# blahgeek/OpenCV-octVR

Hardware: AMD Instinct MI355X
Metric: stitched megapixels/sec (6x4K->8K equirect) (higher is better)
Workload: dtype u8

## Files before the change

### include/octvr_hip.h

```cpp
#ifndef OCTVR_HIP_H
#define OCTVR_HIP_H

#include <stddef.h>
#include <stdint.h>

#ifdef __cplusplus
extern "C" {
#endif

#define OCTVR_HIP_ABI_VERSION 1

enum {
    OCTVR_OK = 0,
    OCTVR_E_INVALID = -1,
    OCTVR_E_PARSE = -2,
    OCTVR_E_HIP = -3,
    OCTVR_E_UNSUPPORTED = -4,
    OCTVR_E_IO = -5
};

typedef struct octvr_rig octvr_rig;
typedef struct octvr_mapper octvr_mapper;

typedef struct {
    int roi_x, roi_y, roi_w, roi_h;
    const float* map1;
    const float* map2;
    const uint8_t* mask;
    const uint8_t* seam_mask;
    const float* vignette;
    int vignette_w, vignette_h;
} octvr_input_view;

int octvr_abi_version(void);
const char* octvr_last_error(void);
int octvr_device_count(int* count);

int octvr_dev_malloc(int device, size_t bytes, void** ptr);
int octvr_dev_free(void* ptr);
int octvr_memcpy_h2d(void* dst_dev, const void* src_host, size_t bytes);
int octvr_memcpy_d2h(void* dst_host, const void* src_dev, size_t bytes);
int octvr_stream_sync(void* stream);

int octvr_rig_create_json(const char* json, int out_w, int out_h, int use_roi, int device, octvr_rig** rig);
#define OCTVR_JSON_EXACT 1
int octvr_rig_create(const char* out_type, const char* out_opts_json, int out_w, int out_h, int device, int flags,
                     octvr_rig** rig);
int octvr_rig_add_input(octvr_rig* rig, const char* type, const char* opts_json, int overlay, int use_roi, int flags);
int octvr_rig_load_dat(const char* path, octvr_rig** rig);
typedef size_t (*octvr_read_fn)(void* ctx, void* buf, size_t n);
typedef size_t (*octvr_write_fn)(void* ctx, const void* data, size_t n);
int octvr_rig_load_stream(octvr_read_fn read, void* ctx, octvr_rig** rig);
int octvr_rig_dump_stream(octvr_rig* rig, octvr_write_fn write, void* ctx);
int octvr_rig_dump_dat(octvr_rig* rig, const char* path);
int octvr_rig_create_masks(octvr_rig* rig, int device);
int octvr_rig_create_from_arrays(int out_w, int out_h, int n_inputs, const int* rois, const float* const* map1,
                                 const float* const* map2, const uint8_t* const* masks,
                                 const uint8_t* const* seam_masks_or_null, octvr_rig** rig);
int octvr_rig_set_vignette(octvr_rig* rig, int i, int overlay, const float* map, int w, int h);
int octvr_rig_add_overlay_arrays(octvr_rig* rig, const int* roi, const float* map1, const float* map2,
                                 const uint8_t* mask);
int octvr_rig_num_inputs(const octvr_rig* rig, int* n);
int octvr_rig_out_size(const octvr_rig* rig, int* w, int* h);
int octvr_rig_get_input(const octvr_rig* rig, int i, octvr_input_view* view);

int octvr_rig_num_overlays(const octvr_rig* rig, int* n);
int octvr_rig_get_overlay(const octvr_rig* rig, int i, octvr_input_view* view);
int octvr_rig_morph_controlpoints(octvr_rig* rig, const char* control_points_json, int* n_used);
int octvr_rig_get_triangles(const octvr_rig* rig, int i, float* src, float* dst, int cap, int* n);
void octvr_rig_destroy(octvr_rig* rig);
int octvr_rig_clone(const octvr_rig* rig, octvr_rig** out);

int octvr_mapper_create(const octvr_rig* rig, int device, int n_inputs, const int* in_w, const int* in_h, int blend,
                        int enable_gain, int scale_w, int scale_h, octvr_mapper** mapper);
#define OCTVR_REMAP_TEXTURE 1
int octvr_mapper_create_ex(const octvr_rig* rig, int device, int n_inputs, const int* in_w, const int* in_h, int blend,
                           int enable_gain, int scale_w, int scale_h, int flags, octvr_mapper** mapper);
int octvr_mapper_stitch_yuv420p(octvr_mapper* mapper, const uint8_t* const* in_dev, const size_t* in_pitch,
                                uint8_t* out_dev, size_t out_pitch, const double* gains, int n_gains, void* stream);
int octvr_mapper_stitch_batch(octvr_mapper* mapper, int n_frames, const uint8_t* const* in_dev, const size_t* in_pitch,
                              uint8_t* const* out_dev, size_t out_pitch, const double* gains, void* stream);
int octvr_mapper_stitch_preview(octvr_mapper* mapper, const uint8_t* const* in_dev, const size_t* in_pitch,
                                uint8_t* out_dev, size_t out_pitch, uint8_t* preview_dev, int preview_w, int preview_h,
                                size_t preview_pitch, const double* gains, int n_gains, void* stream);
int octvr_mapper_gains(octvr_mapper* mapper, double* gains, int n);
#define OCTVR_MAX_FRAMES_IN_FLIGHT 16
int octvr_mapper_set_frames_in_flight(octvr_mapper* mapper, int k);
enum { OCTVR_PIX_YUV420P = 0, OCTVR_PIX_NV12 = 1 };
int octvr_mapper_set_pixel_formats(octvr_mapper* mapper, int in_format, int out_format);
int octvr_mapper_pixel_formats(const octvr_mapper* mapper, int* in_format, int* out_format);
int octvr_mapper_traffic(const octvr_mapper* mapper, double* bytes_per_frame);
int octvr_mapper_traffic_parts(const octvr_mapper* mapper, double* lut_bytes, double* frame_bytes);
int octvr_mapper_set_timing(octvr_mapper* mapper, int enable);
int octvr_mapper_kernel_time(octvr_mapper* mapper, double* total_ms, int* launches);
int octvr_mapper_kernel_busy(octvr_mapper* mapper, double* span_ms, double* busy_ms, int* launches);
int octvr_mapper_kernel_intervals(octvr_mapper* mapper, double* start_ms, double* end_ms, int cap, int* n);
int octvr_interval_union(const double* start, const double* end, int n, double* span, double* busy);
int octvr_mapper_info(const octvr_mapper* mapper, char* buf, size_t len);
void octvr_mapper_destroy(octvr_mapper* mapper);

typedef struct octvr_async octvr_async;
int octvr_async_create(const octvr_rig* const* rigs, int n_rigs, int device, int n_inputs, const int* in_w,
                       const int* in_h, int out_w, int out_h, const int* blend_modes, const int* gain_modes,
                       const double* output_regions, octvr_async** async);
int octvr_async_create_ex(const octvr_rig* const* rigs, int n_rigs, int device, int n_inputs, const int* in_w,
                          const int* in_h, int out_w, int out_h, const int* blend_modes, const int* gain_modes,
                          const double* output_regions, int flags, octvr_async** async);
int octvr_async_create_preview(const octvr_rig* const* rigs, int n_rigs, int device, int n_inputs, const int* in_w,
                               const int* in_h, int out_w, int out_h, const int* blend_modes, const int* gain_modes,
                               const double* output_regions, int flags, int preview_w, int preview_h,
                               octvr_async** async);
typedef struct octvr_preview_header {
    int width, height;
    int step;
    double fps;
} octvr_preview_header;
int octvr_async_pop_preview(octvr_async* async, uint8_t* rgb, size_t pitch, octvr_preview_header* hdr);
typedef void (*octvr_preview_sink)(void* user, const uint8_t* rgb, size_t pitch, const octvr_preview_header* hdr);
int octvr_async_set_preview_sink(octvr_async* async, octvr_preview_sink sink, void* user);
int octvr_async_info(const octvr_async* async, char* buf, size_t len);
int octvr_async_set_pixel_formats(octvr_async* async, int in_format, int out_format);
int octvr_async_pixel_formats(const octvr_async* async, int* in_format, int* out_format);
int octvr_async_push(octvr_async* async, const uint8_t* const* in_planes, const size_t* in_pitches,
                     uint8_t* const* out_planes, const size_t* out_pitches);
int octvr_async_push_device(octvr_async* async, const uint8_t* const* in_dev, const size_t* in_pitch,
                            uint8_t* out_dev, size_t out_pitch, void* ready_event);
int octvr_async_pop(octvr_async* async);
int octvr_async_register_output(octvr_async* async, uint8_t* const* planes, const size_t* pitches);
int octvr_async_unregister_output(octvr_async* async, uint8_t* const* planes);
int octvr_async_pending(const octvr_async* async, int* n);
void octvr_async_destroy(octvr_async* async);

typedef struct octvr_fastmapper octvr_fastmapper;
int octvr_fastmapper_create(const octvr_rig* rig, int device, int n_inputs, const int* in_w, const int* in_h,
                            octvr_fastmapper** fastmapper);
int octvr_fastmapper_stitch_nv12(octvr_fastmapper* fastmapper, const uint8_t* const* in_dev, const size_t* in_pitch,
                                 uint8_t* out_dev, size_t out_pitch, void* stream);
int octvr_fastmapper_stitch_nv12_batch(octvr_fastmapper* fastmapper, int n_frames, const uint8_t* const* in_dev,
                                       const size_t* in_pitch, uint8_t* const* out_dev, size_t out_pitch, void* stream);
int octvr_fastmapper_traffic(const octvr_fastmapper* fastmapper, double* bytes);
int octvr_fastmapper_traffic_parts(const octvr_fastmapper* fastmapper, double* lut_bytes, double* frame_bytes);
void octvr_fastmapper_destroy(octvr_fastmapper* fastmapper);

int octvr_remap_u8(const uint8_t* src_dev, int sw, int sh, size_t spitch, int cn, const float* map1_dev,
                   const float* map2_dev, int mw, int mh, size_t mpitch_elems, float scale_x, float scale_y,
                   uint8_t* dst_dev, size_t dpitch, void* stream);

int octvr_fill_poly_u8(uint8_t* img, int w, int h, const int* pts, int npts, uint8_t color);
int octvr_png_decode_rgb(const uint8_t* png, size_t n, uint8_t* rgb, size_t rgb_cap, int* w, int* h);

int octvr_rig_lut_recomputed(const octvr_rig* rig, int i, uint64_t* n);
int octvr_debug_project_f64(const char* json, int out_w, int out_h, int input, int device, int where, double* x,
                            double* y, uint8_t* fragile);
int octvr_debug_fastmapper_audit(const octvr_rig* rig, int n_inputs, const int* in_w, const int* in_h, int force_wide,
                                 int pitch_pad, char* json, size_t len);
int octvr_debug_tiled_lut_info(const octvr_rig* rig, int n_inputs, const int* in_w, const int* in_h, int flags,
                               char* json, size_t len);
int octvr_debug_gain_plan(const octvr_rig* rig, int n_inputs, const int* in_w, const int* in_h, int flags,
                          uint32_t* samples, uint16_t* partners, size_t cap, size_t* count);
int octvr_debug_json_number(const char* json, int flags, double* value);
int octvr_debug_pack_runs(int n_inputs, const int* in_w, const int* in_h, const uint32_t* runs, int n_runs,
                          const uint8_t* const* planes, const size_t* pitches, int format, uint8_t* packed, size_t cap,
                          size_t* sizes, size_t* bytes);
int octvr_debug_worker_failure(int n_threads, int failing);
int octvr_selftest_sat_u8(const float* in_dev, uint8_t* out_dev, int n, int method, void* stream);

#ifdef __cplusplus
}
#endif
#endif
```

### opencv-octvr_amd/csrc/composite.hip

```cpp
#include <hip/hip_runtime.h>
#include <hip/hip_ext.h>

#include <algorithm>
#include <cfloat>
#include <cstddef>
#include <cstdint>
#include <cstring>

#include "device_common.hpp"
#include "kernels.hpp"

namespace octvr {

static_assert(sizeof(TileSlot) == 16, "TileSlot layout");

static_assert(offsetof(FrameBatch<1>, src) == 0 && offsetof(FrameBatch<4>, src) == 0, "FrameBatch layout");
__device__ __forceinline__ SourceFrame kernarg_frame(uint32_t idx) {
    const kSourceFrame* kf = (const kSourceFrame*)__builtin_amdgcn_kernarg_segment_ptr();
    SourceFrame s;
    s.yuv = kf[idx].yuv;
    s.w = kf[idx].w;
    s.h = kf[idx].h;
    s.pitch = kf[idx].pitch;
    s.vig = kf[idx].vig;
// ... 53 lines not shown
#pragma unroll
        for (int j = 1; j < kTileSlots; j++) q += (j < nslots && c >= (int)(slot_word(m, j, 3) & 0xFFFFu)) ? 1 : 0;
    }
    const uint32_t d0 = slot_word(m, q, 0), d1 = slot_word(m, q, 1);
    const uint32_t d2 = slot_word(m, q, 2), d3 = slot_word(m, q, 3);
    s.cam = s.live ? (d0 & 31u) : 0u;
    s.bw = d0 >> 16;
    s.bh = d1 & 0xFFFFu;
    s.lds = d1 >> 16;
    s.bx0 = d2 & 0xFFFFu;
    s.by0 = d2 >> 16;
    s.chunk0 = d3 & 0xFFFFu;
    s.f = kernarg_frame(m.fbase + s.cam);
    return s;
}

template <bool DWORD_STAGE, bool VIG, int IN = kInPlanar>
__device__ __forceinline__ void stage_load(const StageSlot& s, uint32_t stride, uint32_t g, StageGroup& sg,
                                           bool nv12 = false) {
    const bool ok = s.live && (g & kGroupValid) != 0u;
    const uint32_t row_k = ok ? (g & 255u) : 0u, col_k = ok ? (g >> 8) & 31u : 0u;
    const SourceFrame& f = s.f;
    const bool img = s.bx0 + col_k * 8u < (uint32_t)f.w && s.by0 + row_k < (uint32_t)f.h;
    const uint32_t row = img ? row_k : 0u, col = img ? col_k : 0u;
    const uint32_t p32 = (uint32_t)f.pitch;
    const gu8* base = (const gu8*)f.yuv;
    const gu8* Yb = base + (int64_t)s.by0 * f.pitch + s.bx0;
    const gu8* Ub = base + (int64_t)(f.h + (int)(s.by0 >> 1)) * f.pitch + (s.bx0 >> 1);
    const gu8* Vb = Ub + (f.w >> 1);
    const uint32_t oy = __umul24(row, p32) + col * 8u, oc = __umul24(row >> 1, p32) + col * 4u;
    if (IN == kInNv12 || (IN == kInRuntime && nv12)) {
        const gu8* Cp = base + (int64_t)(f.h + (int)(s.by0 >> 1)) * f.pitch + s.bx0 + (oc + col * 4u);
        if (DWORD_STAGE) {
            const uint64_t yy = *(const gu64*)(Yb + oy);
            const uint64_t cc = *(const gu64*)Cp;
            sg.y0 = (uint32_t)yy;
            sg.y1 = (uint32_t)(yy >> 32);
            sg.uq = (uint32_t)cc;
            sg.vq = (uint32_t)(cc >> 32);
        } else {
            const gu8* Yp = Yb + oy;
            sg.y0 = (uint32_t)Yp[0] | ((uint32_t)Yp[1] << 8) | ((uint32_t)Yp[2] << 16) | ((uint32_t)Yp[3] << 24);
            sg.y1 = (uint32_t)Yp[4] | ((uint32_t)Yp[5] << 8) | ((uint32_t)Yp[6] << 16) | ((uint32_t)Yp[7] << 24);
            sg.uq = (uint32_t)Cp[0] | ((uint32_t)Cp[1] << 8) | ((uint32_t)Cp[2] << 16) | ((uint32_t)Cp[3] << 24);
            sg.vq = (uint32_t)Cp[4] | ((uint32_t)Cp[5] << 8) | ((uint32_t)Cp[6] << 16) | ((uint32_t)Cp[7] << 24);
        }
    } else if (DWORD_STAGE) {
        const uint64_t yy = *(const gu64*)(Yb + oy);
        sg.y0 = (uint32_t)yy;
        sg.y1 = (uint32_t)(yy >> 32);
        sg.uq = *(const gu32*)(Ub + oc);
        sg.vq = *(const gu32*)(Vb + oc);
    } else {
        const gu8* Yp = Yb + oy;
        const gu8* Up = Ub + oc;
        const gu8* Vp = Vb + oc;
        sg.y0 = (uint32_t)Yp[0] | ((uint32_t)Yp[1] << 8) | ((uint32_t)Yp[2] << 16) | ((uint32_t)Yp[3] << 24);
        sg.y1 = (uint32_t)Yp[4] | ((uint32_t)Yp[5] << 8) | ((uint32_t)Yp[6] << 16) | ((uint32_t)Yp[7] << 24);
        sg.uq = (uint32_t)Up[0] | ((uint32_t)Up[1] << 8) | ((uint32_t)Up[2] << 16) | ((uint32_t)Up[3] << 24);
        sg.vq = (uint32_t)Vp[0] | ((uint32_t)Vp[1] << 8) | ((uint32_t)Vp[2] << 16) | ((uint32_t)Vp[3] << 24);
    }
    sg.flags = img ? 0u : kStageBlack;
    if (IN == kInRuntime && nv12) sg.flags |= kStageNv12;
    sg.dst = ok ? (int32_t)(s.lds + __umul24(row_k, stride) + col_k * 8u) : -1;
    if (VIG) {
        const float* gv = f.vig ? f.vig + (int64_t)(s.by0 + row) * f.w + s.bx0 + col * 8u
                                : reinterpret_cast<const float*>(f.yuv);
        sg.g0 = *reinterpret_cast<const float4*>(gv);
        sg.g1 = *reinterpret_cast<const float4*>(gv + 4);
        if (!f.vig) sg.flags |= kStageNoVig;
    }
}

__device__ __forceinline__ uint16_t group_issue(const __amdgpu_buffer_rsrc_t& gr, int t, int t_end, int lg) {
    const int tt = (t < t_end ? t : 0) >> lg;
    return __builtin_amdgcn_raw_buffer_load_b16(gr, (uint32_t)threadIdx.x * 2u,
                                                (uint32_t)uniform(tt) * (uint32_t)(kGroupFirst * 64 * 2), 0);
}

template <bool VIG, int IN = kInPlanar>
__device__ __forceinline__ void stage_store(const StageGroup& sg, uint32_t* s_rgb) {
    if (sg.dst < 0) return;
    const bool black = (sg.flags & kStageBlack) != 0;
    const uint32_t y0 = black ? 0u : sg.y0, y1 = black ? 0u : sg.y1;
    uint32_t uq = black ? 0u : sg.uq ^ 0x80808080u, vq = black ? 0u : sg.vq ^ 0x80808080u;
    auto ch = [](uint32_t w, int k) { return (float)(signed char)((w >> (8 * k)) & 255u); };
    uint4 a, b;
    if constexpr (IN == kInNv12) {
        yuv2_to_rgba_c(y0 & 255u, (y0 >> 8) & 255u, ch(uq, 0), ch(uq, 1), a.x, a.y);
        yuv2_to_rgba_c((y0 >> 16) & 255u, y0 >> 24, ch(uq, 2), ch(uq, 3), a.z, a.w);
        yuv2_to_rgba_c(y1 & 255u, (y1 >> 8) & 255u, ch(vq, 0), ch(vq, 1), b.x, b.y);
        yuv2_to_rgba_c((y1 >> 16) & 255u, y1 >> 24, ch(vq, 2), ch(vq, 3), b.z, b.w);
    } else {
        if (IN == kInRuntime && (sg.flags & kStageNv12)) {
            const uint32_t lo = uq, hi = vq;
            uq = __builtin_amdgcn_perm(hi, lo, 0x06040200u);
            vq = __builtin_amdgcn_perm(hi, lo, 0x07050301u);
        }
        yuv2_to_rgba_c(y0 & 255u, (y0 >> 8) & 255u, ch(uq, 0), ch(vq, 0), a.x, a.y);
        yuv2_to_rgba_c((y0 >> 16) & 255u, y0 >> 24, ch(uq, 1), ch(vq, 1), a.z, a.w);
        yuv2_to_rgba_c(y1 & 255u, (y1 >> 8) & 255u, ch(uq, 2), ch(vq, 2), b.x, b.y);
        yuv2_to_rgba_c((y1 >> 16) & 255u, y1 >> 24, ch(uq, 3), ch(vq, 3), b.z, b.w);
    }
    if (VIG && !(sg.flags & kStageNoVig)) {
        a.x = vig_mul(a.x, sg.g0.x);
        a.y = vig_mul(a.y, sg.g0.y);
        a.z = vig_mul(a.z, sg.g0.z);
        a.w = vig_mul(a.w, sg.g0.w);
        b.x = vig_mul(b.x, sg.g1.x);
        b.y = vig_mul(b.y, sg.g1.y);
        b.z = vig_mul(b.z, sg.g1.z);
        b.w = vig_mul(b.w, sg.g1.w);
    }
    *reinterpret_cast<uint4*>(s_rgb + sg.dst) = a;
    *reinterpret_cast<uint4*>(s_rgb + sg.dst + 4) = b;
}

constexpr int kStitchBlocksPerCU = 6;
constexpr int kStitchRegBlocks = kStitchBlocksPerCU + 1;
constexpr int kStitchSgprs = 96, kStitchVgprs = 72;
constexpr int kStitchTexRegBlocks = 5, kStitchTexVgprs = 96;

__device__ __forceinline__ uint4 meta_issue(const __amdgpu_buffer_rsrc_t& mr, int t, int t_end, int lg) {
    const int lane = threadIdx.x & 63;
    const int tt = (t < t_end ? t : 0) >> lg;
    typedef unsigned int u32x4 __attribute__((ext_vector_type(4)));
    uint4 v;
    if (lane < kMetaWords) {
        const u32x4 r = __builtin_amdgcn_raw_buffer_load_b128(mr, (uint32_t)lane * 16u,
                                                              (uint32_t)uniform(tt) * (uint32_t)(kMetaWords * 16), 0);
        v = uint4{r.x, r.y, r.z, r.w};
    }
    return v;
}

__device__ __forceinline__ TileMeta meta_read(const uint4& v, int t, int lg, int cam_lg) {
    TileMeta m;
    m.t = t;
    m.frame = (uint32_t)t & ((1u << lg) - 1u);
    m.fbase = m.frame << cam_lg;
    m.v = v;
    m.tile = (uint32_t)__builtin_amdgcn_readlane((int)v.x, 0);
    m.nslots = (uint32_t)__builtin_amdgcn_readlane((int)v.y, 0);
    m.stride = (uint32_t)__builtin_amdgcn_readlane((int)v.w, 0);
    m.map = (uint32_t)__builtin_amdgcn_readlane((int)v.z, 0);
    return m;
}

struct TileData {
    uint4 e4[kItemHalves];
    StageGroup sg;
};

template <bool DWORD_STAGE, bool VIG, bool E24, int IN = kInPlanar>
__device__ __forceinline__ void data_issue(const __amdgpu_buffer_rsrc_t& er, const TileMeta& m, int t_end, int lg,
                                           const StageSlot& sl, uint32_t g, TileData& d, bool nv12 = false) {
    const bool live = m.t < t_end;
    const int tid = threadIdx.x;
#pragma unroll
    for (int h = 0; h < kItemHalves; h++) {
        const uint32_t so =
            (uint32_t)uniform(((live ? m.t : 0) >> lg) * kItemHalves + h) * (uint32_t)(kTilePx * (E24 ? 3 : 4));
        if constexpr (E24) {
            typedef unsigned int u32x3e __attribute__((ext_vector_type(3)));
            const u32x3e v = __builtin_amdgcn_raw_buffer_load_b96(er, (uint32_t)tid * 12u, so, 0);
            d.e4[h] = uint4{v.x, v.y, v.z, 0u};
        } else {
            typedef unsigned int u32x4e __attribute__((ext_vector_type(4)));
            const u32x4e v = __builtin_amdgcn_raw_buffer_load_b128(er, (uint32_t)tid * 16u, so, 0);
            d.e4[h] = uint4{v.x, v.y, v.z, v.w};
        }
    }
    if (!sl.live) {
        d.sg.dst = -1;
        return;
    }
    stage_load<DWORD_STAGE, VIG, IN>(sl, m.stride & ((1u << kStrideBits) - 1u), g, d.sg, nv12);
}

template <int MODE>
__device__ __forceinline__ QuadOut finish_any(const float (&rgb)[4][3], const f32x2_t (&gain)[4]) {
    if constexpr (MODE == 0) {
        return finish_quad2f(rgb, gain);
    } else {
        uint32_t px[4];
#pragma unroll
        for (int p = 0; p < 4; p++) {
            uint32_t v = pack_u8(rgb[p][0] * gain[p].x, 0, 0u);
            v = pack_u8(rgb[p][1] * gain[p].x, 1, v);
            px[p] = pack_u8(rgb[p][2] * gain[p].x, 2, v);
        }
        return QuadOut{px[0], px[1], px[2], px[3]};
    }
}

struct RgbaSink {
    __amdgpu_buffer_rsrc_t rsrc;
    const MbCamLevel* cams;
};

__device__ __forceinline__ OutFrame make_result_frame(const RgbaOut& r) {
    OutFrame o;
    o.rsrc = __builtin_amdgcn_make_buffer_rsrc(r.res, 0, (int)r.res_bytes, 0x00020000);
    o.pitch = r.res_pitch;
    o.u_off = r.res_u_off;
    o.v_off = r.res_v_off;
    return o;
}

template <int OUT = kOutPlanar>
__device__ __forceinline__ void store_result(const OutFrame& o, bool rgba, const QuadOut& q, int x, int y, bool in) {
    if (rgba) {
        typedef unsigned int u32x2 __attribute__((ext_vector_type(2)));
        const uint32_t off = in ? (uint32_t)y * o.pitch + (uint32_t)x * 4u : kDropOffset;
        __builtin_amdgcn_raw_buffer_store_b64(u32x2{q.y01, q.y23}, o.rsrc, off, 0, 0);
        __builtin_amdgcn_raw_buffer_store_b64(u32x2{q.u, q.v}, o.rsrc, in ? off + o.pitch : kDropOffset, 0, 0);
        return;
    }
    const uint32_t px[4] = {q.y01, q.y23, q.u, q.v};
    store_quad<OUT>(o, quad_yuv(px), x, y, in);
}

__device__ __forceinline__ void store_rgba(const RgbaSink& o, const QuadOut& q, uint32_t cam, int x, int y, bool in) {
    typedef __attribute__((address_space(4))) const MbCamLevel kMbCamLevel;
    const kMbCamLevel* c = (const kMbCamLevel*)o.cams + uniform((int)cam);
    const int ox = c->ox, oy = c->oy, cw = c->w, chh = c->h;
    const uint32_t goff = c->g_off, gp = c->g_pitch;
    const int xl = x - ox, yl = y - oy;
    const bool ok = in && xl >= 0 && yl >= 0 && xl < cw && yl < chh;
    const uint32_t off = ok ? goff + (uint32_t)yl * gp + (uint32_t)xl * 4u : kDropOffset;
    typedef unsigned int u32x2 __attribute__((ext_vector_type(2)));
    const u32x2 r0 = {q.y01, q.y23}, r1 = {q.u, q.v};
    __builtin_amdgcn_raw_buffer_store_b64(r0, o.rsrc, off, 0, 0);
    __builtin_amdgcn_raw_buffer_store_b64(r1, o.rsrc, ok ? off + gp : kDropOffset, 0, 0);
}

template <int MODE, int OUT = kOutPlanar>
__device__ __forceinline__ void store_half(const OutFrame& of, const RgbaSink& ro, bool res_rgba, const QuadOut& q,
                                           uint32_t cam, uint32_t flags, int h, int x, int y, bool in) {
    if constexpr (MODE == 0) {
        store_quad<OUT>(of, q, x, y, in);
    } else {
        const int q4 = (int)((threadIdx.x & 63u) >> 4);
        if (flags & item_g0_bit(h, q4)) store_rgba(ro, q, cam, x, y, in);
        if (flags & item_result_bit(h, q4)) store_result<OUT>(of, res_rgba, q, x, y, in);
    }
}

struct alignas(16) StitchLds {
    uint32_t rgb[kTileLdsBytes / 4];
    uint32_t spare[kMaxCams];
    f32x2_t slot_gain[kTileSlots];
    uint32_t claim[2];
    uint32_t pad[2];
};
static_assert(sizeof(StitchLds) == 0x4000, "the weight table at LDS 0x4000 (wtab_read)");

__device__ __forceinline__ uint2 wtab_read(uint32_t e) {
    typedef __attribute__((address_space(3))) const uint64_t lds_u64;
    const uint64_t w = *(const lds_u64*)(uintptr_t)((e & 0x1FF8u) | 0x4000u);
    return uint2{(uint32_t)w, (uint32_t)(w >> 32)};
}

__device__ __forceinline__ uint32_t tap_off(uint32_t e) { return (e >> 13) & 0x3FFFu; }

constexpr int kPfPlanar = 0, kPfNv12 = 3, kPfRuntime = 4;
template <bool DWORD_STAGE, int MODE, bool VIG, bool TEX, int LG, bool E24, int PF = kPfPlanar>
__device__ __forceinline__ void stitch_tiled_body(const FrameBatch<1 << LG>& frames, TiledLut lut, int W, int H, int use_gain,
                                                  int64_t out_pitch, RgbaOut rgba, int pix = 0) {
    constexpr int IN = PF == kPfRuntime ? kInRuntime : PF == kPfNv12 ? kInNv12 : kInPlanar;
    constexpr int OUT = PF == kPfRuntime ? kOutRuntime : PF == kPfNv12 ? kOutNv12 : kOutPlanar;
    const bool in_nv12 = IN == kInRuntime ? (pix & kPixInNv12) != 0 : IN == kInNv12;
    const bool out_nv12 = OUT == kOutRuntime ? (pix & kPixOutNv12) != 0 : OUT == kOutNv12;
    __shared__ StitchLds L;
    extern __shared__ __attribute__((aligned(16))) uint2 s_wtab[];
    uint32_t* const s_rgb = L.rgb;
    float* const s_gain = reinterpret_cast<float*>(s_wtab + 1024);
    constexpr int lg = LG, cam_lg = LG <= 1 ? 5 : 4;
    static_assert(MODE == 0 || LG == 0, "frame batches: MODE 0 only");
    f32x2_t* const s_slot_gain = L.slot_gain;
    uint32_t* const s_claim = L.claim;
    constexpr int kItemH = kTileH * kItemHalves;

    const int groups = kStitchBands;
    const int g = blockIdx.x % groups;
    const int step = (gridDim.x - g + groups - 1) / groups;
    const int t_begin = lut.bands[g] << lg;
    const int t_end = lut.bands[g + 1] << lg;
    const __amdgpu_buffer_rsrc_t ersrc = __builtin_amdgcn_make_buffer_rsrc(
        const_cast<uint32_t*>(lut.entries), 0,
        (int)((uint32_t)max(lut.n_items, 1) * (uint32_t)(kItemHalves * kTilePx * (E24 ? 3 : 4))), 0x00020000);
    const __amdgpu_buffer_rsrc_t mrsrc = __builtin_amdgcn_make_buffer_rsrc(
        const_cast<TileHdr*>(lut.meta), 0, (int)((uint32_t)max(lut.n_items, 1) * (uint32_t)(kMetaWords * 16)), 0x00020000);
    const __amdgpu_buffer_rsrc_t grsrc = __builtin_amdgcn_make_buffer_rsrc(
        const_cast<uint16_t*>(lut.grp0), 0, (int)((uint32_t)max(lut.n_items, 1) * (uint32_t)(kGroupFirst * 64 * 2)), 0x00020000);
    const __amdgpu_buffer_rsrc_t g1rsrc =
        __builtin_amdgcn_make_buffer_rsrc(const_cast<uint16_t*>(lut.grp1), 0, (int)(lut.n_grp1 * 2u), 0x00020000);
    OutFrame of{};
    RgbaSink ro{};
    bool res_rgba = false;
    const int out_bytes = (int)((uint32_t)out_pitch * (uint32_t)(H + H / 2));
    if constexpr (MODE == 0) {
        of = make_out_frame(kernarg_out<1 << LG>(0), W, H, out_pitch, out_nv12);
    } else {
        ro = RgbaSink{__builtin_amdgcn_make_buffer_rsrc(rgba.base, 0, (int)rgba.bytes, 0x00020000), rgba.cams};
        of = make_result_frame(rgba);
        res_rgba = rgba.res_rgba != 0;
    }
    const int tid = threadIdx.x;
    const int qx = tid & 63, qy = tid >> 6;

    if (tid < (1 << (lg + cam_lg))) {
        const double* gf = kernarg_gains<1 << LG>((uint32_t)tid >> cam_lg);
        s_gain[tid] = use_gain ? (float)gf[tid & ((1 << cam_lg) - 1)] : 1.0f;
    }
    if (tid < kTileZeroDwords) s_rgb[tid] = 0u;
#pragma unroll
    for (int k = 0; k < 4; k++) s_wtab[tid + 256 * k] = bilerp_weights((uint32_t)(tid + 256 * k));
    const int t0 = t_begin + (int)(blockIdx.x / groups);
    const int dyn0 = t_begin + 3 * step;
    uint32_t* const q = lut.queue + g * kQueueStride;
    const int wave = uniform(tid >> 6);
    TileMeta cur = meta_read(meta_issue(mrsrc, t0, t_end, lg), t0, lg, cam_lg);
    const uint32_t g0 = group_issue(grsrc, t0, t_end, lg);
    __syncthreads();
    TileData d;
    data_issue<DWORD_STAGE, VIG, E24, IN>(ersrc, cur, t_end, lg, stage_slot<true>(cur, t_end, wave), g0, d, in_nv12);
    int t_mv = t0 + step < t_end ? t0 + step : t_end;
    int t_n2 = t_mv < t_end && t0 + 2 * step < t_end ? t0 + 2 * step : t_end;
    uint4 mv = meta_issue(mrsrc, t_mv, t_end, lg);
    uint16_t mg = group_issue(grsrc, t_mv, t_end, lg);
    uint32_t claim = 0u;
    bool claimed = false;
    bool first = true;
    asm volatile("" : "+v"(mv.x), "+v"(mv.y), "+v"(mv.z), "+v"(mv.w), "+v"(mg));
#pragma unroll
    for (int h = 0; h < kItemHalves; h++) {
        asm volatile("" : "+v"(d.e4[h].x), "+v"(d.e4[h].y), "+v"(d.e4[h].z));
        if constexpr (!E24) asm volatile("" : "+v"(d.e4[h].w));
    }
    asm volatile("" : "+v"(d.sg.y0), "+v"(d.sg.y1), "+v"(d.sg.uq), "+v"(d.sg.vq));

    QuadOut prev[kItemHalves];
#pragma unroll
    for (int h = 0; h < kItemHalves; h++) prev[h] = QuadOut{0u, 0u, 0u, 0u};
    int px = 0, py = 0;
    const uint32_t lane_y = (uint32_t)(2 * qy) * of.pitch + (uint32_t)(2 * qx),
                   lane_c = (uint32_t)qy * of.pitch + (uint32_t)(out_nv12 ? 2 * qx : qx);
    int pox = 0, poy = 0;
    bool pfull = false;
    uint32_t pcam = 0, pfl = 0;
    uint32_t pfr = 0;
    bool pin = false;
    uint32_t par = 0;
    while (cur.t < t_end) {
        const int x = (int)(cur.tile & 0xFFFFu) * kTileW + qx * 2, y = (int)(cur.tile >> 16) * kItemH + qy * 2;
        const uint32_t S = cur.stride & ((1u << kStrideBits) - 1u);
        uint4 e4[kItemHalves];
#pragma unroll
        for (int h = 0; h < kItemHalves; h++) e4[h] = d.e4[h];
        __syncthreads();
        if (tid < kTileZeroDwords) s_rgb[tid] = 0u;
        const TileMeta nxt = meta_read(mv, t_mv, lg, cam_lg);
        {
            const uint32_t cw = (uint32_t)__shfl((int)cur.v.x, 1 + (tid & 3), 64);
            const float gs = s_gain[cur.fbase + (cw & 31u)];
            const float gc = MODE == 0 ? __builtin_fminf(__builtin_fmaxf(gs, 0.f), FLT_MAX) : gs;
            if (tid < kTileSlots) s_slot_gain[tid] = f32x2_t{gc, gc};
        }
        if (claimed && tid == 0) s_claim[par] = claim;
        stage_store<VIG, IN>(d.sg, s_rgb);
        const uint32_t nch = (cur.nslots >> 8) & 0xFFu;
        if (nch > (uint32_t)kGroupFirst) {
            const uint32_t ovf = cur.stride >> kStrideBits;
            for (int c = kGroupFirst + wave; c < (int)nch; c += 4) {
                const uint32_t gk = __builtin_amdgcn_raw_buffer_load_b16(
                    g1rsrc, (uint32_t)(tid & 63) * 2u, (ovf + (uint32_t)(c - kGroupFirst)) * 128u, 0);
                StageGroup sg;
                stage_load<DWORD_STAGE, VIG, IN>(stage_slot(cur, t_end, c), S, gk, sg, in_nv12);
                stage_store<VIG, IN>(sg, s_rgb);
            }
        }
        __syncthreads();
        if (!first) {
            const uint32_t cv = min((uint32_t)uniform((int)s_claim[par]), 0x3FFFFFFFu);
            const int v = claimed ? dyn0 + (int)cv : t_end;
            t_n2 = v < t_end ? v : t_end;
        }
        first = false;
        if (MODE == 0 && lg) of.rsrc = __builtin_amdgcn_make_buffer_rsrc(kernarg_out<1 << LG>(pfr), 0, out_bytes, 0x00020000);
        if (MODE == 0 && pfull) {
#pragma unroll
            for (int h = 0; h < kItemHalves; h++) {
                const uint32_t sy = (uint32_t)uniform((poy + h * kTileH) * (int)of.pitch + pox);
                const uint32_t sc =
                    (uint32_t)uniform(((poy + h * kTileH) >> 1) * (int)of.pitch + (out_nv12 ? pox : pox >> 1));
                __builtin_amdgcn_raw_buffer_store_b16((uint16_t)prev[h].y01, of.rsrc, lane_y, sy, kOutPolicy);
                __builtin_amdgcn_raw_buffer_store_b16((uint16_t)prev[h].y23, of.rsrc, lane_y, sy + of.pitch, kOutPolicy);
                if (out_nv12) {
                    __builtin_amdgcn_raw_buffer_store_b16((uint16_t)(prev[h].u | prev[h].v << 8), of.rsrc, lane_c,
                                                          sc + of.u_off, kOutPolicy);
                } else {
                    __builtin_amdgcn_raw_buffer_store_b8((uint8_t)prev[h].u, of.rsrc, lane_c, sc + of.u_off, kOutPolicy);
                    __builtin_amdgcn_raw_buffer_store_b8((uint8_t)prev[h].v, of.rsrc, lane_c, sc + of.v_off, kOutPolicy);
                }
            }
        } else {
#pragma unroll
            for (int h = 0; h < kItemHalves; h++)
                store_half<MODE, OUT>(of, ro, res_rgba, prev[h], pcam, pfl, h, px, py + h * kTileH, pin && py + h * kTileH < H);
        }
        data_issue<DWORD_STAGE, VIG, E24, IN>(ersrc, nxt, t_end, lg, stage_slot<true>(nxt, t_end, wave), mg, d, in_nv12);
        mv = meta_issue(mrsrc, t_n2, t_end, lg);
        mg = group_issue(grsrc, t_n2, t_end, lg);
        t_mv = t_n2;
        claimed = t_n2 < t_end;
        if (claimed && tid == 0) {
            int zero = tid;
            asm volatile("" : "+v"(zero));
            claim = __hip_atomic_fetch_add(q + zero, 1u, __ATOMIC_RELAXED, __HIP_MEMORY_SCOPE_AGENT);
        }
#pragma unroll
        for (int h = 0; h < kItemHalves; h++) {
            const uint32_t ent[4] = {e4[h].x, E24 ? __builtin_amdgcn_alignbit(e4[h].y, e4[h].x, 24u) : e4[h].y,
                                     E24 ? __builtin_amdgcn_alignbit(e4[h].z, e4[h].y, 16u) : e4[h].z,
                                     E24 ? e4[h].z >> 8 : e4[h].w};
            float rgb[4][3];
            f32x2_t gain[4];
#pragma unroll
            for (int p = 0; p < 4; p++) {
                const uint32_t e = ent[p];
                const uint8_t* r0 = reinterpret_cast<const uint8_t*>(s_rgb) +
                                    (TEX ? (e >> 15) & 0x3FFCu : E24 ? (e >> 10) & 0x3FFCu : tap_off(e));
                const uint8_t* r1 = r0 + 4u * S;
                const uint32_t c00 = reinterpret_cast<const uint32_t*>(r0)[0];
                const uint32_t c01 = reinterpret_cast<const uint32_t*>(r0)[1];
                const uint32_t c10 = reinterpret_cast<const uint32_t*>(r1)[0];
                const uint32_t c11 = reinterpret_cast<const uint32_t*>(r1)[1];
                if constexpr (TEX) {
                    tex_bilerp_f(c00, c01, c10, c11, (e >> 1) & 255u, (e >> 9) & 255u, rgb[p]);
                    gain[p] = *reinterpret_cast<const f32x2_t*>(reinterpret_cast<const uint8_t*>(s_slot_gain) + ((e >> 30) << 3));
                } else {
                    bilerp_rgba_w(c00, c01, c10, c11, wtab_read(E24 ? e << 1 : e), rgb[p]);
                    const uint32_t go = E24 ? (e << 3) & 0x18u : e >> 27;
                    gain[p] = *reinterpret_cast<const f32x2_t*>(reinterpret_cast<const uint8_t*>(s_slot_gain) + go);
                }
                if (MODE == 1 && !E24 && (e & kEntryNoGain)) gain[p] = f32x2_t{1.0f, 1.0f};
            }
            prev[h] = finish_any<MODE>(rgb, gain);
        }
        px = x;
        py = y;
        pox = (int)(cur.tile & 0xFFFFu) * kTileW;
        poy = (int)(cur.tile >> 16) * kItemH;
        pfull = pox + kTileW <= W && poy + kItemH <= H;
        pcam = (cur.nslots >> 16) & 31u;
        pfr = cur.frame;
        pfl = MODE == 1 ? (cur.map >> 8) & 0xFFFFu : 0u;
        pin = x < W && y < H;
        par ^= 1u;
        cur = nxt;
    }
    if (tid == 0) {
        asm volatile("s_waitcnt vmcnt(0)" ::: "memory");
        (void)claim;
        if (__hip_atomic_fetch_add(lut.queue + kStitchBands * kQueueStride, 1u, __ATOMIC_RELAXED,
                                   __HIP_MEMORY_SCOPE_AGENT) == gridDim.x - 1) {
            for (int k = 0; k <= kStitchBands; k++)
                __hip_atomic_exchange(lut.queue + k * kQueueStride, 0u, __ATOMIC_RELAXED, __HIP_MEMORY_SCOPE_AGENT);
        }
    }
    if (MODE == 0 && lg) of.rsrc = __builtin_amdgcn_make_buffer_rsrc(kernarg_out<1 << LG>(pfr), 0, out_bytes, 0x00020000);
#pragma unroll
    for (int h = 0; h < kItemHalves; h++)
        store_half<MODE, OUT>(of, ro, res_rgba, prev[h], pcam, pfl, h, px, py + h * kTileH, pin && py + h * kTileH < H);
}

template <bool DWORD_STAGE, int MODE, bool VIG, int LG, bool E24, int PF = kPfPlanar>
__global__ void __launch_bounds__(256, kStitchRegBlocks) __attribute__((amdgpu_num_sgpr(kStitchSgprs)))
__attribute__((amdgpu_num_vgpr(kStitchVgprs))) stitch_tiled_kernel(FrameBatch<1 << LG> frames, TiledLut lut, int W, int H,
                                                                   int use_gain, int64_t out_pitch, RgbaOut rgba) {
    stitch_tiled_body<DWORD_STAGE, MODE, VIG, false, LG, E24, PF>(frames, lut, W, H, use_gain, out_pitch, rgba);
}
template <int MODE, bool TEX, int LG, bool E24>
__global__ void __launch_bounds__(256, kStitchTexRegBlocks) __attribute__((amdgpu_num_sgpr(kStitchSgprs)))
__attribute__((amdgpu_num_vgpr(kStitchTexVgprs))) stitch_tiled_pix_kernel(FrameBatch<1 << LG> frames, TiledLut lut, int W,
                                                                          int H, int use_gain, int64_t out_pitch,
                                                                          RgbaOut rgba, int pix) {
    stitch_tiled_body<false, MODE, true, TEX, LG, E24, kPfRuntime>(frames, lut, W, H, use_gain, out_pitch, rgba, pix);
}
template <bool DWORD_STAGE, int MODE, bool VIG, int LG>
__global__ void __launch_bounds__(256, kStitchTexRegBlocks) __attribute__((amdgpu_num_sgpr(kStitchSgprs)))
__attribute__((amdgpu_num_vgpr(kStitchTexVgprs))) stitch_tiled_tex_kernel(FrameBatch<1 << LG> frames, TiledLut lut, int W,
                                                                          int H, int use_gain, int64_t out_pitch,
                                                                          RgbaOut rgba) {
    stitch_tiled_body<DWORD_STAGE, MODE, VIG, true, LG, false>(frames, lut, W, H, use_gain, out_pitch, rgba);
}

template <int MODE>
__global__ void __launch_bounds__(256) stitch_wide_kernel(FrameSet frames, TiledLut lut, int W, int H,
                                                          const double* gains, int use_gain, uint8_t* out,
                                                          int64_t out_pitch, RgbaOut rgba, int pix) {
    __shared__ float s_gain[kMaxCams];
    const int tid = threadIdx.x;
    if (tid < kMaxCams) s_gain[tid] = use_gain ? (float)gains[tid] : 1.0f;
    __syncthreads();
    OutFrame of{};
    RgbaSink ro{};
    if constexpr (MODE == 0) {
        of = make_out_frame(out, W, H, out_pitch, (pix & kPixOutNv12) != 0);
    } else {
        ro = RgbaSink{__builtin_amdgcn_make_buffer_rsrc(rgba.base, 0, (int)rgba.bytes, 0x00020000), rgba.cams};
        of = make_result_frame(rgba);
    }
    const uint32_t tile = (uint32_t)uniform((int)lut.wide_tiles[blockIdx.x]);
    const int x = (int)(tile & 0xFFFFu) * kTileW + (tid & 63) * 2, y = (int)(tile >> 16) * kTileH + (tid >> 6) * 2;
    const uint4* wp = reinterpret_cast<const uint4*>(lut.wide + (int64_t)blockIdx.x * kTilePx) + tid * 2;
    const uint4 e0 = wp[0], e1 = wp[1];
    const uint32_t xy[4] = {e0.x, e0.z, e1.x, e1.z};
    const uint32_t cd[4] = {e0.y, e0.w, e1.y, e1.w};
    Taps tp[4];
#pragma unroll
    for (int p = 0; p < 4; p++) {
        if (pix & kPixInNv12)
            gather_taps<true>(frames, xy[p], cd[p], tp[p]);
        else
            gather_taps<false>(frames, xy[p], cd[p], tp[p]);
    }
    uint32_t rgb[4][3];
    f32x2_t gain[4];
#pragma unroll
    for (int p = 0; p < 4; p++) {
        if (cd[p] & kCodeTex)
            tex_bilerp(tp[p].c[0], tp[p].c[1], tp[p].c[2], tp[p].c[3], tp[p].fx, tp[p].fy, rgb[p]);
        else
            bilerp_rgba(tp[p].c[0], tp[p].c[1], tp[p].c[2], tp[p].c[3], tp[p].fx, tp[p].fy, rgb[p]);
        float gp = (MODE == 1 && (cd[p] & kCodeNoGain)) ? 1.0f : s_gain[(cd[p] >> 10) & 31u];
        gain[p] = f32x2_t{gp, gp};
    }
    const uint32_t camb = MODE == 1 ? (uint32_t)uniform((int)lut.wide_cams[blockIdx.x]) : 0u;
    float rgbf[4][3];
#pragma unroll
    for (int p = 0; p < 4; p++)
#pragma unroll
        for (int ch = 0; ch < 3; ch++) rgbf[p][ch] = (float)rgb[p][ch];
    const uint32_t fl = ((camb >> 8) & 15u) | ((camb >> 12) & 15u) << 8;
    store_half<MODE, kOutRuntime>(of, ro, rgba.res_rgba != 0, finish_any<MODE>(rgbf, gain), camb & 31u, fl, 0, x, y,
                                  x < W && y < H);
}

struct TiledLaunch {
    int blocks;
    const FrameSet* frames;
    const double* const* gains;
    uint8_t* const* out;
    const TiledLut& lut;
    int W, H, use_gain;
    int64_t out_pitch;
    const RgbaOut& rgba;
    hipStream_t s;
    hipEvent_t ev0, ev1;
    int pix;
    bool dw, vig;
    int lg;
};

template <bool DW, int MODE, bool V, bool TEX, int LG, bool E24, int PF>
constexpr auto tiled_kernel() {
    if constexpr (PF == kPfRuntime)
        return &stitch_tiled_pix_kernel<MODE, TEX, LG, E24>;
    else if constexpr (TEX)
        return &stitch_tiled_tex_kernel<DW, MODE, V, LG>;
    else
        return &stitch_tiled_kernel<DW, MODE, V, LG, E24, PF>;
}

static hipError_t stitch_lds_check(const void* kernel) {
    hipFuncAttributes a;
    const hipError_t e = hipFuncGetAttributes(&a, kernel);
    if (e != hipSuccess) return e;
    return a.sharedSizeBytes == sizeof(StitchLds) ? hipSuccess : hipErrorInvalidKernelFile;
}

constexpr uint32_t kStitchDynLds = kWtabBytes + 4u * 2u * kMaxCams;

template <int LG>
static void frame_batch(const FrameSet* frames, const double* const* gains, uint8_t* const* out,
                        FrameBatch<1 << LG>& fb) {
    constexpr int cam_lg = FrameBatch<1 << LG>::kCamLog2;
    memset(&fb, 0, sizeof fb);
    for (int f = 0; f < (1 << LG); f++) {
        for (int i = 0; i < (1 << cam_lg); i++) fb.src[(f << cam_lg) + i] = frames[f].f[i];
        fb.out[f] = out ? out[f] : nullptr;
        fb.gains[f] = gains[f];
    }
}

template <bool DW, int MODE, bool V, bool TEX, int LG, bool E24, int PF>
static hipError_t launch_tiled(const TiledLaunch& a) {
    static_assert(PF != kPfNv12 || !TEX, "compiled-in NV12: the default sampling's instances");
    constexpr auto kernel = tiled_kernel<DW, MODE, V, TEX, LG, E24, PF>();
    static const hipError_t lds_ok = stitch_lds_check(reinterpret_cast<const void*>(kernel));
    if (lds_ok != hipSuccess) return lds_ok;
    FrameBatch<1 << LG> fb;
    frame_batch<LG>(a.frames, a.gains, a.out, fb);
    const dim3 grid(a.blocks), block(256);
    if constexpr (PF == kPfRuntime) {
        if (a.ev0) (void)hipEventRecord(a.ev0, a.s);
        hipLaunchKernelGGL(kernel, grid, block, kStitchDynLds, a.s, fb, a.lut, a.W, a.H, a.use_gain, a.out_pitch, a.rgba,
                           a.pix);
        if (a.ev0) (void)hipEventRecord(a.ev1, a.s);
    } else if constexpr (TEX) {
        hipLaunchKernelGGL(kernel, grid, block, kStitchDynLds, a.s, fb, a.lut, a.W, a.H, a.use_gain, a.out_pitch, a.rgba);
        if (a.ev0) (void)hipEventRecord(a.ev1, a.s);
    } else if (a.ev0) {
        hipExtLaunchKernelGGL(kernel, grid, block, kStitchDynLds, a.s, a.ev0, a.ev1, 0, fb, a.lut, a.W, a.H, a.use_gain,
                              a.out_pitch, a.rgba);
    } else {
        hipLaunchKernelGGL(kernel, grid, block, kStitchDynLds, a.s, fb, a.lut, a.W, a.H, a.use_gain, a.out_pitch, a.rgba);
    }
    return hipGetLastError();
}

template <bool DW, int MODE, bool V, bool TEX, bool E24, int PF = kPfPlanar>
static hipError_t launch_tiled_lg(const TiledLaunch& a) {
    if constexpr (MODE == 0) {
        if (a.lg == 1) return launch_tiled<DW, MODE, V, TEX, 1, E24, PF>(a);
        if (a.lg == 2) return launch_tiled<DW, MODE, V, TEX, 2, E24, PF>(a);
    }
    if (a.lg != 0) return hipErrorInvalidValue;
    return launch_tiled<DW, MODE, V, TEX, 0, E24, PF>(a);
}

template <int MODE, bool TEX, bool E24>
static hipError_t launch_tiled_vd(const TiledLaunch& a) {
    if (a.pix) {
        if constexpr (MODE == 0 && !TEX) {
            if (a.pix == (kPixInNv12 | kPixOutNv12) && a.dw && !a.vig)
                return launch_tiled_lg<true, MODE, false, TEX, E24, kPfNv12>(a);
        }
        return launch_tiled_lg<false, MODE, true, TEX, E24, kPfRuntime>(a);
    }
    if (a.dw && !a.vig) return launch_tiled_lg<true, MODE, false, TEX, E24>(a);
    if (a.dw) return launch_tiled_lg<true, MODE, true, TEX, E24>(a);
    if (!a.vig) return launch_tiled_lg<false, MODE, false, TEX, E24>(a);
    return launch_tiled_lg<false, MODE, true, TEX, E24>(a);
}

template <int MODE, bool TEX>
static hipError_t launch_tiled_for(const TiledLaunch& a) {
    if constexpr (!TEX) {
        if (a.lut.e24) return launch_tiled_vd<MODE, TEX, true>(a);
    } else {
        if (a.lut.e24) return hipErrorInvalidValue;
    }
    return launch_tiled_vd<MODE, TEX, false>(a);
}

template <int MODE>
static hipError_t launch_composite(const FrameSet* frames, int nf, const TiledLut& lut, int W, int H,
                                   const double* const* gains, int use_gain, uint8_t* const* out, int64_t out_pitch,
                                   const RgbaOut& rgba, hipStream_t s, hipEvent_t ev0 = nullptr,
                                   hipEvent_t ev1 = nullptr, int pix = 0) {
    if (pix & ~(kPixInNv12 | kPixOutNv12)) return hipErrorInvalidValue;
    if (lut.n_items > 0 && lut.qpl != kItemHalves) return hipErrorInvalidValue;
    const int lg = nf == 1 ? 0 : nf == 2 ? 1 : nf == 4 ? 2 : -1;
    if (lg < 0 || (MODE == 1 && nf != 1)) return hipErrorInvalidValue;
    const int cam_lg = nf <= 2 ? 5 : 4;
    for (int f = 0; f < nf; f++)
        for (int i = 1 << cam_lg; i < kMaxCams; i++)
            if (frames[f].f[i].yuv) return hipErrorInvalidValue;
    const bool ext_ev = ev0 && lut.n_items > 0 && lut.n_wide == 0;
    if (ev0 && !ext_ev) {
        const hipError_t e = hipEventRecord(ev0, s);
        if (e != hipSuccess) return e;
    }
    if (lut.n_items > 0) {
        const int units = lut.n_items * nf;
        int blocks = std::min(units, 256 * kStitchBlocksPerCU);
        if (units < 3 * 256 * kStitchBlocksPerCU) blocks = (units + 2) / 3;
        blocks = std::max(8, (blocks + 7) / 8 * 8);
        bool dw = true, vig = false;
        for (int f = 0; f < nf; f++)
            for (int i = 0; i < kMaxCams; i++) {
                const SourceFrame& sf = frames[f].f[i];
                if (!sf.yuv) continue;
                if ((reinterpret_cast<uintptr_t>(sf.yuv) & 7u) || (sf.pitch & 7) || (sf.w & 7)) dw = false;
                vig |= sf.vig != nullptr;
            }
        const TiledLaunch a{blocks, frames, gains, out, lut, W, H, use_gain, out_pitch, rgba, s,
                            ext_ev ? ev0 : nullptr, ext_ev ? ev1 : nullptr, pix, dw, vig, lg};
        const hipError_t e = lut.tex ? launch_tiled_for<MODE, true>(a) : launch_tiled_for<MODE, false>(a);
        if (e != hipSuccess) return e;
    }
    if (lut.n_wide > 0)
        for (int f = 0; f < nf; f++)
            hipLaunchKernelGGL(stitch_wide_kernel<MODE>, dim3(lut.n_wide), dim3(256), 0, s, frames[f], lut, W, H,
                               gains[f], use_gain, out ? out[f] : nullptr, out_pitch, rgba, pix);
    if (ev0 && !ext_ev) {
        const hipError_t e = hipEventRecord(ev1, s);
        if (e != hipSuccess) return e;
    }
    return hipGetLastError();
}

int composite_qpl() { return kItemHalves; }

hipError_t launch_stitch_batch(const FrameSet* frames, int nf, const TiledLut& lut, int W, int H,
                               const double* const* gains, int use_gain, uint8_t* const* out, int64_t out_pitch,
                               hipStream_t s, hipEvent_t ev0, hipEvent_t ev1, int pix) {
    if (nf < 1 || nf > kMaxBatch) return hipErrorInvalidValue;
    return launch_composite<0>(frames, nf, lut, W, H, gains, use_gain, out, out_pitch, RgbaOut{}, s, ev0, ev1, pix);
}

hipError_t launch_stitch(const FrameSet& frames, const TiledLut& lut, int W, int H, const double* gains,
                         int use_gain, uint8_t* out, int64_t out_pitch, hipStream_t s, hipEvent_t ev0, hipEvent_t ev1,
                         int pix) {
    return launch_composite<0>(&frames, 1, lut, W, H, &gains, use_gain, &out, out_pitch, RgbaOut{}, s, ev0, ev1, pix);
}

hipError_t launch_mb_remap(const FrameSet& frames, const TiledLut& lut, const double* gains, int use_gain,
                           const RgbaOut& out, hipStream_t s, int pix) {
    const int p = (pix & kPixInNv12) | ((out.res && !out.res_rgba && out.res_v_off == 0u) ? kPixOutNv12 : 0);
    return launch_composite<1>(&frames, 1, lut, 1 << 16, 1 << 16, &gains, use_gain, nullptr, 0, out, s, nullptr, nullptr, p);
}

__global__ void __launch_bounds__(256) resize_rgba_yuv420_kernel(const uint8_t* __restrict__ rgba, int sw, int sh,
                                                                 int64_t spitch, float fx, float fy, uint8_t* out,
                                                                 int dw, int dh, int64_t out_pitch, int out_nv12) {
    const OutFrame of = make_out_frame(out, dw, dh, out_pitch, out_nv12 != 0);
    const int qw = dw >> 1, qh = dh >> 1;
    const int64_t total = (int64_t)qw * qh;
    for (int64_t q = (int64_t)blockIdx.x * blockDim.x + threadIdx.x; q < total; q += (int64_t)gridDim.x * blockDim.x) {
        const int qy = (int)(q / qw), qx = (int)(q - (int64_t)qy * qw);
        uint32_t rgb[4][3];
#pragma unroll
        for (int p = 0; p < 4; p++) {
            const int x = 2 * qx + (p & 1), y = 2 * qy + (p >> 1);
            const float src_x = (float)x * fx, src_y = (float)y * fy;
            const int x1 = (int)floorf(src_x), y1 = (int)floorf(src_y);
            const int x2 = x1 + 1, y2 = y1 + 1;
            const int x2r = min(x2, sw - 1), y2r = min(y2, sh - 1);
            const uint32_t* r1 = reinterpret_cast<const uint32_t*>(rgba + (int64_t)y1 * spitch);
            const uint32_t* r2 = reinterpret_cast<const uint32_t*>(rgba + (int64_t)y2r * spitch);
            const uint32_t c00 = r1[x1], c01 = r1[x2r], c10 = r2[x1], c11 = r2[x2r];
            const float w00 = ((float)x2 - src_x) * ((float)y2 - src_y);
            const float w01 = (src_x - (float)x1) * ((float)y2 - src_y);
            const float w10 = ((float)x2 - src_x) * (src_y - (float)y1);
            const float w11 = (src_x - (float)x1) * (src_y - (float)y1);
#pragma unroll
            for (int ch = 0; ch < 3; ch++) {
                const uint32_t sh8 = 8u * ch;
                float o = 0.f;
                o = __builtin_fmaf((float)((c00 >> sh8) & 255u), w00, o);
                o = __builtin_fmaf((float)((c01 >> sh8) & 255u), w01, o);
                o = __builtin_fmaf((float)((c10 >> sh8) & 255u), w10, o);
                o = __builtin_fmaf((float)((c11 >> sh8) & 255u), w11, o);
                rgb[p][ch] = (uint32_t)sat_u8_rne(o);
            }
        }
        store_quad<kOutRuntime>(of, finish_quad_u8(rgb), 2 * qx, 2 * qy, true);
    }
}

hipError_t launch_resize_rgba_yuv420(const uint8_t* rgba, int sw, int sh, int64_t spitch, uint8_t* out, int dw, int dh,
                                     int64_t out_pitch, hipStream_t s, int out_nv12) {
    if (dw <= 0 || dh <= 0 || (dw & 1) || (dh & 1)) return hipErrorInvalidValue;
    const float fx = (float)(1.0 / ((double)dw / sw)), fy = (float)(1.0 / ((double)dh / sh));
    const int64_t total = (int64_t)(dw / 2) * (dh / 2);
    const int blocks = (int)std::min<int64_t>((total + 255) / 256, 256 * 16);
    hipLaunchKernelGGL(resize_rgba_yuv420_kernel, dim3(blocks), dim3(256), 0, s, rgba, sw, sh, spitch, fx, fy, out, dw,
                       dh, out_pitch, out_nv12);
    return hipGetLastError();
}

}
```

### opencv-octvr_amd/csrc/debug_abi.cpp

```cpp
#include <hip/hip_runtime.h>

#include <algorithm>
#include <cstdio>
#include <cstring>
#include <string>
#include <vector>

#include "abi_guard.hpp"
#include "async_host.hpp"
#include "camera_math.hpp"
#include "json_lite.hpp"
#include "mapper.hpp"

using namespace octvr;

extern "C" {

int octvr_debug_pack_runs(int n_inputs, const int* in_w, const int* in_h, const uint32_t* runs, int n_runs,
                          const uint8_t* const* planes, const size_t* pitches, int format, uint8_t* packed, size_t cap,
                          size_t* sizes, size_t* bytes) {
    return guarded([&] {
        REQUIRE(in_w && in_h && runs && planes && pitches && packed && bytes, "NULL argument");
        REQUIRE(n_inputs > 0 && n_inputs <= kMaxCams && n_runs >= 0, "bad counts");
        REQUIRE(format == OCTVR_PIX_YUV420P || format == OCTVR_PIX_NV12,
// ... 11 lines not shown
        size_t off = 0;
        for (int k = 0; k < n_runs; k++) {
            const uint32_t cam = runs[4 * k], rp = runs[4 * k + 1], g0 = runs[4 * k + 2], ng = runs[4 * k + 3];
            REQUIRE(cam < (uint32_t)n_inputs, "run: no such camera");
            const int w = in_w[cam], h = in_h[cam];
            REQUIRE(rp < (uint32_t)h / 2 && ng > 0 && g0 < (uint32_t)(w + 7) / 8 && ng <= (uint32_t)(w + 7) / 8 - g0,
                    "run outside its frame");
            const size_t n = 3 * (size_t)run_luma_bytes(w, (int)g0, (int)ng);
            REQUIRE(off + n <= cap, "buffer too small");
            const size_t got = pack_run(packed + off, w, (int)rp, (int)g0, (int)ng, planes + 3 * cam, pitches + 3 * cam, nv12);
            REQUIRE(got == n, "pack_run size");
            if (sizes) sizes[k] = got;
            off += got;
        }
        *bytes = off;
    });
}

int octvr_debug_gain_plan(const octvr_rig* rig, int n_inputs, const int* in_w, const int* in_h, int flags,
                          uint32_t* samples, uint16_t* partners, size_t cap, size_t* count) {
    return guarded([&] {
        REQUIRE(rig && in_w && in_h && count, "bad arguments");
        REQUIRE((flags & ~OCTVR_REMAP_TEXTURE) == 0, "unknown mapper flags");
        const int n = (int)rig->inputs.size();
        REQUIRE(n_inputs == n && n > 0 && n <= kGainMaxCams, "in_sizes must cover the inputs");
        const GainPlan g = plan_gain(*rig, n, std::vector<int>(in_w, in_w + n), std::vector<int>(in_h, in_h + n),
                                     (flags & OCTVR_REMAP_TEXTURE) ? 1 : 0);
        *count = g.samples.size();
        if (!samples || !partners) return;
        REQUIRE(cap >= g.samples.size(), "buffer too small");
        for (size_t k = 0; k < g.samples.size(); k++) {
            samples[2 * k] = g.samples[k].xy;
            samples[2 * k + 1] = g.samples[k].code;
            partners[k] = g.partners[k];
        }
    });
}

int octvr_debug_tiled_lut_info(const octvr_rig* rig, int n_inputs, const int* in_w, const int* in_h, int flags,
                               char* json, size_t len) {
    return guarded([&] {
        REQUIRE(rig && in_w && in_h && json && len > 0, "bad arguments");
        REQUIRE((flags & ~OCTVR_REMAP_TEXTURE) == 0, "unknown mapper flags");
        const bool tex = (flags & OCTVR_REMAP_TEXTURE) != 0;
        const int n = (int)rig->inputs.size();
        REQUIRE(n_inputs == n && n > 0 && n <= kMaxCams, "in_sizes must cover the inputs");
        const int W = rig->out_w, H = rig->out_h;
        std::vector<CompositeEntry> lut((size_t)W * H, CompositeEntry{0u, 0u});
        parallel_for((size_t)H, [&](size_t y) {
            for (int i = 0; i < n; i++) {
                const RigInput& in = rig->inputs[i];
                const int ry = (int)y - in.roi[1];
                if (ry < 0 || ry >= in.roi[3]) continue;
                for (int rx = 0; rx < in.roi[2]; rx++) {
                    const size_t k = (size_t)ry * in.roi[2] + rx;
                    if (!in.mask[k]) continue;
                    lut[y * W + (size_t)(rx + in.roi[0])] =
                        tex ? make_entry_tex(in.map1[k], in.map2[k], (float)in_w[i], (float)in_h[i], i)
                            : make_entry(in.map1[k], in.map2[k], (float)in_w[i], (float)in_h[i], i);
                }
            }
        });
        const TiledLutBuild b = build_frame_tiles(lut, W, H, std::vector<int>(in_w, in_w + n), std::vector<int>(in_h, in_h + n));
        const int qpl = b.qpl;
        double box_px = 0;
        for (int t = 0; t < b.n_items; t++)
            for (int j = 0; j < (int)(b.hdr[t].nslots & 0xFFu); j++)
                box_px += (double)b.slots[(size_t)t * kTileSlots + j].bw * b.slots[(size_t)t * kTileSlots + j].bh;
        double tap_cyc = 0, tap_extra = 0, wt_cyc = 0, wt_extra = 0, st_cyc = 0, st_extra = 0;
        {
            const int item_px = kTilePx * qpl;
            auto group_cost = [](const uint32_t* a, int n, int lanes, int banks, double& cyc, double& extra) {
                uint32_t seen[64][16];
                int cnt[64] = {};
                int mx = 0;
                for (int l = 0; l < lanes; l++)
                    for (int i = 0; i < n; i++) {
                        const uint32_t d = a[l * n + i], bk = d % (uint32_t)banks;
                        bool dup = false;
                        for (int k = 0; k < cnt[bk]; k++) dup |= seen[bk][k] == d;
                        if (!dup && cnt[bk] < 16) seen[bk][cnt[bk]++] = d;
                        mx = std::max(mx, cnt[bk]);
                    }
                cyc += std::max(mx, 1);
                extra += std::max(mx, 1) - 1;
            };
            uint32_t a[64 * 4];
            for (int t = 0; t < b.n_items; t++) {
                const TileHdr& hd = b.hdr[t];
                const uint32_t S = hd.stride & ((1u << kStrideBits) - 1u);
                const uint32_t* E = b.entries.data() + (size_t)t * item_px;
                for (int h = 0; h < qpl; h++)
                    for (int w = 0; w < 4; w++)
                        for (int p = 0; p < 4; p++) {
                            for (int half = 0; half < 2; half++) {
                                const uint32_t* e = E + (size_t)h * kTilePx + (size_t)(w * 64 + half * 32) * 4 + p;
                                for (int r = 0; r < 2; r++)
                                    for (int c = 0; c < 2; c++) {
                                        for (int l = 0; l < 32; l++)
                                            a[l] = (b.tex ? (e[l * 4] >> 17) & 0xFFFu : ((e[l * 4] >> 13) & 0x3FFFu) / 4u) + r * S + c;
                                        group_cost(a, 1, 32, 32, tap_cyc, tap_extra);
                                    }
                                if (b.tex) continue;
                                for (int l = 0; l < 32; l++) {
                                    const uint32_t d = (0x4000u | (e[l * 4] & 0x1FF8u)) / 4u;
                                    a[2 * l] = d;
                                    a[2 * l + 1] = d + 1;
                                }
                                group_cost(a, 2, 32, 64, wt_cyc, wt_extra);
                            }
                        }
                const int ns = (int)(hd.nslots & 0xFFu), nch = (int)((hd.nslots >> 8) & 0xFFu);
                const TileSlot* ts = b.slots.data() + (size_t)t * kTileSlots;
                for (int c = 0; c < nch; c++) {
                    int j = 0;
                    for (int k = 1; k < ns; k++)
                        if (c >= (int)ts[k].chunk0) j = k;
                    const uint16_t* G = c < kGroupFirst ? b.grp0.data() + ((size_t)t * kGroupFirst + c) * 64
                                                        : b.grp1.data() + ((size_t)(hd.stride >> kStrideBits) + c - kGroupFirst) * 64;
                    for (int sgi = 0; sgi < 2; sgi++)
                        for (int grp = 0; grp < 8; grp++) {
                            int n = 0;
                            for (int l = grp * 8; l < grp * 8 + 8; l++) {
                                if (!(G[l] & kGroupValid)) continue;
                                const uint32_t d = ts[j].lds + (G[l] & 255u) * S + ((G[l] >> 8) & 31u) * 8u + 4u * sgi;
                                for (int i = 0; i < 4; i++) a[n * 4 + i] = d + i;
                                n++;
                            }
                            if (n) group_cost(a, 4, n, 32, st_cyc, st_extra);
                        }
                }
            }
        }
        SourceFootprint fp;
        fp.init(std::vector<int>(in_w, in_w + n), std::vector<int>(in_h, in_h + n));
        footprint_add_tiles(fp, b);
        const double foot = fp.bytes();
        double frame_bytes = 0;
        for (int i = 0; i < n; i++) frame_bytes += 1.5 * in_w[i] * in_h[i];
        char tmp[1024];
        snprintf(tmp, sizeof tmp,
                 "{\"tex\": %d, \"footprint_bytes\": %.0f, \"frame_bytes\": %.0f, \"lds_model\": {\"tap_cycles\": %.0f, \"tap_extra\": %.0f, \"wtab_cycles\": %.0f, "
                 "\"wtab_extra\": %.0f, \"stage_cycles\": %.0f, \"stage_extra\": %.0f}, "
                 "\"items\": %d, \"wide_tiles\": %d, \"staged_px\": %.0f, \"box_px\": %.0f, \"staged_bytes\": %.0f, "
                 "\"source_bytes\": %.0f, \"grp1_entries\": %zu, ",
                 b.tex, foot, frame_bytes, tap_cyc, tap_extra, wt_cyc, wt_extra, st_cyc, st_extra, b.n_items, b.n_wide, b.staged_bytes / 2.0, box_px, b.staged_bytes, b.source_bytes,
                 b.grp1.size());
        std::string js = std::string(tmp) + b.stats + "}";
        REQUIRE(js.size() < len, "buffer too small");
        memcpy(json, js.c_str(), js.size() + 1);
    });
}

int octvr_debug_json_number(const char* json, int flags, double* value) {
    return guarded([&] {
        REQUIRE(json && value, "NULL argument");
        const JsonValue v = json_parse(json, (flags & OCTVR_JSON_EXACT) != 0);
        const JsonValue& n = v.kind == JsonValue::Array ? v[0] : v;
        *value = n.as_double();
    });
}

int octvr_debug_worker_failure(int n_threads, int failing) {
    return guarded([&] {
        REQUIRE(n_threads > 0 && n_threads <= 64, "bad arguments");
        run_threads((size_t)n_threads, [&](size_t t) {
            REQUIRE((int)t != failing, "worker " + std::to_string(t) + " failed (test hook)");
        });
    });
}

int octvr_rig_lut_recomputed(const octvr_rig* rig, int i, uint64_t* n) {
    return guarded([&] {
        REQUIRE(rig && n && i >= 0 && i < (int)rig->inputs.size(), "bad arguments");
        *n = rig->inputs[i].n_fragile;
    });
}

int octvr_debug_project_f64(const char* json, int out_w, int out_h, int input, int device, int where, double* x,
                            double* y, uint8_t* fragile) {
    return guarded([&] {
        REQUIRE(json && x && y && out_w > 0 && out_h > 0 && (where == 0 || where == 1), "bad arguments");
        JsonValue doc = json_parse(json);
        const CameraParams out_cam = camera_from_json(doc["output"]);
        const JsonValue& ins = doc["inputs"];
        REQUIRE(input >= 0 && input < (int)ins.size(), "bad input index");
        const JsonValue& cam = ins[(size_t)input];
        CameraParams c = camera_from_json(cam);
        std::vector<uint8_t> excl, incl;
        if (cam.has("options")) build_camera_masks(cam["options"], excl, incl);
        if (!excl.empty() || !incl.empty()) {
            c.sel = 0;
            c.width = cam["options"]["width"].as_int();
            c.height = cam["options"]["height"].as_int();
        }
        const size_t total = (size_t)out_w * out_h;
        if (where == 1) {
            c.excl = excl.empty() ? nullptr : excl.data();
            c.incl = nullptr;
            parallel_for((size_t)out_h, [&](size_t h) {
                for (int w = 0; w < out_w; w++)
                    project_output_to_input(out_cam, c, (double)w / out_w, (double)h / out_h, &x[h * out_w + w],
                                            &y[h * out_w + w]);
            });
            return;
        }
        REQUIRE(fragile, "fragile is NULL");
        DeviceGuard dg(device);
        DevBuf<uint8_t> excl_d;
        if (!excl.empty()) {
            excl_d.upload(excl.data(), excl.size());
            c.excl = excl_d.p;
        }
        c.incl = nullptr;
        const CameraParams both[2] = {out_cam, c};
        DevBuf<CameraParams> cams;
        cams.upload(both, 2);
        DevBuf<double> xd, yd;
        DevBuf<uint8_t> fd;
        xd.alloc(total);
        yd.alloc(total);
        fd.alloc(total);
        HIP_CHECK(launch_project_f64(cams.p, out_w, out_h, xd.p, yd.p, fd.p, nullptr));
        HIP_CHECK(hipDeviceSynchronize());
        HIP_CHECK(hipMemcpy(x, xd.p, total * sizeof(double), hipMemcpyDeviceToHost));
        HIP_CHECK(hipMemcpy(y, yd.p, total * sizeof(double), hipMemcpyDeviceToHost));
        HIP_CHECK(hipMemcpy(fragile, fd.p, total, hipMemcpyDeviceToHost));
    });
}

int octvr_selftest_sat_u8(const float* in, uint8_t* out, int n, int method, void* stream) {
    return guarded([&] {
        REQUIRE(in && out && n >= 0 && (method == 0 || method == 1), "bad arguments");
        HIP_CHECK(launch_selftest_sat(in, out, n, method, (hipStream_t)stream));
    });
}

}
```

### opencv-octvr_amd/csrc/host_common.hpp

```cpp
#pragma once

#include <hip/hip_runtime.h>

#include <algorithm>
#include <cstdint>
#include <exception>
#include <functional>
#include <iosfwd>
#include <memory>
#include <mutex>
#include <stdexcept>
#include <string>
#include <thread>
#include <vector>

#include "kernels.hpp"
#include "octvr_hip.h"

namespace octvr {

struct OctvrError : std::runtime_error {
    int code;
    OctvrError(int c, const std::string& m) : std::runtime_error(m), code(c) {}
};

#define HIP_CHECK(expr)                                                                                \
    do {                                                                                               \
        hipError_t e_ = (expr);                                                                        \
        if (e_ != hipSuccess)                                                                          \
            throw ::octvr::OctvrError(OCTVR_E_HIP, std::string(#expr) + ": " + hipGetErrorString(e_)); \
    } while (0)

#define REQUIRE(cond, msg)                                                  \
    do {                                                                    \
        if (!(cond)) throw ::octvr::OctvrError(OCTVR_E_INVALID, (msg));     \
    } while (0)

template <class F>
void run_threads(size_t T, F f) {
    std::exception_ptr first;
    std::mutex mu;
    std::vector<std::thread> th;
    th.reserve(T);
    for (size_t t = 0; t < T; t++)
        th.emplace_back([&, t] {
            try {
                f(t);
            } catch (...) {
                std::lock_guard<std::mutex> g(mu);
                if (!first) first = std::current_exception();
            }
        });
    for (auto& x : th) x.join();
    if (first) std::rethrow_exception(first);
}

template <class F>
void parallel_for(size_t n, F f) {
    const size_t T = std::max<size_t>(1, std::min<size_t>({16, (size_t)std::thread::hardware_concurrency(), n}));
    if (T <= 1) {
        for (size_t k = 0; k < n; k++) f(k);
        return;
    }
    run_threads(T, [&](size_t t) {
        for (size_t k = n * t / T; k < n * (t + 1) / T; k++) f(k);
    });
}

struct DeviceGuard {
    int prev = -1;
    explicit DeviceGuard(int dev) {
        HIP_CHECK(hipGetDevice(&prev));
        if (dev != prev) HIP_CHECK(hipSetDevice(dev));
    }
    ~DeviceGuard() {
        if (prev >= 0) (void)hipSetDevice(prev);
    }
};

template <class T>
struct DevBuf {
    T* p = nullptr;
    size_t n = 0;
    DevBuf() = default;
    DevBuf(const DevBuf&) = delete;
    DevBuf& operator=(const DevBuf&) = delete;
    DevBuf(DevBuf&& o) noexcept : p(o.p), n(o.n) { o.p = nullptr; o.n = 0; }
    ~DevBuf() { reset(); }
    void alloc(size_t count) {
        reset();
        if (count == 0) return;
        HIP_CHECK(hipMalloc(reinterpret_cast<void**>(&p), count * sizeof(T)));
        n = count;
    }
    void upload(const T* h, size_t count) {
        alloc(count);
        if (count) HIP_CHECK(hipMemcpy(p, h, count * sizeof(T), hipMemcpyHostToDevice));
    }
    void reset() {
        if (p) (void)hipFree(p);
        p = nullptr;
        n = 0;
    }
};

}

struct RigInput {
    int roi[4] = {0, 0, 0, 0};
    int in_w = 0, in_h = 0;
    std::vector<float> map1, map2;
    std::vector<uint8_t> mask;
    std::vector<float> vignette;
    int vig_w = 0, vig_h = 0;
    std::vector<float> src_tris, dst_tris;
    size_t n_fragile = 0;
};

struct octvr_rig {
    int out_w = 0, out_h = 0;
    int device = 0;
    std::vector<RigInput> inputs;
    std::vector<RigInput> overlays;
    std::vector<std::vector<uint8_t>> seam_masks;
    bool has_cameras = false;
    bool out_cam_masks = false;
    octvr::CameraParams out_cam{};
    std::vector<octvr::CameraParams> cams;
    octvr::DevBuf<uint8_t> visible;
};

namespace octvr {
void rig_create_masks(octvr_rig& rig);
struct JsonValue;
int rig_morph_controlpoints(octvr_rig& rig, const JsonValue& control_points);
void chamfer_l2_3x3(const uint8_t* src, int w, int h, float* dist);

CameraParams camera_from_json(const JsonValue& cam);
void build_camera_masks(const JsonValue& options, std::vector<uint8_t>& excl, std::vector<uint8_t>& incl);
std::unique_ptr<octvr_rig> rig_new(const JsonValue& out_cam, int out_w, int out_h, int device);
void rig_add(octvr_rig& rig, const JsonValue& cam, bool overlay, bool use_roi);
JsonValue camera_json(const char* type, const char* opts_json, int flags);

void dat_write(octvr_rig& rig, std::ostream& os);
void dat_write(octvr_rig& rig, octvr_write_fn write, void* ctx);
std::unique_ptr<octvr_rig> dat_read(std::istream& is);
std::unique_ptr<octvr_rig> dat_read(octvr_read_fn read, void* ctx);

SourceFrame checked_source_frame(const uint8_t* ptr, size_t pitch, int w, int h, const float* vig);

struct TileJob {
    int tx, ty;
    int cam;
    uint32_t flags = kItemAllG0;
};
using EntryFn = std::function<CompositeEntry(int job, int x, int y)>;
struct TiledLutBuild {
    std::vector<TileHdr> hdr;
    std::vector<TileSlot> slots;
    std::vector<uint32_t> entries;
    std::vector<CompositeEntry> wide;
    std::vector<uint32_t> wide_tiles;
    std::vector<uint16_t> wide_cams;
    std::vector<uint16_t> item_flags;
    std::vector<uint16_t> grp0, grp1;
    std::vector<int32_t> bands;
    int n_items = 0, n_wide = 0;
    int qpl = 1;
    int tex = 0;
    double staged_bytes = 0;
    double source_bytes = 0;
    std::string stats;
};
TiledLutBuild build_tiled_lut(const std::vector<TileJob>& jobs, const EntryFn& entry, const std::vector<int>& in_w,
                              const std::vector<int>& in_h, int qpl = 1);
struct TiledLutDev {
    DevBuf<TileHdr> meta;
    DevBuf<uint32_t> entries;
    DevBuf<CompositeEntry> wide;
    DevBuf<uint32_t> wide_tiles;
    DevBuf<uint16_t> wide_cams;
    DevBuf<int32_t> bands;
    DevBuf<uint32_t> queue;
    DevBuf<uint16_t> grp0, grp1;
    double staged_bytes = 0;
    double source_bytes = 0;
    double g0_bytes = 0;
    double result_bytes = 0;
    std::string stats;
    TiledLut view{};
    void upload(const TiledLutBuild& b, bool e24 = false);
};

struct SourceFootprint {
    std::vector<int> w, h;
    std::vector<std::vector<uint64_t>> bits;
    void init(const std::vector<int>& in_w, const std::vector<int>& in_h);
    int groups(int i) const { return (w[i] + 7) / 8; }
    int words(int i) const { return (groups(i) + 63) / 64; }
    int row_pairs(int i) const { return (h[i] + 1) / 2; }
    bool test(int cam, int r, int g) const { return (bits[cam][(size_t)r * words(cam) + g / 64] >> (g % 64)) & 1u; }
    void mark(int cam, int y, int g) { bits[cam][(size_t)(y >> 1) * words(cam) + g / 64] |= 1ull << (g % 64); }
    void mark_taps(const CompositeEntry& e);
    void merge(const SourceFootprint& o);
    double bytes() const;
};
void footprint_add_tiles(SourceFootprint& f, const TiledLutBuild& b);

struct OverlayListDev {
    DevBuf<uint32_t> groups;
    DevBuf<CompositeEntry> entries;
    size_t covered = 0;
    double source_bytes = 0;
    OverlayList view{};
};

class MultiBand;
struct MultiBandDeleter {
    void operator()(MultiBand* p) const;
};
MultiBand* multiband_create(const octvr_rig& rig, int device, int bands, const std::vector<int>& in_w,
                            const std::vector<int>& in_h, int feather_border = 0, SourceFootprint* foot = nullptr,
                            int tex = 0);
void multiband_run(MultiBand& mb, int slot, const FrameSet& frames, const double* gains_dev, int use_gain, uint8_t* out,
                   int64_t out_pitch, hipStream_t s, uint8_t* rgba = nullptr, int64_t rgba_pitch = 0, int pix = 0);
void multiband_set_slots(MultiBand& mb, int k);
double multiband_traffic(const MultiBand& mb);
std::string multiband_info(const MultiBand& mb);
}
```

### opencv-octvr_amd/csrc/kernels.hpp

```cpp
#pragma once

#include <hip/hip_runtime.h>
#include <cstdint>

#include "camera_math.hpp"

namespace octvr {

constexpr int kMaxCams = 32;

struct CompositeEntry {
    uint32_t xy;
    uint32_t code;
};

__host__ __device__ inline int quantize_coord(float m, float scale) {
    float X = m * scale;
    float f = X * 32.0f;
    if (!(f >= -2147483648.f && f < 2147483648.f)) return INT32_MIN;
    return (int)rintf(f);
}

__host__ __device__ inline CompositeEntry make_entry(float m1, float m2, float w, float h, int cam) {
    int ix = quantize_coord(m1, w), iy = quantize_coord(m2, h);
// ... 28 lines not shown
    c.ix1 = (unsigned)(sx + 1) < (unsigned)w;
    c.iy0 = (unsigned)sy < (unsigned)h;
    c.iy1 = (unsigned)(sy + 1) < (unsigned)h;
    c.x0 = min(max(sx, 0), w - 1);
    c.x1 = min(max(sx + 1, 0), w - 1);
    c.y0 = min(max(sy, 0), h - 1);
    c.y1 = min(max(sy + 1, 0), h - 1);
    return c;
}

constexpr int kTileW = 128, kTileH = 8, kTilePx = kTileW * kTileH;
constexpr int kTileSlots = 4;
constexpr int kItemHalves = 2;
constexpr int kTileLdsBytes = 16 * 1024 - 176;
static_assert(kTileLdsBytes <= (1 << 14), "the tiled entry's LDS byte offset field");
constexpr uint32_t kWtabBytes = 1024u * 8u;
constexpr int kTileZeroDwords = 4;
constexpr int kStageAlignDwords = 4;
constexpr uint32_t kStridePadMax = 28;

struct TileSlot {
    uint16_t cam;
    uint16_t bw, bh;
    uint16_t lds;
    uint16_t bx0, by0;
    uint16_t chunk0;
    uint16_t pad1;
};

struct TileHdr {
    uint32_t tile;
    uint32_t nslots;
    uint32_t stage_groups;
    uint32_t stride;
};
constexpr int kStrideBits = 9;
static_assert(256 + kStridePadMax < (1u << kStrideBits), "a padded stride fits its field");
constexpr int kGroupFirst = 4;
constexpr uint32_t kGroupValid = 0x8000u;

constexpr int kPixInNv12 = 1, kPixOutNv12 = 2;

struct SourceFrame {
    const uint8_t* yuv;
    int32_t w, h;
    int64_t pitch;
    const float* vig;
};

struct FrameSet {
    SourceFrame f[kMaxCams];
};

constexpr int kMaxBatch = 4;
template <int NF>
struct FrameBatch {
    static constexpr int kCamLog2 = NF <= 2 ? 5 : 4;
    SourceFrame src[NF << kCamLog2];
    uint8_t* out[NF];
    const double* gains[NF];
};


struct FastMapperPlane {
    bool compact;
    const uint2* ent;
    const uint32_t* off;
    const uint8_t* wgt;
    const uint2* hdr;
    const uint2* runs;
    uint32_t nblk;
};

struct CamTemplate {
    const float* map1;
    const float* map2;
    const uint8_t* mask;
    int32_t roi_x, roi_y, roi_w, roi_h;
    int32_t in_w, in_h;
};

constexpr int kGainMaxCams = 16;
constexpr int kGainPer = 3;
constexpr int kGainWaveRun = 64 * kGainPer;
constexpr int kGainChunk = 4 * kGainWaveRun;
constexpr int kGainTotalStride = 32;

hipError_t launch_lut_build(const CameraParams* cams_dev, int W, int H, float* map1, float* map2, uint8_t* mask,
                            int32_t* bbox, uint8_t* visible, uint32_t* fragile, uint32_t cap, hipStream_t s);

hipError_t launch_project_f64(const CameraParams* cams_dev, int W, int H, double* x, double* y, uint8_t* fragile,
                              hipStream_t s);

hipError_t launch_composite_lut(const CamTemplate* cams_dev, int n, int W, int H, CompositeEntry* lut,
                                hipStream_t s, int tex = 0);

hipError_t launch_gain_feed(const FrameSet& frames, const CompositeEntry* samples, const uint16_t* partners, int tex,
                            int n_chunks, const int32_t* N, int n,
                            unsigned long long* totals, uint32_t* tickets, double* gains, hipStream_t s,
                            bool lean = false,
                            int pix = 0);

template <int NF>
struct FastBatch {
    SourceFrame src[NF << (NF <= 2 ? 5 : 4)];
    uint8_t* out[NF];
};

template <int NF>
struct FeedBatch {
    SourceFrame src[NF * kGainMaxCams];
    unsigned long long* totals[NF];
    uint32_t* tickets[NF];
    double* gains[NF];
};
hipError_t launch_gain_feed_batch(const FrameSet* frames, int nf, const CompositeEntry* samples, const uint16_t* partners,
                                  int tex, int n_chunks, const int32_t* N, int n, unsigned long long* const* totals,
                                  uint32_t* const* tickets, double* const* gains, hipStream_t s, bool lean, int pix = 0);

hipError_t launch_set_gains(const double* host_gains, int n, double* gains_dev, hipStream_t s);

struct FootRun {
    uint32_t cam;
    uint32_t g0, ng;
    uint32_t off;
};
struct FootFrames {
    uint8_t* f[kMaxCams];
    int w[kMaxCams], h[kMaxCams];
};
hipError_t launch_unpack_runs(const uint8_t* packed, const FootRun* runs, int n_runs, const FootFrames& frames,
                              hipStream_t s);
hipError_t launch_unpack_runs_layout(const uint8_t* packed, const FootRun* runs, int n_runs, const FootFrames& frames,
                                     int nv12, hipStream_t s);
struct MergeTable;
hipError_t launch_merge_regions(uint8_t* out, const MergeTable& t, hipStream_t s);

struct TiledLut {
    const TileHdr* meta;
    const uint32_t* entries;
    int n_items;
    const uint32_t* wide_tiles;
    const CompositeEntry* wide;
    int n_wide;
    const uint16_t* wide_cams;
    const int32_t* bands;
    uint32_t* queue;
    int qpl;
    const uint16_t* grp0;
    const uint16_t* grp1;
    uint32_t n_grp1;
    int tex;
    int e24;
};
constexpr int kMetaWords = 1 + kTileSlots;
constexpr int kQueueStride = 32;
constexpr int kStitchBands = 8;
constexpr uint32_t kEntryNoGain = 1u;
constexpr int kEntrySlotShift = 30;
constexpr uint32_t kCodeNoGain = 1u << 16;

__host__ __device__ constexpr uint32_t tiled_entry(uint32_t off, uint32_t fxy, uint32_t slot, bool nogain) {
    return (nogain ? kEntryNoGain : 0u) | (fxy & 1023u) << 3 | off << 13 | slot << kEntrySlotShift;
}

__host__ __device__ constexpr uint32_t tiled_entry24(uint32_t e) {
    return (e >> 30) | ((e >> 3) & 1023u) << 2 | ((e >> 15) & 4095u) << 12;
}

__host__ __device__ constexpr uint32_t tiled_entry_tex(uint32_t off, uint32_t ab, uint32_t slot, bool nogain) {
    return (nogain ? kEntryNoGain : 0u) | (ab & 0xFFFFu) << 1 | (off >> 2) << 17 | slot << kEntrySlotShift;
}

int composite_qpl();

hipError_t launch_stitch(const FrameSet& frames_dev, const TiledLut& lut, int W, int H,
                         const double* gains, int use_gain, uint8_t* out, int64_t out_pitch, hipStream_t s,
                         hipEvent_t ev0 = nullptr, hipEvent_t ev1 = nullptr, int pix = 0);
hipError_t launch_stitch_batch(const FrameSet* frames, int nf, const TiledLut& lut, int W, int H,
                               const double* const* gains, int use_gain, uint8_t* const* out, int64_t out_pitch,
                               hipStream_t s, hipEvent_t ev0 = nullptr, hipEvent_t ev1 = nullptr, int pix = 0);

constexpr int kMbMaxBands = 10;
constexpr int kUpPatchRows = 8, kUpPatchCols = 72;
struct alignas(16) UpQuad {
    uint16_t idx[3];
    uint16_t pad0;
    uint8_t w0[3], w1[3];
    uint8_t pad1[2];
};
static_assert(sizeof(UpQuad) == 16, "UpQuad layout");

__host__ __device__ inline int up_clamp(int u, int n_src) {
    u = u < 0 ? -u : u;
    return u < n_src - 1 ? u : n_src - 1;
}
struct UpArith {
    int idx[3];
    int w0[3], w1[3];
};
__host__ __device__ inline UpArith up_arith(int g, int off, int n_local, int n_src, bool rows) {
    UpArith e;
    const int o0 = g - off;
    const int h = o0 >> 1;
    const bool odd = (o0 & 1) != 0;
    const int m8 = o0 & 7;
    const bool v0 = o0 >= 0 && o0 < n_local, v1 = o0 + 1 >= 0 && o0 + 1 < n_local;
    int u0, u2;
    if (!odd) {
        u0 = h - 1;
        u2 = h + 1 + ((rows && m8 == 6) ? 1 : 0);
        e.w0[0] = 1, e.w0[1] = 6, e.w0[2] = 1;
        e.w1[0] = 0, e.w1[1] = 4, e.w1[2] = 4;
    } else {
        u0 = h;
        u2 = h + 2 + ((rows && m8 == 5) ? 1 : 0);
        const bool q7 = rows && m8 == 7;
        e.w0[0] = 4, e.w0[1] = q7 ? 0 : 4, e.w0[2] = q7 ? 4 : 0;
        e.w1[0] = 1, e.w1[1] = 6, e.w1[2] = 1;
    }
    e.idx[0] = up_clamp(u0, n_src);
    e.idx[1] = up_clamp(u0 + 1, n_src);
    e.idx[2] = up_clamp(u2, n_src);
#pragma unroll
    for (int j = 0; j < 3; j++) {
        e.w0[j] = v0 ? e.w0[j] : 0;
        e.w1[j] = v1 ? e.w1[j] : 0;
    }
    return e;
}

struct MbCamLevel {
    uint32_t g_off;
    uint32_t g_pitch;
    int32_t ox, oy, w, h;
    const void* weight;
    const UpQuad* up_rows;
    const UpQuad* up_cols;
    const int32_t* up_r0;
    const int32_t* up_c0;
};

struct RgbaOut {
    uint8_t* base;
    uint32_t bytes;
    const MbCamLevel* cams;
    uint8_t* res;
    uint32_t res_bytes;
    uint32_t res_pitch, res_u_off, res_v_off;
    int res_rgba;
};
constexpr int kSubW = 32, kSubs = kTileW / kSubW;
__host__ __device__ constexpr uint32_t item_result_bit(int h, int q) { return 1u << (4 * h + q); }
__host__ __device__ constexpr uint32_t item_g0_bit(int h, int q) { return 1u << (8 + 4 * h + q); }
constexpr uint32_t kItemAllG0 = 0xFF00u;

hipError_t launch_mb_remap(const FrameSet& frames, const TiledLut& lut, const double* gains, int use_gain,
                           const RgbaOut& out, hipStream_t s, int pix = 0);
hipError_t launch_mb_down(const uint2* items, int n_items, const MbCamLevel* cams_l, const MbCamLevel* cams_prev,
                          const uint8_t* g_prev, uint8_t* g_l, hipStream_t s);
struct MbBlendArgs {
    int level, bands, n_cams;
    int w_u8;
    int feather;
    float out_scale;
    int W, H;
    int tiles_x;
    const uint32_t* tile_cams;
    const uint8_t* owned;
    const uint2* work;
    int n_work;
    const MbCamLevel* cams;
    const MbCamLevel* cams_next;
    const uint8_t* g;
    const uint8_t* g_next;
    const int16_t* r_next;
    int W_next, H_next;
    const UpQuad* rup_rows;
    const UpQuad* rup_cols;
    const int32_t* rup_r0;
    const int32_t* rup_c0;
    int16_t* r_out;
    uint8_t* out;
    int64_t out_pitch;
    int out_nv12;
    int out_w, out_h;
    int ax, ay, crop_w, crop_h;
    uint8_t* rgba;
    int64_t rgba_pitch;
};
hipError_t launch_mb_blend(const MbBlendArgs& a, hipStream_t s);
hipError_t launch_pyr_down_f32(const float* src, int sw, int sh, float* dst, int dw, int dh, hipStream_t s);
hipError_t launch_block_activity(const void* weight, int is_u8, int w, int h, int ox, int oy, int bx_n, uint8_t* blocks,
                                 hipStream_t s);

hipError_t launch_remap_u8(const uint8_t* src, int sw, int sh, int64_t spitch, int cn, const float* map1,
                           const float* map2, int mw, int mh, int64_t mpitch, float scale_x, float scale_y,
                           uint8_t* dst, int64_t dpitch, hipStream_t s);

hipError_t launch_morph_warp(const float* map1, const float* map2, const uint8_t* mask, int w, int h,
                             const int16_t* owner, const double* M, float* out1, float* out2, uint8_t* out_mask,
                             hipStream_t s);

struct ResizeTables {
    const int32_t* xofs;
    const int16_t* ax;
    const int32_t* rows;
    const int16_t* by;
    int32_t xmax;
    int32_t area2;
};
hipError_t launch_resize_u8(const uint8_t* src, int sw, int sh, int64_t spitch, uint8_t* dst, int dw, int dh,
                            int64_t dpitch, const ResizeTables& t, hipStream_t s);

hipError_t launch_resize_rgba_yuv420(const uint8_t* rgba, int sw, int sh, int64_t spitch, uint8_t* out, int dw, int dh,
                                     int64_t out_pitch, hipStream_t s, int out_nv12 = 0);

hipError_t launch_resize_rgba_rgb(const uint8_t* rgba, int sw, int sh, int64_t spitch, uint8_t* out, int dw, int dh,
                                  int64_t out_pitch, hipStream_t s);

// ... 15 lines not shown
```

### opencv-octvr_amd/csrc/mapper.cpp

```cpp
#include "mapper.hpp"
#include "overlay_list.hpp"

#include <hip/hip_runtime.h>

#include <cmath>
#include <cstring>
#include <memory>
#include <vector>

namespace octvr {

namespace {

void ensure_result(octvr_mapper& m) {
    if (m.result.p) return;
    REQUIRE((uint64_t)m.W * m.H * 4 < 0x7FFFFF80ull, "stitch frame larger than 2 GiB as RGBA");
    DeviceGuard dg(m.device);
    m.result.alloc((size_t)m.W * m.H * 4);
    HIP_CHECK(hipMemset(m.result.p, 0, m.result.n));
    MbCamLevel v{};
    v.g_off = 0;
    v.g_pitch = (uint32_t)m.W * 4;
    v.w = m.W;
    v.h = m.H;
// ... 174 lines not shown
    const bool timed = e0 != nullptr;
    const bool overlays = m->ov.view.n_groups > 0;
    if (timed && (m->scaled || m->mb || preview)) HIP_CHECK(hipEventRecord(e0, s));
    if (m->scaled || preview || overlays) {
        if (m->mb)
            multiband_run(*m->mb, 0, fs, sl.gains, m->use_gain, nullptr, 0, s, m->result.p, (int64_t)m->W * 4, m->pix);
        else
            HIP_CHECK(launch_mb_remap(fs, m->tiles.view, sl.gains, m->use_gain,
                                      RgbaOut{m->result.p, (uint32_t)m->result.n, m->result_view.p}, s, m->pix));
        if (overlays) HIP_CHECK(launch_overlay_apply(fs, m->ov.view, m->result.p, (int64_t)m->W * 4, s, m->pix));
        HIP_CHECK(launch_resize_rgba_yuv420(m->result.p, m->W, m->H, (int64_t)m->W * 4, out_dev, m->SW, m->SH,
                                            (int64_t)out_pitch, s, (m->pix & kPixOutNv12) != 0));
        if (preview)
            HIP_CHECK(launch_resize_rgba_rgb(m->result.p, m->W, m->H, (int64_t)m->W * 4, preview->dev, preview->w,
                                             preview->h, (int64_t)preview->pitch, s));
    } else if (m->mb) {
        multiband_run(*m->mb, m->cur_slot, fs, sl.gains, m->use_gain, out_dev, (int64_t)out_pitch, s, nullptr, 0, m->pix);
    } else {
        TiledLut view = m->tiles.view;
        view.queue = sl.queue;
        HIP_CHECK(launch_stitch(fs, view, m->W, m->H, sl.gains, m->use_gain, out_dev, (int64_t)out_pitch, s, e0, e1,
                                m->pix));
    }
    if (timed && (m->scaled || m->mb || preview)) HIP_CHECK(hipEventRecord(e1, s));
    ev.keep();
    finish_slot(sl, s);
}

void mapper_stitch_batch(octvr_mapper* m, int nb, const uint8_t* const* in_dev, const size_t* in_pitch,
                         uint8_t* const* out_dev, size_t out_pitch, const double* gains, hipStream_t s) {
    REQUIRE(m && in_dev && in_pitch && out_dev, "NULL argument");
    REQUIRE(nb == 1 || nb == 2 || nb == 4, "a batch holds 1, 2 or 4 frames");
    for (int f = 0; f < nb; f++) REQUIRE(out_dev[f], "NULL output");
    if (nb == 1 || m->scaled || m->mb) {
        for (int f = 0; f < nb; f++)
            mapper_stitch(m, in_dev + (size_t)f * m->nc, in_pitch + (size_t)f * m->nc, out_dev[f], out_pitch,
                          gains ? gains + (size_t)f * m->n : nullptr, gains ? m->n : 0, nullptr, s);
        return;
    }
    REQUIRE((int)m->slots.size() >= nb, "a batch of n frames needs n frames in flight (octvr_mapper_set_frames_in_flight)");
    REQUIRE(nb <= 2 || m->nc <= 16, "a batch of 4 frames holds 16 cameras per frame (inputs and overlays)");
    check_out_pitch(m, out_pitch);
    DeviceGuard dg(m->device);
    FrameSet fs[kMaxBatch];
    for (int f = 0; f < nb; f++) fs[f] = frame_set(m, in_dev + (size_t)f * m->nc, in_pitch + (size_t)f * m->nc);
    const double* g[kMaxBatch];
    octvr_mapper::FrameSlot* sl[kMaxBatch];
    const bool feed = m->use_gain && !gains && m->n_chunks > 0;
    unsigned long long* tot[kMaxBatch];
    uint32_t* tick[kMaxBatch];
    double* gd[kMaxBatch];
    for (int f = 0; f < nb; f++) {
        sl[f] = &take_slot(m, s);
        if (!feed) stitch_gains(m, *sl[f], fs[f], gains ? gains + (size_t)f * m->n : nullptr, nullptr, s);
        g[f] = sl[f]->gains;
        tot[f] = sl[f]->totals;
        tick[f] = sl[f]->tickets;
        gd[f] = sl[f]->gains;
    }
    if (feed)
        HIP_CHECK(launch_gain_feed_batch(fs, nb, m->samples.p, m->partners.p, m->tex, m->n_chunks, m->N.p, m->n, tot, tick,
                                         gd, s, true, m->pix));
    TimedPair ev(m);
    TiledLut view = m->tiles.view;
    view.queue = sl[0]->queue;
    HIP_CHECK(launch_stitch_batch(fs, nb, view, m->W, m->H, g, m->use_gain, out_dev, (int64_t)out_pitch, s, ev.e0, ev.e1,
                                  m->pix));
    ev.keep();
    for (int f = 0; f < nb; f++) finish_slot(*sl[f], s);
}

int mapper_num_inputs(const octvr_mapper* m) { return m->n; }
bool mapper_has_gain(const octvr_mapper* m) { return m->use_gain != 0; }
const double* mapper_gains_dev(const octvr_mapper* m) { return m->slots[m->cur_slot].gains; }
const SourceFootprint& mapper_footprint(const octvr_mapper* m) { return m->foot; }
void mapper_out_size(const octvr_mapper* m, int* w, int* h) {
    *w = m->SW;
    *h = m->SH;
}

SourceFrame checked_source_frame(const uint8_t* ptr, size_t pitch, int w, int h, const float* vig) {
    REQUIRE(ptr && pitch >= (size_t)w, "bad input frame");
    REQUIRE(pitch < ((size_t)1 << 24), "input pitch must be below 16 MiB");
    REQUIRE((uint64_t)pitch * (uint64_t)(h + h / 2) < 0x7FFFFFFFull, "input frame larger than 2 GiB");
    REQUIRE((uint64_t)pitch * (uint64_t)(h + h / 2) >= 8, "input frame below 8 bytes");
    return SourceFrame{ptr, w, h, (int64_t)pitch, vig};
}

TiledLutBuild build_frame_tiles(const std::vector<CompositeEntry>& lut, int W, int H, const std::vector<int>& in_w,
                                const std::vector<int>& in_h, int* n_jobs) {
    const int qpl = composite_qpl();
    const int tx_n = (W + kTileW - 1) / kTileW, ty_n = (H + kTileH * qpl - 1) / (kTileH * qpl);
    std::vector<TileJob> jobs;
    jobs.reserve((size_t)tx_n * ty_n);
    for (int ty = 0; ty < ty_n; ty++)
        for (int tx = 0; tx < tx_n; tx++) jobs.push_back(TileJob{tx, ty, 0});
    if (n_jobs) *n_jobs = tx_n * ty_n;
    return build_tiled_lut(jobs, [&](int, int x, int y) {
        return (x < W && y < H) ? lut[(size_t)y * W + x] : CompositeEntry{0u, 0u};
    }, in_w, in_h, qpl);
}

std::unique_ptr<octvr_mapper> mapper_create(const octvr_rig* rig, int device, int n_inputs, const int* in_w,
                                            const int* in_h, int blend, int enable_gain, int scale_w, int scale_h,
                                            int flags) {
    REQUIRE(rig && in_w && in_h, "NULL argument");
    REQUIRE((flags & ~OCTVR_REMAP_TEXTURE) == 0, "unknown mapper flags");
    const int n_in = (int)rig->inputs.size(), n_ov = (int)rig->overlays.size();
    REQUIRE(n_in + n_ov <= kMaxCams, "too many inputs and overlays");
    REQUIRE(n_inputs == n_in + n_ov, n_ov ? "in_sizes must cover every input and every overlay (N + K)"
                                          : "in_sizes must cover every input");
    REQUIRE(scale_w >= 0 && scale_h >= 0 && (scale_w == 0) == (scale_h == 0), "bad scaled output size");
    REQUIRE(rig->out_w % 2 == 0 && rig->out_h % 2 == 0, "YUV420 output needs even width/height");
    auto m = std::make_unique<octvr_mapper>();
    m->device = device;
    m->tex = (flags & OCTVR_REMAP_TEXTURE) ? 1 : 0;
    m->n = n_in;
    m->nc = n_in + n_ov;
    m->W = rig->out_w;
    m->H = rig->out_h;
    m->SW = scale_w ? scale_w : m->W;
    m->SH = scale_h ? scale_h : m->H;
    REQUIRE(m->SW % 2 == 0 && m->SH % 2 == 0, "YUV420 output needs even width/height");
    m->scaled = m->SW != m->W || m->SH != m->H;
    REQUIRE(!m->scaled || (uint64_t)m->W * m->H * 4 < 0x7FFFFF80ull, "stitch frame larger than 2 GiB as RGBA");
    m->in_w.assign(in_w, in_w + n_inputs);
    m->in_h.assign(in_h, in_h + n_inputs);
    for (int i = 0; i < m->nc; i++)
        REQUIRE(m->in_w[i] > 0 && m->in_h[i] > 0 && m->in_w[i] % 2 == 0 && m->in_h[i] % 2 == 0 &&
                    m->in_w[i] <= 65535 && m->in_h[i] <= 65535,
                "input and overlay sizes must be even and < 65536");
    m->use_gain = (enable_gain && m->n > 1) ? 1 : 0;
    m->blend = m->n > 1 ? blend : 0;
    REQUIRE(!m->use_gain || m->n <= 16, "gain estimation supports at most 16 inputs");
    DeviceGuard dg(device);
    auto camera = [&](int i) -> const RigInput& { return i < n_in ? rig->inputs[i] : rig->overlays[i - n_in]; };
    m->vig.resize(m->nc);
    for (int i = 0; i < m->nc; i++) {
        const RigInput& in = camera(i);
        if (in.vignette.empty()) continue;
        const std::vector<float> v = resize_linear_f32(in.vignette.data(), in.vig_w, in.vig_h, m->in_w[i], m->in_h[i]);
        m->vig[i].upload(v.data(), v.size());
    }
    m->foot.init(m->in_w, m->in_h);
    if (m->blend > 0) {
        const int bands = (int)(std::ceil(std::log((double)m->blend) / std::log(2.)) - 1.);
        m->mb.reset(multiband_create(*rig, device, bands, m->in_w, m->in_h, 0, &m->foot, m->tex));
    } else if (m->blend < 0) {
        m->mb.reset(multiband_create(*rig, device, 0, m->in_w, m->in_h, -m->blend, &m->foot, m->tex));
    } else {
        const std::vector<CompositeEntry> lut8 = winner_lut(*m, camera, 0, m->nc);
        const TiledLutBuild tb = build_frame_tiles(lut8, m->W, m->H, m->in_w, m->in_h, &m->n_tiles);
        footprint_add_tiles(m->foot, tb);
        m->tiles.upload(tb);
    }
    if (m->mb && n_ov) setup_overlays(*m, camera);
    if (m->scaled || m->ov.view.n_groups) ensure_result(*m);
    m->last_gains.assign(m->n, 1.0);
    if (m->use_gain) setup_gain(*m, *rig);
    m->slots.push_back(make_slot(*m));
    HIP_CHECK(hipDeviceSynchronize());
    return m;
}

void mapper_sync(octvr_mapper& m) {
    for (auto& sl : m.slots)
        if (sl.done) HIP_CHECK(hipEventSynchronize(sl.done));
}

void mapper_set_frames_in_flight(octvr_mapper* m, int k) {
    REQUIRE(m && k >= 1 && k <= OCTVR_MAX_FRAMES_IN_FLIGHT, "frames in flight must be 1..OCTVR_MAX_FRAMES_IN_FLIGHT");
    if (k > 1 && m->scaled)
        throw OctvrError(OCTVR_E_UNSUPPORTED, "frames in flight > 1 need the output at template size (no scaled output)");
    if (k > 1 && m->ov.view.n_groups)
        throw OctvrError(OCTVR_E_UNSUPPORTED, "frames in flight > 1 with overlays need blend 0 (no multi-band or feather)");
    DeviceGuard dg(m->device);
    mapper_sync(*m);
    if (m->cur_slot != 0) {
        HIP_CHECK(hipMemcpy(m->slots[0].gains, m->slots[m->cur_slot].gains, sizeof(double) * m->n,
                            hipMemcpyDeviceToDevice));
        m->cur_slot = 0;
    }
    for (size_t i = 1; i < m->slots.size(); i++)
        if (m->slots[i].done) (void)hipEventDestroy(m->slots[i].done);
    m->slots.resize(1);
    m->slot_bufs.resize(1);
    for (int i = 1; i < k; i++) m->slots.push_back(make_slot(*m));
    if (m->mb) multiband_set_slots(*m->mb, k);
    HIP_CHECK(hipDeviceSynchronize());
}

void mapper_set_timing(octvr_mapper* m, int enable) {
    REQUIRE(m && enable >= 0, "bad arguments");
    m->timing = enable;
    m->timed_calls = 0;
    if (enable) {
        DeviceGuard dg(m->device);
        constexpr size_t kEventReserve = 1024;
        while (m->free_events.size() + m->events.size() < kEventReserve) {
            hipEvent_t e0 = nullptr, e1 = nullptr;
            HIP_CHECK(hipEventCreate(&e0));
            const hipError_t e = hipEventCreate(&e1);
            if (e != hipSuccess) (void)hipEventDestroy(e0);
            HIP_CHECK(e);
            m->free_events.emplace_back(e0, e1);
        }
    }
}

int mapper_drain_timing(octvr_mapper* m, const std::function<void(double, double)>& f) {
    DeviceGuard dg(m->device);
    for (auto& e : m->events) {
        HIP_CHECK(hipEventSynchronize(e.second));
        float start = 0, len = 0;
        HIP_CHECK(hipEventElapsedTime(&start, m->events[0].first, e.first));
        HIP_CHECK(hipEventElapsedTime(&len, e.first, e.second));
        f((double)start, (double)start + (double)len);
    }
    const int launches = (int)m->events.size();
    m->free_events.insert(m->free_events.end(), m->events.begin(), m->events.end());
    m->events.clear();
    return launches;
}

double tiled_lut_bytes(const TiledLut& t) {
    return (t.e24 ? 3.0 : 4.0) * t.n_items * kTilePx * t.qpl + 8.0 * t.n_wide * kTilePx +
           (double)t.n_items * (sizeof(TileHdr) + kTileSlots * sizeof(TileSlot)) + 4.0 * t.n_wide;
}

double mapper_traffic(const octvr_mapper* m) {
    if (m->mb && m->ov.view.n_groups)
        return multiband_traffic(*m->mb) + 4.0 * m->W * m->H + 1.5 * m->SW * m->SH +
               (double)m->ov.view.n_groups * (4.0 + 8.0 * kOvGroupPx) + m->ov.source_bytes + 4.0 * (double)m->ov.covered;
    if (m->mb) return multiband_traffic(*m->mb);
    return tiled_lut_bytes(m->tiles.view) + 1.5 * m->W * m->H + m->tiles.source_bytes;
}

}
```

### opencv-octvr_amd/csrc/mapper.hpp

```cpp
#pragma once

#include <memory>
#include <utility>
#include <vector>

#include "host_common.hpp"

struct octvr_mapper {
    template <class T>
    using DevBuf = octvr::DevBuf<T>;
    int device = 0;
    int n = 0;
    int nc = 0;
    int W = 0, H = 0;
    int use_gain = 0;
    std::vector<int> in_w, in_h;
    octvr::TiledLutDev tiles;
    int n_tiles = 0;
    std::unique_ptr<octvr::MultiBand, octvr::MultiBandDeleter> mb;
    int blend = 0;
    DevBuf<octvr::CompositeEntry> samples;
    DevBuf<uint16_t> partners;
    DevBuf<int32_t> N;
    int n_chunks = 0, n_samples = 0;
    size_t n_entries = 0;
    std::vector<double> last_gains;
    std::vector<DevBuf<float>> vig;
    octvr::SourceFootprint foot;
    int tex = 0;
    int SW = 0, SH = 0;
    bool scaled = false;
    DevBuf<uint8_t> result;
    DevBuf<octvr::MbCamLevel> result_view;
    octvr::OverlayListDev ov;
    struct FrameSlot {
        double* gains = nullptr;
        unsigned long long* totals = nullptr;
        uint32_t* tickets = nullptr;
        uint32_t* queue = nullptr;
        hipEvent_t done = nullptr;
    };
    struct SlotBufs {
        DevBuf<double> gains;
        DevBuf<unsigned long long> totals;
        DevBuf<uint32_t> tickets, queue;
    };
    std::vector<FrameSlot> slots;
    std::vector<std::unique_ptr<SlotBufs>> slot_bufs;
    int cur_slot = 0;
    int timing = 0;
    uint64_t timed_calls = 0;
    int pix = 0;
    std::vector<std::pair<hipEvent_t, hipEvent_t>> events, free_events;
    ~octvr_mapper() {
        for (auto& sl : slots)
            if (sl.done) (void)hipEventDestroy(sl.done);
        for (auto* v : {&events, &free_events})
            for (auto& e : *v) {
                (void)hipEventDestroy(e.first);
                (void)hipEventDestroy(e.second);
            }
    }
};

namespace octvr {

std::unique_ptr<octvr_mapper> mapper_create(const octvr_rig* rig, int device, int n_inputs, const int* in_w,
                                            const int* in_h, int blend, int enable_gain, int scale_w, int scale_h,
                                            int flags);
struct PreviewOut {
    uint8_t* dev;
    int w, h;
    size_t pitch;
};
void mapper_stitch(octvr_mapper* m, const uint8_t* const* in_dev, const size_t* in_pitch, uint8_t* out_dev,
                   size_t out_pitch, const double* gains, int n_gains, const double* gains_dev, hipStream_t s,
                   const PreviewOut* preview = nullptr);
void mapper_stitch_batch(octvr_mapper* m, int nb, const uint8_t* const* in_dev, const size_t* in_pitch,
                         uint8_t* const* out_dev, size_t out_pitch, const double* gains, hipStream_t s);
void mapper_sync(octvr_mapper& m);
void mapper_set_frames_in_flight(octvr_mapper* m, int k);
void mapper_set_timing(octvr_mapper* m, int enable);
int mapper_drain_timing(octvr_mapper* m, const std::function<void(double start_ms, double end_ms)>& f);
double mapper_traffic(const octvr_mapper* m);
double tiled_lut_bytes(const TiledLut& t);
TiledLutBuild build_frame_tiles(const std::vector<CompositeEntry>& lut, int W, int H, const std::vector<int>& in_w,
                                const std::vector<int>& in_h, int* n_jobs = nullptr);
int mapper_num_inputs(const octvr_mapper* m);
bool mapper_has_gain(const octvr_mapper* m);
const double* mapper_gains_dev(const octvr_mapper* m);
void mapper_out_size(const octvr_mapper* m, int* w, int* h);
const SourceFootprint& mapper_footprint(const octvr_mapper* m);

struct GainPlan {
    std::vector<CompositeEntry> samples;
    std::vector<uint16_t> partners;
    std::vector<int32_t> N;
    int n_chunks = 0;
    size_t pairs_px = 0;
};
GainPlan plan_gain(const octvr_rig& rig, int n, const std::vector<int>& in_w, const std::vector<int>& in_h, int tex);
void setup_gain(octvr_mapper& m, const octvr_rig& rig);
std::vector<float> resize_linear_f32(const float* src, int sw, int sh, int dw, int dh);

}
```

### opencv-octvr_amd/csrc/octvr_hip.cpp

```cpp
#include "octvr_hip.h"

#include <hip/hip_runtime.h>

#include <algorithm>
#include <cstdio>
#include <cstring>
#include <fstream>
#include <memory>
#include <string>
#include <vector>

#include "abi_guard.hpp"
#include "json_lite.hpp"
#include "mapper.hpp"
#include "masks.hpp"

using namespace octvr;

extern "C" {

int octvr_abi_version(void) { return OCTVR_HIP_ABI_VERSION; }

const char* octvr_last_error(void) { return last_error().c_str(); }

// ... 222 lines not shown
int octvr_rig_get_overlay(const octvr_rig* rig, int i, octvr_input_view* v) {
    return guarded([&] {
        REQUIRE(rig && v && i >= 0 && i < (int)rig->overlays.size(), "bad overlay index");
        const RigInput& in = rig->overlays[i];
        v->roi_x = in.roi[0];
        v->roi_y = in.roi[1];
        v->roi_w = in.roi[2];
        v->roi_h = in.roi[3];
        v->map1 = in.map1.data();
        v->map2 = in.map2.data();
        v->mask = in.mask.data();
        v->seam_mask = nullptr;
        v->vignette = in.vignette.empty() ? nullptr : in.vignette.data();
        v->vignette_w = in.vig_w;
        v->vignette_h = in.vig_h;
    });
}

int octvr_rig_morph_controlpoints(octvr_rig* rig, const char* control_points_json, int* n_used) {
    return guarded([&] {
        REQUIRE(rig && control_points_json, "NULL argument");
        if (rig->has_cameras && rig->out_cam_masks)
            throw OctvrError(OCTVR_E_UNSUPPORTED, "morph_controlpoints with output-camera masks is not implemented");
        const JsonValue cps = json_parse(control_points_json);
        const int k = rig_morph_controlpoints(*rig, cps);
        if (n_used) *n_used = k;
    });
}

int octvr_rig_get_triangles(const octvr_rig* rig, int i, float* src, float* dst, int cap, int* n) {
    return guarded([&] {
        REQUIRE(rig && n && i >= 0 && i < (int)rig->inputs.size(), "bad input index");
        const RigInput& in = rig->inputs[i];
        const int nt = (int)in.src_tris.size() / 6;
        *n = nt;
        if (src && dst) {
            REQUIRE(cap >= nt, "triangle buffer too small");
            std::copy(in.src_tris.begin(), in.src_tris.end(), src);
            std::copy(in.dst_tris.begin(), in.dst_tris.end(), dst);
        }
    });
}

void octvr_rig_destroy(octvr_rig* rig) { delete rig; }

int octvr_rig_clone(const octvr_rig* src, octvr_rig** out) {
    return guarded([&] {
        REQUIRE(src && out, "NULL argument");
        auto r = std::make_unique<octvr_rig>();
        r->out_w = src->out_w;
        r->out_h = src->out_h;
        r->device = src->device;
        r->inputs = src->inputs;
        r->overlays = src->overlays;
        r->seam_masks = src->seam_masks;
        r->has_cameras = src->has_cameras;
        r->out_cam_masks = src->out_cam_masks;
        r->out_cam = src->out_cam;
        r->cams = src->cams;
        if (src->visible.p) {
            DeviceGuard dg(src->device);
            r->visible.alloc(src->visible.n);
            HIP_CHECK(hipMemcpy(r->visible.p, src->visible.p, src->visible.n, hipMemcpyDeviceToDevice));
        }
        *out = r.release();
    });
}

int octvr_mapper_create(const octvr_rig* rig, int device, int n_inputs, const int* in_w, const int* in_h, int blend,
                        int enable_gain, int scale_w, int scale_h, octvr_mapper** out) {
    return octvr_mapper_create_ex(rig, device, n_inputs, in_w, in_h, blend, enable_gain, scale_w, scale_h, 0, out);
}

int octvr_mapper_create_ex(const octvr_rig* rig, int device, int n_inputs, const int* in_w, const int* in_h, int blend,
                           int enable_gain, int scale_w, int scale_h, int flags, octvr_mapper** out) {
    return guarded([&] {
        REQUIRE(out, "NULL argument");
        *out = mapper_create(rig, device, n_inputs, in_w, in_h, blend, enable_gain, scale_w, scale_h, flags).release();
    });
}

int octvr_mapper_stitch_yuv420p(octvr_mapper* m, const uint8_t* const* in_dev, const size_t* in_pitch,
                                uint8_t* out_dev, size_t out_pitch, const double* gains, int n_gains, void* stream) {
    return guarded([&] {
        mapper_stitch(m, in_dev, in_pitch, out_dev, out_pitch, gains, n_gains, nullptr, (hipStream_t)stream);
    });
}

int octvr_mapper_stitch_batch(octvr_mapper* m, int n_frames, const uint8_t* const* in_dev, const size_t* in_pitch,
                              uint8_t* const* out_dev, size_t out_pitch, const double* gains, void* stream) {
    return guarded([&] {
        mapper_stitch_batch(m, n_frames, in_dev, in_pitch, out_dev, out_pitch, gains, (hipStream_t)stream);
    });
}

int octvr_mapper_stitch_preview(octvr_mapper* m, const uint8_t* const* in_dev, const size_t* in_pitch,
                                uint8_t* out_dev, size_t out_pitch, uint8_t* preview_dev, int preview_w, int preview_h,
                                size_t preview_pitch, const double* gains, int n_gains, void* stream) {
    return guarded([&] {
        const PreviewOut pv{preview_dev, preview_w, preview_h, preview_pitch};
        mapper_stitch(m, in_dev, in_pitch, out_dev, out_pitch, gains, n_gains, nullptr, (hipStream_t)stream,
                      preview_dev ? &pv : nullptr);
    });
}

int octvr_mapper_gains(octvr_mapper* m, double* g, int n) {
    return guarded([&] {
        REQUIRE(m && g && n >= m->n, "bad arguments");
        DeviceGuard dg(m->device);
        if (!m->use_gain) {
            for (int i = 0; i < n; i++) g[i] = 1.0;
            return;
        }
        const octvr_mapper::FrameSlot& sl = m->slots[m->cur_slot];
        if (sl.done) HIP_CHECK(hipEventSynchronize(sl.done));
        HIP_CHECK(hipMemcpy(g, sl.gains, m->n * sizeof(double), hipMemcpyDeviceToHost));
    });
}

int octvr_mapper_set_frames_in_flight(octvr_mapper* m, int k) {
    return guarded([&] { mapper_set_frames_in_flight(m, k); });
}

int octvr_mapper_set_pixel_formats(octvr_mapper* m, int in_format, int out_format) {
    return guarded([&] {
        REQUIRE(m, "NULL argument");
        REQUIRE((in_format == OCTVR_PIX_YUV420P || in_format == OCTVR_PIX_NV12) &&
                    (out_format == OCTVR_PIX_YUV420P || out_format == OCTVR_PIX_NV12),
                "pixel format must be OCTVR_PIX_YUV420P or OCTVR_PIX_NV12");
        DeviceGuard dg(m->device);
        mapper_sync(*m);
        m->pix = (in_format == OCTVR_PIX_NV12 ? kPixInNv12 : 0) | (out_format == OCTVR_PIX_NV12 ? kPixOutNv12 : 0);
    });
}

int octvr_mapper_pixel_formats(const octvr_mapper* m, int* in_format, int* out_format) {
    return guarded([&] {
        REQUIRE(m && in_format && out_format, "NULL argument");
        *in_format = (m->pix & kPixInNv12) ? OCTVR_PIX_NV12 : OCTVR_PIX_YUV420P;
        *out_format = (m->pix & kPixOutNv12) ? OCTVR_PIX_NV12 : OCTVR_PIX_YUV420P;
    });
}

int octvr_mapper_traffic(const octvr_mapper* m, double* bytes) {
    return guarded([&] {
        REQUIRE(m && bytes, "NULL argument");
        *bytes = mapper_traffic(m);
    });
}

int octvr_mapper_traffic_parts(const octvr_mapper* m, double* lut_bytes, double* frame_bytes) {
    return guarded([&] {
        REQUIRE(m && lut_bytes && frame_bytes, "NULL argument");
        *lut_bytes = m->mb ? 0.0 : tiled_lut_bytes(m->tiles.view);
        *frame_bytes = mapper_traffic(m) - *lut_bytes;
    });
}

int octvr_mapper_set_timing(octvr_mapper* m, int enable) {
    return guarded([&] { mapper_set_timing(m, enable); });
}

int octvr_interval_union(const double* start, const double* end, int n, double* span, double* busy) {
    return guarded([&] {
        REQUIRE(n >= 0 && span && busy && (n == 0 || (start && end)), "bad arguments");
        std::vector<std::pair<double, double>> iv;
        double sp = 0;
        for (int k = 0; k < n; k++) {
            REQUIRE(end[k] >= start[k], "interval ends before it starts");
            iv.emplace_back(start[k], end[k]);
            sp += end[k] - start[k];
        }
        std::sort(iv.begin(), iv.end());
        double bz = 0;
        bool open = false;
        double ra = 0, rb = 0;
        for (const auto& x : iv) {
            if (open && x.first <= rb) {
                rb = std::max(rb, x.second);
            } else {
                if (open) bz += rb - ra;
                ra = x.first;
                rb = x.second;
                open = true;
            }
        }
        if (open) bz += rb - ra;
        *span = sp;
        *busy = bz;
    });
}

int octvr_mapper_kernel_time(octvr_mapper* m, double* total_ms, int* launches) {
    return guarded([&] {
        REQUIRE(m && total_ms && launches, "NULL argument");
        double t = 0;
        *launches = mapper_drain_timing(m, [&](double a, double b) { t += b - a; });
        *total_ms = t;
    });
}

int octvr_mapper_kernel_busy(octvr_mapper* m, double* span_ms, double* busy_ms, int* launches) {
    return guarded([&] {
        REQUIRE(m && span_ms && busy_ms && launches, "NULL argument");
        std::vector<double> st, en;
        *launches = mapper_drain_timing(m, [&](double a, double b) {
            st.push_back(a);
            en.push_back(b);
        });
        if (octvr_interval_union(st.data(), en.data(), (int)st.size(), span_ms, busy_ms) != OCTVR_OK)
            throw OctvrError(OCTVR_E_HIP, "kernel_busy: inconsistent event timestamps");
    });
}

int octvr_mapper_kernel_intervals(octvr_mapper* m, double* start_ms, double* end_ms, int cap, int* n) {
    return guarded([&] {
        REQUIRE(m && n && cap >= 0 && (cap == 0 || (start_ms && end_ms)), "bad arguments");
        int k = 0;
        *n = mapper_drain_timing(m, [&](double a, double b) {
            if (k < cap) {
                start_ms[k] = a;
                end_ms[k] = b;
            }
            k++;
        });
    });
}

int octvr_mapper_info(const octvr_mapper* m, char* buf, size_t len) {
    return guarded([&] {
        REQUIRE(m && buf && len > 0, "bad arguments");
        char tmp[768];
        snprintf(tmp, sizeof tmp,
                 "{\"inputs\": %d, \"out\": [%d, %d], \"blend\": %d, \"tiles\": %d, \"wide_tiles\": %d, "
                 "\"staged_bytes\": %.0f, \"source_bytes\": %.0f, \"gain\": %d, \"gain_samples\": %d, \"gain_pairs_px\": %zu, "
                 "\"gain_chunks\": %d, \"scaled_out\": [%d, %d], \"footprint_bytes\": %.0f, \"overlays\": %d, "
                 "\"overlay_groups\": %d, \"overlay_px\": %zu",
                 m->n, m->W, m->H, m->blend, m->n_tiles, m->tiles.view.n_wide,
                 m->mb ? 0.0 : m->tiles.staged_bytes, m->mb ? 0.0 : m->tiles.source_bytes, m->use_gain, m->n_samples, m->n_entries, m->n_chunks, m->SW, m->SH,
                 m->foot.bytes(), m->nc - m->n, m->ov.view.n_groups, m->ov.covered);
        std::string js = tmp;
        if (m->mb) js += ", " + multiband_info(*m->mb);
        else if (!m->tiles.stats.empty()) js += ", " + m->tiles.stats;
        js += "}";
        REQUIRE(js.size() < len, "buffer too small");
        memcpy(buf, js.c_str(), js.size() + 1);
    });
}

void octvr_mapper_destroy(octvr_mapper* m) {
    if (!m) return;
    int prev = -1;
    if (hipGetDevice(&prev) == hipSuccess && prev != m->device) (void)hipSetDevice(m->device);
    delete m;
    if (prev >= 0) (void)hipSetDevice(prev);
}

int octvr_remap_u8(const uint8_t* src, int sw, int sh, size_t spitch, int cn, const float* map1, const float* map2,
                   int mw, int mh, size_t mpitch, float scale_x, float scale_y, uint8_t* dst, size_t dpitch,
                   void* stream) {
    return guarded([&] {
        REQUIRE(src && map1 && map2 && dst && sw > 0 && sh > 0 && mw >= 0 && mh >= 0, "bad arguments");
        REQUIRE(cn == 1 || cn == 3 || cn == 4, "cn must be 1, 3 or 4");
        if (mw == 0 || mh == 0) return;
        HIP_CHECK(launch_remap_u8(src, sw, sh, (int64_t)spitch, cn, map1, map2, mw, mh, (int64_t)mpitch, scale_x,
                                  scale_y, dst, (int64_t)dpitch, (hipStream_t)stream));
    });
}


}
```

### opencv-octvr_amd/csrc/tiling.cpp

```cpp
#include <algorithm>
#include <atomic>
#include <cstring>
#include <cstdlib>
#include <thread>
#include <vector>

#include "host_common.hpp"
#include "kernels.hpp"

namespace octvr {

TiledLutBuild build_tiled_lut(const std::vector<TileJob>& jobs, const EntryFn& entry, const std::vector<int>& in_w,
                              const std::vector<int>& in_h, int qpl) {
    const int n_jobs = (int)jobs.size();
    const int item_px = kTilePx * qpl;
    TiledLutBuild b;
    b.qpl = qpl;
    b.hdr.resize(n_jobs);
    b.slots.resize((size_t)n_jobs * kTileSlots);
    b.entries.assign((size_t)n_jobs * item_px, 0u);
    std::vector<uint8_t> is_wide(n_jobs, 0);
    std::vector<std::vector<CompositeEntry>> wide_raw(n_jobs);
    std::vector<std::vector<uint16_t>> grp_job(n_jobs);
    const int T = std::max(1u, std::min(16u, std::thread::hardware_concurrency()));
    std::atomic<int> any_tex{0};
    auto work = [&](int tid) {
        struct Px {
            int slot, x0, y0, fxy, mask, nogain;
        };
        std::vector<Px> px(item_px);
        std::vector<CompositeEntry> raw(item_px);
        for (int t = tid; t < n_jobs; t += T) {
            const TileJob& J = jobs[t];
            int cams[8], ns = 0;
            int minx[8], maxx[8], miny[8], maxy[8];
            bool wide = false, item_tex = false;
            for (int k = 0; k < item_px; k++) {
                const int h = k / kTilePx, q = (k % kTilePx) >> 2, p = k & 3;
                const int x = J.tx * kTileW + (q & 63) * 2 + (p & 1);
                const int y = J.ty * kTileH * qpl + h * kTileH + (q >> 6) * 2 + (p >> 1);
                const CompositeEntry e = entry(t, x, y);
                raw[k] = e;
                px[k].mask = 0;
                if (!(e.code & 0x8000u)) continue;
                const int cam = (int)((e.code >> 10) & 31u);
                const int sx = (int)(int16_t)(e.xy & 0xFFFFu), sy = (int)(int16_t)(e.xy >> 16);
                const int iw = in_w[cam], ih = in_h[cam];
                int mask, fxy;
                if (e.code & kCodeTex) {
                    if (sx < 0 || sy < 0 || sx + 1 >= iw || sy + 1 >= ih) {
                        wide = true;
                        continue;
                    }
                    mask = 15;
                    fxy = (int)((e.code & 255u) | ((e.code >> 17) & 255u) << 8);
                    item_tex = true;
                } else {
                    const TapCell tc = tap_cell(e.xy, iw, ih);
                    mask = ((tc.ix0 && tc.iy0) ? 1 : 0) | ((tc.ix1 && tc.iy0) ? 2 : 0) | ((tc.ix0 && tc.iy1) ? 4 : 0) |
                           ((tc.ix1 && tc.iy1) ? 8 : 0);
                    if (!mask) continue;
                    if (sx < 0 || sy < 0) {
                        wide = true;
                        continue;
                    }
                    fxy = (int)(e.code & 1023u);
                }
                const int x0 = sx, y0 = sy, x1 = x0 + 1, y1 = y0 + 1;
                int sl = -1;
                for (int j = 0; j < ns; j++)
                    if (cams[j] == cam) sl = j;
                if (sl < 0) {
                    if (ns == 8) {
                        wide = true;
                        continue;
                    }
                    sl = ns++;
                    cams[sl] = cam;
                    minx[sl] = miny[sl] = INT32_MAX;
                    maxx[sl] = maxy[sl] = -1;
                }
                minx[sl] = std::min(minx[sl], x0);
                maxx[sl] = std::max(maxx[sl], x1);
                miny[sl] = std::min(miny[sl], y0);
                maxy[sl] = std::max(maxy[sl], y1);
                px[k] = Px{sl, x0, y0, fxy, mask, (e.code & kCodeNoGain) ? 1 : 0};
            }
            if (ns > kTileSlots) wide = true;
            TileSlot ts[kTileSlots] = {};
            int bws[kTileSlots] = {}, bhs[kTileSlots] = {};
            uint32_t stride = 0;
            for (int j = 0; j < ns && !wide; j++) {
                if (in_w[cams[j]] % 8) {
                    wide = true;
                    break;
                }
                const int bx0 = minx[j] & ~7, by0 = miny[j] & ~1;
                const int bx1 = (maxx[j] + 1 + 7) & ~7, by1 = (maxy[j] + 1 + 1) & ~1;
                bws[j] = bx1 - bx0;
                bhs[j] = by1 - by0;
                if (bws[j] > 256 || bhs[j] > 256) {
                    wide = true;
                    break;
                }
                ts[j].cam = (uint16_t)cams[j];
                ts[j].bw = (uint16_t)bws[j];
                ts[j].bh = (uint16_t)bhs[j];
                ts[j].bx0 = (uint16_t)bx0;
                ts[j].by0 = (uint16_t)by0;
                stride = std::max<uint32_t>(stride, (uint32_t)bws[j]);
            }
            std::vector<uint16_t>& G = grp_job[t];
            G.clear();
            uint32_t chunks = 0, groups = 0;
            if (!wide) {
                std::vector<int> g_lo[kTileSlots], g_hi[kTileSlots];
                for (int j = 0; j < ns; j++) {
                    g_lo[j].assign(bhs[j], INT32_MAX);
                    g_hi[j].assign(bhs[j], -1);
                }
                for (int k = 0; k < item_px; k++) {
                    if (!px[k].mask) continue;
                    const int j = px[k].slot;
                    const int r = px[k].y0 - ts[j].by0, ga = (px[k].x0 - ts[j].bx0) >> 3, gb = (px[k].x0 + 1 - ts[j].bx0) >> 3;
                    for (int rr = r; rr <= r + 1; rr++) {
                        g_lo[j][rr] = std::min(g_lo[j][rr], ga);
                        g_hi[j][rr] = std::max(g_hi[j][rr], gb);
                    }
                }
                for (int j = 0; j < ns; j++) {
                    ts[j].chunk0 = (uint16_t)chunks;
                    uint32_t n = 0;
                    for (int r = 0; r < bhs[j]; r++)
                        for (int g = g_lo[j][r]; g <= g_hi[j][r]; g++, n++)
                            G.push_back((uint16_t)(kGroupValid | (uint32_t)g << 8 | (uint32_t)r));
                    const uint32_t c = (n + 63) / 64;
                    G.resize((size_t)(chunks + c) * 64, 0);
                    chunks += c;
                    groups += n;
                }
                std::vector<uint32_t> staged[kTileSlots];
                for (int j = 0; j < ns; j++) staged[j].assign(bhs[j], 0u);
                for (int j = 0; j < ns; j++) {
                    const uint32_t c_end = j + 1 < ns ? ts[j + 1].chunk0 : chunks;
                    for (uint32_t c = ts[j].chunk0; c < c_end; c++)
                        for (int i = 0; i < 64; i++) {
                            const uint16_t g = G[(size_t)c * 64 + i];
                            if (g & kGroupValid) staged[j][g & 255] |= 1u << ((g >> 8) & 31);
                        }
                }
                for (int k = 0; k < item_px; k++) {
                    if (!px[k].mask) continue;
                    const int j = px[k].slot, r = px[k].y0 - ts[j].by0;
                    const int ga = (px[k].x0 - ts[j].bx0) >> 3, gb = (px[k].x0 + 1 - ts[j].bx0) >> 3;
                    const uint32_t need = (1u << ga) | (1u << gb);
                    REQUIRE((staged[j][r] & need) == need && (staged[j][r + 1] & need) == need,
                            "tiled LUT: a tap outside the staged groups (internal error)");
                }
            }
            if (!wide && ns > 0) {
                uint32_t bh_sum = 0;
                for (int j = 0; j < ns; j++) bh_sum += (uint32_t)bhs[j];
                uint32_t lo[kTileSlots];
// ... 39 lines not shown
                    const uint64_t c = cycles(S);
                    if (c < best_cyc) {
                        best_cyc = c;
                        best = S;
                    }
                }
                stride = best;
            }
            uint32_t lds = kTileZeroDwords;
            for (int j = 0; j < ns && !wide; j++) {
                ts[j].lds = (uint16_t)std::min<uint32_t>(lds, 65535u);
                lds += stride * (uint32_t)bhs[j];
            }
            for (int j = ns; j < kTileSlots; j++) ts[j].chunk0 = (uint16_t)std::min<uint32_t>(chunks, 255u);
            if (chunks > 255) wide = true;
            if (lds * 4 > (uint32_t)kTileLdsBytes) wide = true;
            if (wide) {
                is_wide[t] = 1;
                wide_raw[t] = raw;
                G.clear();
                continue;
            }
            if (item_tex) any_tex = 1;
            b.hdr[t] = TileHdr{(uint32_t)J.tx | ((uint32_t)J.ty << 16),
                               (uint32_t)ns | (chunks << 8) | ((uint32_t)J.cam << 16),
                               2 * groups, stride};
            for (int j = 0; j < kTileSlots; j++) b.slots[(size_t)t * kTileSlots + j] = ts[j];
            uint32_t* out = b.entries.data() + (size_t)t * item_px;
            for (int k = 0; k < item_px; k++) {
                if (!px[k].mask) continue;
                const TileSlot& sl = ts[px[k].slot];
                const uint32_t off = sl.lds + (uint32_t)(px[k].y0 - sl.by0) * stride + (uint32_t)(px[k].x0 - sl.bx0);
                out[k] = item_tex ? tiled_entry_tex(off * 4u, (uint32_t)px[k].fxy, (uint32_t)px[k].slot, px[k].nogain != 0)
                                  : tiled_entry(off * 4u, (uint32_t)px[k].fxy, (uint32_t)px[k].slot, px[k].nogain != 0);
            }
        }
    };
    run_threads((size_t)T, [&](size_t i) { work((int)i); });
    b.tex = any_tex.load();
    int n_items = 0;
    for (int t = 0; t < n_jobs; t++) {
        if (is_wide[t]) {
            const TileJob& J = jobs[t];
            for (int h = 0; h < qpl; h++) {
                b.wide_tiles.push_back((uint32_t)J.tx | ((uint32_t)(J.ty * qpl + h) << 16));
                const uint32_t rq = (J.flags >> (4 * h)) & 15u, gq = (J.flags >> (8 + 4 * h)) & 15u;
                b.wide_cams.push_back((uint16_t)(J.cam | rq << 8 | gq << 12));
                b.wide.insert(b.wide.end(), wide_raw[t].begin() + (size_t)h * kTilePx,
                              wide_raw[t].begin() + (size_t)(h + 1) * kTilePx);
            }
            continue;
        }
        if (n_items != t) {
            b.hdr[n_items] = b.hdr[t];
            std::copy(b.slots.begin() + (size_t)t * kTileSlots, b.slots.begin() + (size_t)(t + 1) * kTileSlots,
                      b.slots.begin() + (size_t)n_items * kTileSlots);
            std::copy(b.entries.begin() + (size_t)t * item_px, b.entries.begin() + (size_t)(t + 1) * item_px,
                      b.entries.begin() + (size_t)n_items * item_px);
        }
        b.staged_bytes += 8.0 * b.hdr[n_items].stage_groups;
        b.item_flags.push_back((uint16_t)jobs[t].flags);
        {
            const std::vector<uint16_t>& G = grp_job[t];
            b.grp0.resize((size_t)(n_items + 1) * kGroupFirst * 64, 0);
            const size_t first = std::min<size_t>(G.size(), (size_t)kGroupFirst * 64);
            std::copy(G.begin(), G.begin() + first, b.grp0.begin() + (size_t)n_items * kGroupFirst * 64);
            const size_t ovf_chunk = b.grp1.size() / 64;
            REQUIRE(ovf_chunk < (1u << 23), "tiled LUT: staging group overflow table too large");
            b.hdr[n_items].stride |= (uint32_t)ovf_chunk << kStrideBits;
            b.grp1.insert(b.grp1.end(), G.begin() + first, G.end());
            std::vector<uint16_t>().swap(grp_job[t]);
        }
        n_items++;
    }
    b.n_items = n_items;
    b.n_wide = (int)b.wide_tiles.size();
    {
        const int nc = (int)in_w.size();
        std::vector<std::vector<uint8_t>> lum(nc), chr(nc);
        std::vector<int> cw(nc);
        for (int c = 0; c < nc; c++) {
            cw[c] = (in_w[c] + 7) / 8;
            lum[c].assign((size_t)cw[c] * in_h[c], 0);
            chr[c].assign((size_t)cw[c] * ((in_h[c] + 1) / 2), 0);
        }
        auto mark = [&](int c, int x, int y) {
            if (c < 0 || c >= nc || x < 0 || y < 0 || x >= in_w[c] || y >= in_h[c]) return;
            lum[c][(size_t)y * cw[c] + x / 8] = 1;
            chr[c][(size_t)(y / 2) * cw[c] + x / 8] = 1;
        };
        for (int t = 0; t < n_items; t++) {
            const int ns = (int)(b.hdr[t].nslots & 0xFFu), nch = (int)((b.hdr[t].nslots >> 8) & 0xFFu);
            for (int c = 0; c < nch; c++) {
                int j = 0;
                while (j + 1 < ns && c >= (int)b.slots[(size_t)t * kTileSlots + j + 1].chunk0) j++;
                const TileSlot& sl = b.slots[(size_t)t * kTileSlots + j];
                const uint16_t* g = c < kGroupFirst ? b.grp0.data() + ((size_t)t * kGroupFirst + c) * 64
                                                     : b.grp1.data() + ((size_t)(b.hdr[t].stride >> kStrideBits) + c - kGroupFirst) * 64;
                for (int i = 0; i < 64; i++)
                    if (g[i] & kGroupValid) mark(sl.cam, sl.bx0 + 8 * ((g[i] >> 8) & 31), sl.by0 + (g[i] & 255));
            }
        }
        for (const CompositeEntry& e : b.wide) {
            if (!(e.code & 0x8000u)) continue;
            const int c = (int)((e.code >> 10) & 31u);
            const int sx = (int)(int16_t)(e.xy & 0xFFFFu), sy = (int)(int16_t)(e.xy >> 16);
            for (int k = 0; k < 4; k++) mark(c, sx + (k & 1), sy + (k >> 1));
        }
        double groups = 0, pairs = 0;
        for (int c = 0; c < nc; c++) {
            for (uint8_t x : lum[c]) groups += x;
            for (uint8_t x : chr[c]) pairs += x;
        }
        b.source_bytes = groups * 8 + pairs * 8;
    }
    {
        std::vector<double> cum(n_items + 1, 0.0);
        for (int t = 0; t < n_items; t++) cum[t + 1] = cum[t] + 1.0;
        b.bands.assign(kStitchBands + 1, n_items);
        b.bands[0] = 0;
        int t = 0;
        for (int g = 1; g < kStitchBands; g++) {
            const double goal = cum[n_items] * g / kStitchBands;
            while (t < n_items && cum[t] < goal) t++;
            b.bands[g] = std::max(t, b.bands[g - 1]);
        }
    }
    {
        const int edges[] = {0, 1, 2, 3, 4, 6, 8, 12, 16, 32, 256};
        const int n_bins = (int)(sizeof(edges) / sizeof(edges[0])) - 1;
        std::vector<long> hist(n_bins, 0), lds_hist(7, 0);
        std::vector<long> band_chunks(kStitchBands, 0);
        for (int t = 0; t < n_items; t++) {
            const int ch = (int)((b.hdr[t].nslots >> 8) & 0xFFu);
            int k = 0;
            while (k + 1 < n_bins && ch >= edges[k + 1]) k++;
            hist[k]++;
            uint32_t lds = kTileZeroDwords;
            for (int j = 0; j < (int)(b.hdr[t].nslots & 0xFFu); j++)
                lds += (b.hdr[t].stride & ((1u << kStrideBits) - 1)) * b.slots[(size_t)t * kTileSlots + j].bh;
            const uint32_t kb = lds * 4u / 1024u;
            lds_hist[kb < 1 ? 0 : kb < 2 ? 1 : kb < 4 ? 2 : kb < 8 ? 3 : kb < 16 ? 4 : kb < 24 ? 5 : 6]++;
            for (int g = 0; g < kStitchBands; g++)
                if (t >= b.bands[g] && t < b.bands[g + 1]) band_chunks[g] += ch;
        }
        std::string s = "\"items_by_chunks\": {";
        for (int k = 0; k < n_bins; k++)
            s += (k ? ", \"" : "\"") + std::to_string(edges[k]) + "\": " + std::to_string(hist[k]);
        s += "}, \"items_by_lds_kib\": [";
        for (int k = 0; k < 7; k++) s += (k ? ", " : "") + std::to_string(lds_hist[k]);
        s += "], \"band_chunks\": [";
        for (int g = 0; g < kStitchBands; g++) s += (g ? ", " : "") + std::to_string(band_chunks[g]);
        s += "]";
        b.stats = s;
    }
    b.hdr.resize(std::max(n_items, 1));
    b.grp0.resize((size_t)std::max(n_items, 1) * kGroupFirst * 64, 0);
    if (b.grp1.empty()) b.grp1.assign(64, 0);
    b.slots.resize((size_t)std::max(n_items, 1) * kTileSlots);
    b.entries.resize((size_t)std::max(n_items, 1) * item_px);
    if (b.wide.empty()) {
        b.wide.push_back(CompositeEntry{0, 0});
        b.wide_tiles.push_back(0u);
        b.wide_cams.push_back(0);
    }
    return b;
}

void TiledLutDev::upload(const TiledLutBuild& b, bool want_e24) {
    static_assert(sizeof(TileHdr) == 16 && sizeof(TileSlot) == 16, "16-byte metadata words");
    std::vector<TileHdr> m(b.hdr.size() * kMetaWords);
    for (size_t t = 0; t < b.hdr.size(); t++) {
        m[t * kMetaWords] = b.hdr[t];
        uint32_t map = 0;
        const int ns = (int)(b.hdr[t].nslots & 0xFFu);
        for (int c = 0; c < 4; c++) {
            int q = 0;
            for (int j = 1; j < kTileSlots; j++) q += (j < ns && c >= (int)b.slots[t * kTileSlots + j].chunk0) ? 1 : 0;
            map |= (uint32_t)q << (2 * c);
        }
        if (t < b.item_flags.size()) map |= (uint32_t)b.item_flags[t] << 8;
        m[t * kMetaWords].stage_groups = map;
        std::memcpy(&m[t * kMetaWords + 1], &b.slots[t * kTileSlots], kTileSlots * sizeof(TileSlot));
    }
    meta.upload(m.data(), m.size());
    REQUIRE(b.grp0.size() * 2 < (size_t)1 << 31 && b.grp1.size() * 2 < (size_t)1 << 31, "staging group tables exceed 2 GiB");
    grp0.upload(b.grp0.data(), b.grp0.size());
    grp1.upload(b.grp1.data(), b.grp1.size());
    REQUIRE(b.entries.size() * sizeof(uint32_t) < (size_t)1 << 32, "tiled LUT entries exceed 4 GiB");
    bool e24 = want_e24 && !b.tex && std::getenv("OCTVR_ENTRY32") == nullptr;
    for (size_t k = 0; e24 && k < b.entries.size(); k++) e24 = (b.entries[k] & kEntryNoGain) == 0u;
    if (e24) {
        REQUIRE(b.entries.size() % 4 == 0, "tiled entries: whole quads");
        std::vector<uint32_t> p(b.entries.size() / 4 * 3);
        for (size_t q = 0; q < b.entries.size() / 4; q++) {
            const uint32_t c0 = tiled_entry24(b.entries[4 * q]), c1 = tiled_entry24(b.entries[4 * q + 1]);
            const uint32_t c2 = tiled_entry24(b.entries[4 * q + 2]), c3 = tiled_entry24(b.entries[4 * q + 3]);
            p[3 * q] = c0 | c1 << 24;
            p[3 * q + 1] = c1 >> 8 | c2 << 16;
            p[3 * q + 2] = c2 >> 16 | c3 << 8;
        }
        entries.upload(p.data(), p.size());
    } else {
        entries.upload(b.entries.data(), b.entries.size());
    }
    wide.upload(b.wide.data(), b.wide.size());
    wide_tiles.upload(b.wide_tiles.data(), b.wide_tiles.size());
    wide_cams.upload(b.wide_cams.data(), b.wide_cams.size());
    bands.upload(b.bands.data(), b.bands.size());
    queue.alloc((size_t)(kStitchBands + 1) * kQueueStride);
    HIP_CHECK(hipMemset(queue.p, 0, queue.n * sizeof(uint32_t)));
    staged_bytes = b.staged_bytes;
    source_bytes = b.source_bytes;
    result_bytes = 0;
    g0_bytes = 0;
    constexpr double kSubPx = (double)kSubW * kTileH;
    for (size_t t = 0; t < b.item_flags.size(); t++) {
        const uint32_t f = b.item_flags[t];
        g0_bytes += 4.0 * kSubPx * __builtin_popcount(f & 0xFF00u);
        result_bytes += kSubPx * __builtin_popcount(f & 0xFFu);
    }
    if (!b.item_flags.empty())
        for (uint16_t c : b.wide_cams) {
            g0_bytes += 4.0 * kSubPx * __builtin_popcount((uint32_t)c >> 12);
            result_bytes += kSubPx * __builtin_popcount(((uint32_t)c >> 8) & 15u);
        }
    if (b.item_flags.empty()) g0_bytes = 4.0 * kTilePx * ((double)b.n_items * b.qpl + b.n_wide);
    stats = b.stats;
    view = TiledLut{meta.p, entries.p, b.n_items, wide_tiles.p, wide.p, b.n_wide, wide_cams.p, bands.p, queue.p,
                    b.qpl, grp0.p, grp1.p, (uint32_t)b.grp1.size(), b.tex, e24 ? 1 : 0};
}

void SourceFootprint::init(const std::vector<int>& in_w, const std::vector<int>& in_h) {
    w = in_w;
    h = in_h;
    bits.assign(w.size(), {});
    for (size_t i = 0; i < w.size(); i++) bits[i].assign((size_t)row_pairs((int)i) * words((int)i), 0ull);
}

void SourceFootprint::mark_taps(const CompositeEntry& e) {
    if (!(e.code & 0x8000u)) return;
    const int cam = (int)((e.code >> 10) & 31u);
    if (cam >= (int)w.size()) return;
    const TapCell c = tap_cell(e.xy, w[cam], h[cam]);
    const bool all = (e.code & kCodeTex) != 0;
    if (all || (c.iy0 && c.ix0)) mark(cam, c.y0, c.x0 >> 3);
    if (all || (c.iy0 && c.ix1)) mark(cam, c.y0, c.x1 >> 3);
    if (all || (c.iy1 && c.ix0)) mark(cam, c.y1, c.x0 >> 3);
    if (all || (c.iy1 && c.ix1)) mark(cam, c.y1, c.x1 >> 3);
}

void SourceFootprint::merge(const SourceFootprint& o) {
    REQUIRE(o.w == w && o.h == h, "footprints of different input sizes");
    for (size_t i = 0; i < bits.size(); i++)
        for (size_t k = 0; k < bits[i].size(); k++) bits[i][k] |= o.bits[i][k];
}

double SourceFootprint::bytes() const {
    double n = 0;
    for (int i = 0; i < (int)w.size(); i++)
        for (int r = 0; r < row_pairs(i); r++)
            for (int g = 0; g < groups(i); g++) {
                if (!test(i, r, g)) continue;
                const int yb = std::min(8, w[i] - 8 * g), cb = std::max(0, std::min(4, w[i] / 2 - 4 * g));
                n += yb * (2 * r + 1 < h[i] ? 2 : 1) + 2 * cb;
            }
    return n;
}

void footprint_add_tiles(SourceFootprint& f, const TiledLutBuild& b) {
    for (int t = 0; t < b.n_items; t++) {
        const TileHdr& hd = b.hdr[t];
        const int ns = (int)(hd.nslots & 0xFFu), nch = (int)((hd.nslots >> 8) & 0xFFu);
        const TileSlot* ts = b.slots.data() + (size_t)t * kTileSlots;
        for (int c = 0; c < nch; c++) {
            int j = 0;
            for (int k = 1; k < ns; k++)
                if (c >= (int)ts[k].chunk0) j = k;
            const uint16_t* G = c < kGroupFirst ? b.grp0.data() + ((size_t)t * kGroupFirst + c) * 64
                                                : b.grp1.data() + ((size_t)(hd.stride >> kStrideBits) + c - kGroupFirst) * 64;
            const int cam = ts[j].cam;
            for (int l = 0; l < 64; l++) {
                if (!(G[l] & kGroupValid)) continue;
                const int y = ts[j].by0 + (G[l] & 255), x = ts[j].bx0 + ((G[l] >> 8) & 31) * 8;
                if (y < f.h[cam] && x < f.w[cam]) f.mark(cam, y, x >> 3);
            }
        }
    }
    for (const CompositeEntry& e : b.wide) f.mark_taps(e);
}

}
```

### opencv-octvr_amd/octvr_amd/__init__.py

```python
import ctypes as C
import json as _json
import os

import numpy as np
import torch

_HERE = os.path.dirname(os.path.abspath(__file__))
LIB_PATH = os.environ.get("OCTVR_HIP_LIB") or os.path.join(os.path.dirname(_HERE), "lib", "liboctvr_hip.so")

if not os.path.exists(LIB_PATH):
    raise ImportError(
        "liboctvr_hip.so not found at %s — build it with `make -C opencv-octvr_amd` or "
        "`python -c 'import __graft_entry__ as g; g.build()'`" % LIB_PATH)

_lib = C.CDLL(LIB_PATH)


E_INVALID, E_PARSE, E_HIP, E_UNSUPPORTED, E_IO = -1, -2, -3, -4, -5


class OctvrError(RuntimeError):
    def __init__(self, code, msg):
        super().__init__("octvr error %d: %s" % (code, msg))
        self.code = code


class InputView(C.Structure):
    _fields_ = [("roi_x", C.c_int), ("roi_y", C.c_int), ("roi_w", C.c_int), ("roi_h", C.c_int),
                ("map1", C.c_void_p), ("map2", C.c_void_p), ("mask", C.c_void_p), ("seam_mask", C.c_void_p),
                ("vignette", C.c_void_p), ("vignette_w", C.c_int), ("vignette_h", C.c_int)]


def _check(rc):
    if rc != 0:
        raise OctvrError(rc, _lib.octvr_last_error().decode())


_lib.octvr_last_error.restype = C.c_char_p
_VP = C.c_void_p
_lib.octvr_rig_create_json.argtypes = [C.c_char_p, C.c_int, C.c_int, C.c_int, C.c_int, C.POINTER(_VP)]
_lib.octvr_rig_load_dat.argtypes = [C.c_char_p, C.POINTER(_VP)]
_lib.octvr_rig_dump_dat.argtypes = [_VP, C.c_char_p]
_lib.octvr_rig_create_masks.argtypes = [_VP, C.c_int]
_lib.octvr_rig_create_from_arrays.argtypes = [C.c_int, C.c_int, C.c_int, C.POINTER(C.c_int), C.POINTER(_VP),
                                              C.POINTER(_VP), C.POINTER(_VP), C.POINTER(_VP), C.POINTER(_VP)]
_lib.octvr_rig_num_inputs.argtypes = [_VP, C.POINTER(C.c_int)]
_lib.octvr_rig_out_size.argtypes = [_VP, C.POINTER(C.c_int), C.POINTER(C.c_int)]
_lib.octvr_rig_get_input.argtypes = [_VP, C.c_int, C.POINTER(InputView)]
_lib.octvr_rig_num_overlays.argtypes = [_VP, C.POINTER(C.c_int)]
_lib.octvr_rig_get_overlay.argtypes = [_VP, C.c_int, C.POINTER(InputView)]
_lib.octvr_rig_morph_controlpoints.argtypes = [_VP, C.c_char_p, C.POINTER(C.c_int)]
_lib.octvr_rig_get_triangles.argtypes = [_VP, C.c_int, _VP, _VP, C.c_int, C.POINTER(C.c_int)]
_lib.octvr_rig_destroy.argtypes = [_VP]
_lib.octvr_rig_destroy.restype = None
_lib.octvr_mapper_create.argtypes = [_VP, C.c_int, C.c_int, C.POINTER(C.c_int), C.POINTER(C.c_int), C.c_int, C.c_int,
                                     C.c_int, C.c_int, C.POINTER(_VP)]
if hasattr(_lib, "octvr_mapper_create_ex"):
    _lib.octvr_mapper_create_ex.argtypes = [_VP, C.c_int, C.c_int, C.POINTER(C.c_int), C.POINTER(C.c_int), C.c_int,
                                            C.c_int, C.c_int, C.c_int, C.c_int, C.POINTER(_VP)]
REMAP_TEXTURE = 1
_lib.octvr_mapper_stitch_batch.argtypes = [_VP, C.c_int, C.POINTER(_VP), C.POINTER(C.c_size_t), C.POINTER(_VP),
                                           C.c_size_t, _VP, _VP]
_lib.octvr_mapper_stitch_yuv420p.argtypes = [_VP, C.POINTER(_VP), C.POINTER(C.c_size_t), _VP, C.c_size_t,
                                             C.POINTER(C.c_double), C.c_int, _VP]
_lib.octvr_mapper_stitch_preview.argtypes = [_VP, C.POINTER(_VP), C.POINTER(C.c_size_t), _VP, C.c_size_t, _VP, C.c_int,
                                             C.c_int, C.c_size_t, C.POINTER(C.c_double), C.c_int, _VP]
_lib.octvr_mapper_gains.argtypes = [_VP, C.POINTER(C.c_double), C.c_int]
_lib.octvr_mapper_set_frames_in_flight.argtypes = [_VP, C.c_int]
if hasattr(_lib, "octvr_mapper_set_pixel_formats"):
    _lib.octvr_mapper_set_pixel_formats.argtypes = [_VP, C.c_int, C.c_int]
    _lib.octvr_mapper_pixel_formats.argtypes = [_VP, C.POINTER(C.c_int), C.POINTER(C.c_int)]
_lib.octvr_mapper_traffic.argtypes = [_VP, C.POINTER(C.c_double)]
_lib.octvr_mapper_set_timing.argtypes = [_VP, C.c_int]
_lib.octvr_mapper_kernel_time.argtypes = [_VP, C.POINTER(C.c_double), C.POINTER(C.c_int)]
_lib.octvr_mapper_kernel_busy.argtypes = [_VP, C.POINTER(C.c_double), C.POINTER(C.c_double), C.POINTER(C.c_int)]
_lib.octvr_mapper_kernel_intervals.argtypes = [_VP, C.POINTER(C.c_double), C.POINTER(C.c_double), C.c_int,
                                               C.POINTER(C.c_int)]
_lib.octvr_rig_lut_recomputed.argtypes = [_VP, C.c_int, C.POINTER(C.c_uint64)]
_lib.octvr_debug_project_f64.argtypes = [C.c_char_p, C.c_int, C.c_int, C.c_int, C.c_int, C.c_int, _VP, _VP, _VP]
_lib.octvr_interval_union.argtypes = [_VP, _VP, C.c_int, C.POINTER(C.c_double), C.POINTER(C.c_double)]
_lib.octvr_fastmapper_traffic.argtypes = [_VP, C.POINTER(C.c_double)]
_lib.octvr_mapper_info.argtypes = [_VP, C.c_char_p, C.c_size_t]
_lib.octvr_mapper_destroy.argtypes = [_VP]
_lib.octvr_mapper_destroy.restype = None
_lib.octvr_async_create.argtypes = [C.POINTER(_VP), C.c_int, C.c_int, C.c_int, C.POINTER(C.c_int), C.POINTER(C.c_int),
                                    C.c_int, C.c_int, C.POINTER(C.c_int), C.POINTER(C.c_int), C.POINTER(C.c_double),
                                    C.POINTER(_VP)]
if hasattr(_lib, "octvr_async_create_ex"):
    _lib.octvr_async_create_ex.argtypes = [C.POINTER(_VP), C.c_int, C.c_int, C.c_int, C.POINTER(C.c_int),
                                           C.POINTER(C.c_int), C.c_int, C.c_int, C.POINTER(C.c_int), C.POINTER(C.c_int),
                                           C.POINTER(C.c_double), C.c_int, C.POINTER(_VP)]
_lib.octvr_async_create_preview.argtypes = [C.POINTER(_VP), C.c_int, C.c_int, C.c_int, C.POINTER(C.c_int),
                                            C.POINTER(C.c_int), C.c_int, C.c_int, C.POINTER(C.c_int),
                                            C.POINTER(C.c_int), C.POINTER(C.c_double), C.c_int, C.c_int, C.c_int,
                                            C.POINTER(_VP)]


class PreviewDataHeader(C.Structure):
    _fields_ = [("width", C.c_int), ("height", C.c_int), ("step", C.c_int), ("fps", C.c_double)]


PREVIEW_SINK = C.CFUNCTYPE(None, C.c_void_p, C.POINTER(C.c_uint8), C.c_size_t, C.POINTER(PreviewDataHeader))
_lib.octvr_async_pop_preview.argtypes = [_VP, _VP, C.c_size_t, C.POINTER(PreviewDataHeader)]
_lib.octvr_async_set_preview_sink.argtypes = [_VP, PREVIEW_SINK, _VP]
_lib.octvr_async_info.argtypes = [_VP, C.c_char_p, C.c_size_t]
_lib.octvr_async_register_output.argtypes = [_VP, C.POINTER(_VP), C.POINTER(C.c_size_t)]
_lib.octvr_async_unregister_output.argtypes = [_VP, C.POINTER(_VP)]
_lib.octvr_async_push.argtypes = [_VP, C.POINTER(_VP), C.POINTER(C.c_size_t), C.POINTER(_VP), C.POINTER(C.c_size_t)]
if hasattr(_lib, "octvr_async_push_device"):
    _lib.octvr_async_push_device.argtypes = [_VP, C.POINTER(_VP), C.POINTER(C.c_size_t), _VP, C.c_size_t, _VP]
_lib.octvr_async_pop.argtypes = [_VP]
_lib.octvr_async_pending.argtypes = [_VP, C.POINTER(C.c_int)]
if hasattr(_lib, "octvr_async_set_pixel_formats"):
    _lib.octvr_async_set_pixel_formats.argtypes = [_VP, C.c_int, C.c_int]
    _lib.octvr_async_pixel_formats.argtypes = [_VP, C.POINTER(C.c_int), C.POINTER(C.c_int)]
_lib.octvr_async_destroy.argtypes = [_VP]
_lib.octvr_async_destroy.restype = None
_lib.octvr_fill_poly_u8.argtypes = [_VP, C.c_int, C.c_int, C.POINTER(C.c_int), C.c_int, C.c_uint8]
_lib.octvr_png_decode_rgb.argtypes = [C.c_char_p, C.c_size_t, _VP, C.c_size_t, C.POINTER(C.c_int), C.POINTER(C.c_int)]
_lib.octvr_fastmapper_create.argtypes = [_VP, C.c_int, C.c_int, C.POINTER(C.c_int), C.POINTER(C.c_int), C.POINTER(_VP)]
_lib.octvr_fastmapper_stitch_nv12.argtypes = [_VP, C.POINTER(_VP), C.POINTER(C.c_size_t), _VP, C.c_size_t, _VP]
_lib.octvr_fastmapper_stitch_nv12_batch.argtypes = [_VP, C.c_int, C.POINTER(_VP), C.POINTER(C.c_size_t),
                                                    C.POINTER(_VP), C.c_size_t, _VP]
_lib.octvr_fastmapper_traffic_parts.argtypes = [_VP, C.POINTER(C.c_double), C.POINTER(C.c_double)]
_lib.octvr_mapper_traffic_parts.argtypes = [_VP, C.POINTER(C.c_double), C.POINTER(C.c_double)]
_lib.octvr_fastmapper_destroy.argtypes = [_VP]
_lib.octvr_fastmapper_destroy.restype = None
if hasattr(_lib, "octvr_debug_json_number"):
    _lib.octvr_debug_json_number.argtypes = [C.c_char_p, C.c_int, C.POINTER(C.c_double)]
if hasattr(_lib, "octvr_debug_tiled_lut_info"):
    _lib.octvr_debug_tiled_lut_info.argtypes = [_VP, C.c_int, C.POINTER(C.c_int), C.POINTER(C.c_int), C.c_int,
                                                C.c_char_p, C.c_size_t]
if hasattr(_lib, "octvr_debug_fastmapper_audit"):
    _lib.octvr_debug_fastmapper_audit.argtypes = [_VP, C.c_int, C.POINTER(C.c_int), C.POINTER(C.c_int), C.c_int,
                                                  C.c_int, C.c_char_p, C.c_size_t]
if hasattr(_lib, "octvr_debug_gain_plan"):
    _lib.octvr_debug_gain_plan.argtypes = [_VP, C.c_int, C.POINTER(C.c_int), C.POINTER(C.c_int), C.c_int, _VP, _VP,
                                           C.c_size_t, C.POINTER(C.c_size_t)]
if hasattr(_lib, "octvr_debug_pack_runs"):
    _lib.octvr_debug_pack_runs.argtypes = [C.c_int, C.POINTER(C.c_int), C.POINTER(C.c_int), _VP, C.c_int, C.POINTER(_VP),
                                           C.POINTER(C.c_size_t), C.c_int, _VP, C.c_size_t, _VP, C.POINTER(C.c_size_t)]
if hasattr(_lib, "octvr_debug_worker_failure"):
    _lib.octvr_debug_worker_failure.argtypes = [C.c_int, C.c_int]
_lib.octvr_remap_u8.argtypes = [_VP, C.c_int, C.c_int, C.c_size_t, C.c_int, _VP, _VP, C.c_int, C.c_int, C.c_size_t,
                                C.c_float, C.c_float, _VP, C.c_size_t, _VP]


def lib():
    return _lib


def abi_version():
    return _lib.octvr_abi_version()


def debug_project_f64(rig_json, out_w, out_h, input, device=0, where=0):
    import numpy as _np
    x = _np.empty((out_h, out_w), _np.float64)
    y = _np.empty((out_h, out_w), _np.float64)
    f = _np.zeros((out_h, out_w), _np.uint8)
    _check(_lib.octvr_debug_project_f64(rig_json.encode() if isinstance(rig_json, str) else rig_json, out_w, out_h,
                                        int(input), int(device), int(where), x.ctypes.data_as(_VP),
                                        y.ctypes.data_as(_VP), f.ctypes.data_as(_VP)))
    return x, y, (f if where == 0 else None)


def debug_tiled_lut_info(mt, in_sizes, remap="remap"):
    n = len(in_sizes)
    w = (C.c_int * n)(*[s[0] for s in in_sizes])
    h = (C.c_int * n)(*[s[1] for s in in_sizes])
    buf = C.create_string_buffer(4096)
    _check(_lib.octvr_debug_tiled_lut_info(mt._h, n, w, h, REMAP_TEXTURE if remap == "texture" else 0, buf, len(buf)))
    import json as _json
    return _json.loads(buf.value.decode())


def _plane_args(plane_sets):
    planes = []
    for tri in plane_sets:
        tri = list(tri)
        if len(tri) not in (2, 3):
            raise ValueError("a plane set is (Y, U, V), or (Y, UV) for an NV12 side")
        tri += [None] * (3 - len(tri))
        for p in tri:
            if p is not None:
                assert p.dtype == np.uint8 and p.ndim == 2 and p.strides[1] == 1, \
                    "uint8 2-D planes with unit column stride"
            planes.append(p)
    ptr = (_VP * len(planes))(*[None if p is None else p.ctypes.data for p in planes])
    pitch = (C.c_size_t * len(planes))(*[0 if p is None else p.strides[0] for p in planes])
    return ptr, pitch, planes


def debug_pack_runs(in_sizes, runs, planes, fmt="yuv420p"):
    n = len(in_sizes)
    w = (C.c_int * n)(*[s[0] for s in in_sizes])
    h = (C.c_int * n)(*[s[1] for s in in_sizes])
    r = np.ascontiguousarray(np.asarray(runs, np.uint32).reshape(-1, 4))
    ptr, pitch, keep = _plane_args(planes)
    cap = int(sum(3 * 8 * int(x[3]) for x in r)) + 8
    packed = np.full(cap, 0x5A, np.uint8)
    sizes = np.zeros(len(r), np.uintp)
    total = C.c_size_t()
    _check(_lib.octvr_debug_pack_runs(n, w, h, r.ctypes.data_as(_VP), len(r), ptr, pitch, _pix_value(fmt),
                                      packed.ctypes.data_as(_VP), cap, sizes.ctypes.data_as(_VP), C.byref(total)))
    assert (packed[total.value:] == 0x5A).all()
    return packed[:total.value].copy(), sizes.astype(np.int64)


def debug_worker_failure(n_threads, failing):
    _check(_lib.octvr_debug_worker_failure(int(n_threads), int(failing)))


def debug_gain_plan(mt, in_sizes, remap="remap"):
    import numpy as _np
    n = len(in_sizes)
    w = (C.c_int * n)(*[s[0] for s in in_sizes])
    h = (C.c_int * n)(*[s[1] for s in in_sizes])
    fl = REMAP_TEXTURE if remap == "texture" else 0
    cnt = C.c_size_t()
    _check(_lib.octvr_debug_gain_plan(mt._h, n, w, h, fl, None, None, 0, C.byref(cnt)))
    e = _np.zeros((cnt.value, 2), _np.uint32)
    p = _np.zeros(cnt.value, _np.uint16)
    _check(_lib.octvr_debug_gain_plan(mt._h, n, w, h, fl, e.ctypes.data, p.ctypes.data, cnt.value, C.byref(cnt)))
    return e, p


def debug_json_number(text, exact=True):
    v = C.c_double()
    _check(_lib.octvr_debug_json_number(text.encode(), 1 if exact else 0, C.byref(v)))
    return v.value


def debug_fastmapper_audit(mt, in_sizes, wide=False, pitch_pad=0):
    n = len(in_sizes)
    w = (C.c_int * n)(*[s[0] for s in in_sizes])
    h = (C.c_int * n)(*[s[1] for s in in_sizes])
    buf = C.create_string_buffer(4096)
    rc = _lib.octvr_debug_fastmapper_audit(mt._h, n, w, h, int(bool(wide)), int(pitch_pad), buf, len(buf))
    import json as _json
    if not buf.value:
        _check(rc)
    return rc == 0, _json.loads(buf.value.decode())


def interval_union(starts, ends):
    import numpy as _np
    a = _np.ascontiguousarray(starts, _np.float64)
    b = _np.ascontiguousarray(ends, _np.float64)
    sp, bu = C.c_double(), C.c_double()
    _check(_lib.octvr_interval_union(a.ctypes.data_as(_VP), b.ctypes.data_as(_VP), len(a), C.byref(sp), C.byref(bu)))
    return sp.value, bu.value


def _stream_ptr(stream):
    if isinstance(stream, C.c_void_p):
        return stream
    if stream is None:
        stream = torch.cuda.current_stream()
    return C.c_void_p(stream.cuda_stream)


class MapperTemplate:

    def __init__(self, handle):
        self._h = C.c_void_p(handle)

    @classmethod
    def from_json(cls, rig, out_w, out_h, use_roi=True, device=0):
        text = rig if isinstance(rig, str) else _json.dumps(rig)
        h = _VP()
        _check(_lib.octvr_rig_create_json(text.encode(), out_w, out_h, int(use_roi), device, C.byref(h)))
        return cls(h.value)

    @classmethod
    def load(cls, path):
        h = _VP()
        _check(_lib.octvr_rig_load_dat(os.fsencode(path), C.byref(h)))
        return cls(h.value)

    @classmethod
    def from_arrays(cls, out_w, out_h, rois, map1s, map2s, masks, seams=None):
        n = len(rois)
        map1s = [np.ascontiguousarray(a, np.float32) for a in map1s]
        map2s = [np.ascontiguousarray(a, np.float32) for a in map2s]
        masks = [np.ascontiguousarray(a, np.uint8) for a in masks]
        r = (C.c_int * (4 * n))(*[int(v) for roi in rois for v in roi])
        p1 = (_VP * n)(*[a.ctypes.data for a in map1s])
        p2 = (_VP * n)(*[a.ctypes.data for a in map2s])
        pm = (_VP * n)(*[a.ctypes.data for a in masks])
        ps = None
        if seams is not None:
            seams = [np.ascontiguousarray(a, np.uint8) for a in seams]
            ps = (_VP * n)(*[a.ctypes.data for a in seams])
        h = _VP()
        _check(_lib.octvr_rig_create_from_arrays(out_w, out_h, n, r, p1, p2, pm, ps, C.byref(h)))
        return cls(h.value)

    def dump(self, path):
        _check(_lib.octvr_rig_dump_dat(self._h, os.fsencode(path)))

    def lut_recomputed(self, i):
        n = C.c_uint64()
        _check(_lib.octvr_rig_lut_recomputed(self._h, i, C.byref(n)))
        return n.value

    def create_masks(self, device=0):
        _check(_lib.octvr_rig_create_masks(self._h, device))

    def morph_controlpoints(self, control_points):
        text = control_points if isinstance(control_points, str) else _json.dumps(control_points)
        k = C.c_int()
        _check(_lib.octvr_rig_morph_controlpoints(self._h, text.encode(), C.byref(k)))
        return k.value

    def triangles(self, i):
        n = C.c_int()
        _check(_lib.octvr_rig_get_triangles(self._h, i, None, None, 0, C.byref(n)))
        src = np.zeros((n.value, 6), np.float32)
        dst = np.zeros((n.value, 6), np.float32)
        _check(_lib.octvr_rig_get_triangles(self._h, i, src.ctypes.data, dst.ctypes.data, n.value, C.byref(n)))
        return src, dst

    @property
    def out_size(self):
        w, h = C.c_int(), C.c_int()
        _check(_lib.octvr_rig_out_size(self._h, C.byref(w), C.byref(h)))
# ... 470 lines not shown
```

Measured before the change: 699,700.

## Pack tiled LUT entries into 64-bit quad records to halve LUT traffic

Adds a compressed LUT format in which each quad of four 32-bit pixel entries is encoded as one 64-bit record (shared base offset, per-pixel flags, shared gain slot). Packable items are flagged in the tile header. The stitch kernel then loads a single 128-bit word per item instead of two and decodes offsets with udot2. Non-packable items fall back to loading the second half lazily. The aim is to cut LUT bandwidth, at the cost of extra decode ALU work, more kernel instances, and a branch on the packed flag per tile.

```diff
diff --git a/include/octvr_hip.h b/include/octvr_hip.h
--- a/include/octvr_hip.h
+++ b/include/octvr_hip.h
@@ -156,6 +156,8 @@
                                  int pitch_pad, char* json, size_t len);
 int octvr_debug_tiled_lut_info(const octvr_rig* rig, int n_inputs, const int* in_w, const int* in_h, int flags,
                                char* json, size_t len);
+int octvr_debug_entry_pack(const uint32_t* entries, int n_quads, uint32_t stride, uint64_t* records, uint8_t* ok,
+                           uint32_t* unpacked);
 int octvr_debug_gain_plan(const octvr_rig* rig, int n_inputs, const int* in_w, const int* in_h, int flags,
                           uint32_t* samples, uint16_t* partners, size_t cap, size_t* count);
 int octvr_debug_json_number(const char* json, int flags, double* value);
diff --git a/opencv-octvr_amd/csrc/composite.hip b/opencv-octvr_amd/csrc/composite.hip
--- a/opencv-octvr_amd/csrc/composite.hip
+++ b/opencv-octvr_amd/csrc/composite.hip
@@ -229,25 +229,29 @@
     StageGroup sg;
 };
 
-template <bool DWORD_STAGE, bool VIG, bool E24, int IN = kInPlanar>
+template <bool E24, bool EP>
+__device__ __forceinline__ void entry_issue(const __amdgpu_buffer_rsrc_t& er, const TileMeta& m, int t_end, int lg, int h,
+                                            TileData& d) {
+    const bool live = m.t < t_end;
+    const int tid = threadIdx.x;
+    const uint32_t so =
+        (uint32_t)uniform(((live ? m.t : 0) >> lg) * kItemHalves + h) * (uint32_t)(kTilePx * (E24 ? 3 : 4));
+    if constexpr (E24) {
+        typedef unsigned int u32x3e __attribute__((ext_vector_type(3)));
+        const u32x3e v = __builtin_amdgcn_raw_buffer_load_b96(er, (uint32_t)tid * 12u, so, 0);
+        d.e4[h] = uint4{v.x, v.y, v.z, 0u};
+    } else {
+        typedef unsigned int u32x4e __attribute__((ext_vector_type(4)));
+        const u32x4e v = __builtin_amdgcn_raw_buffer_load_b128(er, (uint32_t)tid * 16u, so, 0);
+        d.e4[h] = uint4{v.x, v.y, v.z, v.w};
+    }
+}
+
+template <bool DWORD_STAGE, bool VIG, bool E24, int IN = kInPlanar, bool EP = false>
 __device__ __forceinline__ void data_issue(const __amdgpu_buffer_rsrc_t& er, const TileMeta& m, int t_end, int lg,
                                            const StageSlot& sl, uint32_t g, TileData& d, bool nv12 = false) {
-    const bool live = m.t < t_end;
-    const int tid = threadIdx.x;
-#pragma unroll
-    for (int h = 0; h < kItemHalves; h++) {
-        const uint32_t so =
-            (uint32_t)uniform(((live ? m.t : 0) >> lg) * kItemHalves + h) * (uint32_t)(kTilePx * (E24 ? 3 : 4));
-        if constexpr (E24) {
-            typedef unsigned int u32x3e __attribute__((ext_vector_type(3)));
-            const u32x3e v = __builtin_amdgcn_raw_buffer_load_b96(er, (uint32_t)tid * 12u, so, 0);
-            d.e4[h] = uint4{v.x, v.y, v.z, 0u};
-        } else {
-            typedef unsigned int u32x4e __attribute__((ext_vector_type(4)));
-            const u32x4e v = __builtin_amdgcn_raw_buffer_load_b128(er, (uint32_t)tid * 16u, so, 0);
-            d.e4[h] = uint4{v.x, v.y, v.z, v.w};
-        }
-    }
+#pragma unroll
+    for (int h = 0; h < (EP ? 1 : kItemHalves); h++) entry_issue<E24, EP>(er, m, t_end, lg, h, d);
     if (!sl.live) {
         d.sg.dst = -1;
         return;
@@ -342,7 +346,7 @@
 __device__ __forceinline__ uint32_t tap_off(uint32_t e) { return (e >> 13) & 0x3FFFu; }
 
 constexpr int kPfPlanar = 0, kPfNv12 = 3, kPfRuntime = 4;
-template <bool DWORD_STAGE, int MODE, bool VIG, bool TEX, int LG, bool E24, int PF = kPfPlanar>
+template <bool DWORD_STAGE, int MODE, bool VIG, bool TEX, int LG, bool E24, int PF = kPfPlanar, bool EP = false>
 __device__ __forceinline__ void stitch_tiled_body(const FrameBatch<1 << LG>& frames, TiledLut lut, int W, int H, int use_gain,
                                                   int64_t out_pitch, RgbaOut rgba, int pix = 0) {
     constexpr int IN = PF == kPfRuntime ? kInRuntime : PF == kPfNv12 ? kInNv12 : kInPlanar;
@@ -354,6 +358,7 @@
     uint32_t* const s_rgb = L.rgb;
     float* const s_gain = reinterpret_cast<float*>(s_wtab + 1024);
     constexpr int lg = LG, cam_lg = LG <= 1 ? 5 : 4;
+    static_assert(!EP || (!TEX && !E24), "quad records: the blend = 0 mapper's 32-bit LUT of the default sampling only");
     static_assert(MODE == 0 || LG == 0, "frame batches: MODE 0 only");
     f32x2_t* const s_slot_gain = L.slot_gain;
     uint32_t* const s_claim = L.claim;
@@ -402,7 +407,7 @@
     const uint32_t g0 = group_issue(grsrc, t0, t_end, lg);
     __syncthreads();
     TileData d;
-    data_issue<DWORD_STAGE, VIG, E24, IN>(ersrc, cur, t_end, lg, stage_slot<true>(cur, t_end, wave), g0, d, in_nv12);
+    data_issue<DWORD_STAGE, VIG, E24, IN, EP>(ersrc, cur, t_end, lg, stage_slot<true>(cur, t_end, wave), g0, d, in_nv12);
     int t_mv = t0 + step < t_end ? t0 + step : t_end;
     int t_n2 = t_mv < t_end && t0 + 2 * step < t_end ? t0 + 2 * step : t_end;
     uint4 mv = meta_issue(mrsrc, t_mv, t_end, lg);
@@ -412,7 +417,7 @@
     bool first = true;
     asm volatile("" : "+v"(mv.x), "+v"(mv.y), "+v"(mv.z), "+v"(mv.w), "+v"(mg));
 #pragma unroll
-    for (int h = 0; h < kItemHalves; h++) {
+    for (int h = 0; h < (EP ? 1 : kItemHalves); h++) {
         asm volatile("" : "+v"(d.e4[h].x), "+v"(d.e4[h].y), "+v"(d.e4[h].z));
         if constexpr (!E24) asm volatile("" : "+v"(d.e4[h].w));
     }
@@ -435,7 +440,7 @@
         const uint32_t S = cur.stride & ((1u << kStrideBits) - 1u);
         uint4 e4[kItemHalves];
 #pragma unroll
-        for (int h = 0; h < kItemHalves; h++) e4[h] = d.e4[h];
+        for (int h = 0; h < (EP ? 1 : kItemHalves); h++) e4[h] = d.e4[h];
         __syncthreads();
         if (tid < kTileZeroDwords) s_rgb[tid] = 0u;
         const TileMeta nxt = meta_read(mv, t_mv, lg, cam_lg);
@@ -487,7 +492,7 @@
             for (int h = 0; h < kItemHalves; h++)
                 store_half<MODE, OUT>(of, ro, res_rgba, prev[h], pcam, pfl, h, px, py + h * kTileH, pin && py + h * kTileH < H);
         }
-        data_issue<DWORD_STAGE, VIG, E24, IN>(ersrc, nxt, t_end, lg, stage_slot<true>(nxt, t_end, wave), mg, d, in_nv12);
+        data_issue<DWORD_STAGE, VIG, E24, IN, EP>(ersrc, nxt, t_end, lg, stage_slot<true>(nxt, t_end, wave), mg, d, in_nv12);
         mv = meta_issue(mrsrc, t_n2, t_end, lg);
         mg = group_issue(grsrc, t_n2, t_end, lg);
         t_mv = t_n2;
@@ -497,8 +502,7 @@
             asm volatile("" : "+v"(zero));
             claim = __hip_atomic_fetch_add(q + zero, 1u, __ATOMIC_RELAXED, __HIP_MEMORY_SCOPE_AGENT);
         }
-#pragma unroll
-        for (int h = 0; h < kItemHalves; h++) {
+        auto half_entries = [&](int h) {
             const uint32_t ent[4] = {e4[h].x, E24 ? __builtin_amdgcn_alignbit(e4[h].y, e4[h].x, 24u) : e4[h].y,
                                      E24 ? __builtin_amdgcn_alignbit(e4[h].z, e4[h].y, 16u) : e4[h].z,
                                      E24 ? e4[h].z >> 8 : e4[h].w};
@@ -525,6 +529,41 @@
                 if (MODE == 1 && !E24 && (e & kEntryNoGain)) gain[p] = f32x2_t{1.0f, 1.0f};
             }
             prev[h] = finish_any<MODE>(rgb, gain);
+        };
+        auto half_records = [&](int h, uint32_t lo, uint32_t hi) {
+            float rgb[4][3];
+            f32x2_t gain[4];
+            const uint32_t base4 = quad_base4(hi);
+            const f32x2_t gq = *reinterpret_cast<const f32x2_t*>(reinterpret_cast<const uint8_t*>(s_slot_gain) + quad_gain_off(hi));
+#pragma unroll
+            for (int p = 0; p < 4; p++) {
+                const uint32_t off = __builtin_amdgcn_udot2(
+                    __builtin_bit_cast(u16x2_t, hi & quad_flag_mask(p)),
+                    __builtin_bit_cast(u16x2_t, (uint32_t)uniform((int)quad_flag_mul(p, S))), base4, false);
+                const uint8_t* r0 = reinterpret_cast<const uint8_t*>(s_rgb) + off;
+                const uint8_t* r1 = r0 + 4u * S;
+                const uint32_t c00 = reinterpret_cast<const uint32_t*>(r0)[0];
+                const uint32_t c01 = reinterpret_cast<const uint32_t*>(r0)[1];
+                const uint32_t c10 = reinterpret_cast<const uint32_t*>(r1)[0];
+                const uint32_t c11 = reinterpret_cast<const uint32_t*>(r1)[1];
+                bilerp_rgba_w(c00, c01, c10, c11, wtab_read(quad_fxy_view(p, lo, hi)), rgb[p]);
+                gain[p] = gq;
+            }
+            prev[h] = finish_any<MODE>(rgb, gain);
+        };
+        bool records = false;
+        if constexpr (EP) records = (cur.nslots & kItemPacked) != 0u;
+        if (records) {
+            half_records(0, e4[0].x, e4[0].y);
+            half_records(1, e4[0].z, e4[0].w);
+        } else {
+            half_entries(0);
+            if constexpr (EP) {
+                TileData dd;
+                entry_issue<E24, EP>(ersrc, cur, t_end, lg, 1, dd);
+                e4[1] = dd.e4[1];
+            }
+            half_entries(1);
         }
         px = x;
         py = y;
@@ -553,18 +592,18 @@
         store_half<MODE, OUT>(of, ro, res_rgba, prev[h], pcam, pfl, h, px, py + h * kTileH, pin && py + h * kTileH < H);
 }
 
-template <bool DWORD_STAGE, int MODE, bool VIG, int LG, bool E24, int PF = kPfPlanar>
+template <bool DWORD_STAGE, int MODE, bool VIG, int LG, bool E24, int PF = kPfPlanar, bool EP = false>
 __global__ void __launch_bounds__(256, kStitchRegBlocks) __attribute__((amdgpu_num_sgpr(kStitchSgprs)))
 __attribute__((amdgpu_num_vgpr(kStitchVgprs))) stitch_tiled_kernel(FrameBatch<1 << LG> frames, TiledLut lut, int W, int H,
                                                                    int use_gain, int64_t out_pitch, RgbaOut rgba) {
-    stitch_tiled_body<DWORD_STAGE, MODE, VIG, false, LG, E24, PF>(frames, lut, W, H, use_gain, out_pitch, rgba);
-}
-template <int MODE, bool TEX, int LG, bool E24>
+    stitch_tiled_body<DWORD_STAGE, MODE, VIG, false, LG, E24, PF, EP>(frames, lut, W, H, use_gain, out_pitch, rgba);
+}
+template <int MODE, bool TEX, int LG, bool E24, bool EP = false>
 __global__ void __launch_bounds__(256, kStitchTexRegBlocks) __attribute__((amdgpu_num_sgpr(kStitchSgprs)))
 __attribute__((amdgpu_num_vgpr(kStitchTexVgprs))) stitch_tiled_pix_kernel(FrameBatch<1 << LG> frames, TiledLut lut, int W,
                                                                           int H, int use_gain, int64_t out_pitch,
                                                                           RgbaOut rgba, int pix) {
-    stitch_tiled_body<false, MODE, true, TEX, LG, E24, kPfRuntime>(frames, lut, W, H, use_gain, out_pitch, rgba, pix);
+    stitch_tiled_body<false, MODE, true, TEX, LG, E24, kPfRuntime, EP>(frames, lut, W, H, use_gain, out_pitch, rgba, pix);
 }
 template <bool DWORD_STAGE, int MODE, bool VIG, int LG>
 __global__ void __launch_bounds__(256, kStitchTexRegBlocks) __attribute__((amdgpu_num_sgpr(kStitchSgprs)))
@@ -642,14 +681,14 @@
     int lg;
 };
 
-template <bool DW, int MODE, bool V, bool TEX, int LG, bool E24, int PF>
+template <bool DW, int MODE, bool V, bool TEX, int LG, bool E24, int PF, bool EP>
 constexpr auto tiled_kernel() {
     if constexpr (PF == kPfRuntime)
-        return &stitch_tiled_pix_kernel<MODE, TEX, LG, E24>;
+        return &stitch_tiled_pix_kernel<MODE, TEX, LG, E24, EP>;
     else if constexpr (TEX)
         return &stitch_tiled_tex_kernel<DW, MODE, V, LG>;
     else
-        return &stitch_tiled_kernel<DW, MODE, V, LG, E24, PF>;
+        return &stitch_tiled_kernel<DW, MODE, V, LG, E24, PF, EP>;
 }
 
 static hipError_t stitch_lds_check(const void* kernel) {
@@ -673,10 +712,10 @@
     }
 }
 
-template <bool DW, int MODE, bool V, bool TEX, int LG, bool E24, int PF>
+template <bool DW, int MODE, bool V, bool TEX, int LG, bool E24, int PF, bool EP>
 static hipError_t launch_tiled(const TiledLaunch& a) {
     static_assert(PF != kPfNv12 || !TEX, "compiled-in NV12: the default sampling's instances");
-    constexpr auto kernel = tiled_kernel<DW, MODE, V, TEX, LG, E24, PF>();
+    constexpr auto kernel = tiled_kernel<DW, MODE, V, TEX, LG, E24, PF, EP>();
     static const hipError_t lds_ok = stitch_lds_check(reinterpret_cast<const void*>(kernel));
     if (lds_ok != hipSuccess) return lds_ok;
     FrameBatch<1 << LG> fb;
@@ -699,35 +738,37 @@
     return hipGetLastError();
 }
 
-template <bool DW, int MODE, bool V, bool TEX, bool E24, int PF = kPfPlanar>
+template <bool DW, int MODE, bool V, bool TEX, bool E24, int PF = kPfPlanar, bool EP = false>
 static hipError_t launch_tiled_lg(const TiledLaunch& a) {
     if constexpr (MODE == 0) {
-        if (a.lg == 1) return launch_tiled<DW, MODE, V, TEX, 1, E24, PF>(a);
-        if (a.lg == 2) return launch_tiled<DW, MODE, V, TEX, 2, E24, PF>(a);
+        if (a.lg == 1) return launch_tiled<DW, MODE, V, TEX, 1, E24, PF, EP>(a);
+        if (a.lg == 2) return launch_tiled<DW, MODE, V, TEX, 2, E24, PF, EP>(a);
     }
     if (a.lg != 0) return hipErrorInvalidValue;
-    return launch_tiled<DW, MODE, V, TEX, 0, E24, PF>(a);
-}
-
-template <int MODE, bool TEX, bool E24>
+    return launch_tiled<DW, MODE, V, TEX, 0, E24, PF, EP>(a);
+}
+
+template <int MODE, bool TEX, bool E24, bool EP = false>
 static hipError_t launch_tiled_vd(const TiledLaunch& a) {
     if (a.pix) {
         if constexpr (MODE == 0 && !TEX) {
             if (a.pix == (kPixInNv12 | kPixOutNv12) && a.dw && !a.vig)
-                return launch_tiled_lg<true, MODE, false, TEX, E24, kPfNv12>(a);
-        }
-        return launch_tiled_lg<false, MODE, true, TEX, E24, kPfRuntime>(a);
-    }
-    if (a.dw && !a.vig) return launch_tiled_lg<true, MODE, false, TEX, E24>(a);
-    if (a.dw) return launch_tiled_lg<true, MODE, true, TEX, E24>(a);
-    if (!a.vig) return launch_tiled_lg<false, MODE, false, TEX, E24>(a);
-    return launch_tiled_lg<false, MODE, true, TEX, E24>(a);
+                return launch_tiled_lg<true, MODE, false, TEX, E24, kPfNv12, EP>(a);
+        }
+        return launch_tiled_lg<false, MODE, true, TEX, E24, kPfRuntime, EP>(a);
+    }
+    if (a.dw && !a.vig) return launch_tiled_lg<true, MODE, false, TEX, E24, kPfPlanar, EP>(a);
+    if (a.dw) return launch_tiled_lg<true, MODE, true, TEX, E24, kPfPlanar, EP>(a);
+    if (!a.vig) return launch_tiled_lg<false, MODE, false, TEX, E24, kPfPlanar, EP>(a);
+    return launch_tiled_lg<false, MODE, true, TEX, E24, kPfPlanar, EP>(a);
 }
 
 template <int MODE, bool TEX>
 static hipError_t launch_tiled_for(const TiledLaunch& a) {
+    if (a.lut.n_packed > 0 && (TEX || a.lut.e24)) return hipErrorInvalidValue;
     if constexpr (!TEX) {
         if (a.lut.e24) return launch_tiled_vd<MODE, TEX, true>(a);
+        if (a.lut.n_packed > 0) return launch_tiled_vd<MODE, TEX, false, true>(a);
     } else {
         if (a.lut.e24) return hipErrorInvalidValue;
     }
diff --git a/opencv-octvr_amd/csrc/debug_abi.cpp b/opencv-octvr_amd/csrc/debug_abi.cpp
--- a/opencv-octvr_amd/csrc/debug_abi.cpp
+++ b/opencv-octvr_amd/csrc/debug_abi.cpp
@@ -187,6 +187,18 @@
     });
 }
 
+int octvr_debug_entry_pack(const uint32_t* entries, int n_quads, uint32_t stride, uint64_t* records, uint8_t* ok,
+                           uint32_t* unpacked) {
+    return guarded([&] {
+        REQUIRE(entries && records && ok && unpacked && n_quads >= 0, "bad arguments");
+        REQUIRE(stride < (1u << kStrideBits), "stride exceeds its header field");
+        for (int q = 0; q < n_quads; q++) {
+            ok[q] = quad_pack(entries + 4 * (size_t)q, stride, &records[q]) ? 1 : 0;
+            quad_unpack(records[q], stride, unpacked + 4 * (size_t)q);
+        }
+    });
+}
+
 int octvr_debug_json_number(const char* json, int flags, double* value) {
     return guarded([&] {
         REQUIRE(json && value, "NULL argument");
diff --git a/opencv-octvr_amd/csrc/host_common.hpp b/opencv-octvr_amd/csrc/host_common.hpp
--- a/opencv-octvr_amd/csrc/host_common.hpp
+++ b/opencv-octvr_amd/csrc/host_common.hpp
@@ -171,6 +171,8 @@
     double staged_bytes = 0;
     double source_bytes = 0;
     std::string stats;
+    std::vector<uint8_t> packable;
+    int n_packable = 0;
 };
 TiledLutBuild build_tiled_lut(const std::vector<TileJob>& jobs, const EntryFn& entry, const std::vector<int>& in_w,
                               const std::vector<int>& in_h, int qpl = 1);
@@ -189,7 +191,8 @@
     double result_bytes = 0;
     std::string stats;
     TiledLut view{};
-    void upload(const TiledLutBuild& b, bool e24 = false);
+    void upload(const TiledLutBuild& b, bool e24 = false, bool quad = false);
+    int n_packed = 0;
 };
 
 struct SourceFootprint {
diff --git a/opencv-octvr_amd/csrc/kernels.hpp b/opencv-octvr_amd/csrc/kernels.hpp
--- a/opencv-octvr_amd/csrc/kernels.hpp
+++ b/opencv-octvr_amd/csrc/kernels.hpp
@@ -204,6 +204,7 @@
     uint32_t n_grp1;
     int tex;
     int e24;
+    int n_packed;
 };
 constexpr int kMetaWords = 1 + kTileSlots;
 constexpr int kQueueStride = 32;
@@ -218,6 +219,65 @@
 
 __host__ __device__ constexpr uint32_t tiled_entry24(uint32_t e) {
     return (e >> 30) | ((e >> 3) & 1023u) << 2 | ((e >> 15) & 4095u) << 12;
+}
+
+constexpr uint32_t kItemPacked = 1u << 24;
+__host__ __device__ constexpr uint32_t quad_flag_mask(int p) {
+    return p == 3 ? (1u << 16 | 1u << 3) : (1u << p | 1u << (17 + p));
+}
+__host__ __device__ constexpr uint32_t quad_flag_mul(int p, uint32_t S) {
+    return p == 3 ? ((S >> 1) | 4u << 16) : ((4u >> p) | ((2u * S) >> p) << 16);
+}
+__host__ __device__ constexpr uint32_t quad_fxy_view(int p, uint32_t lo, uint32_t hi) {
+    return p == 0 ? lo << 1 : p == 1 ? lo >> 9 : p == 2 ? lo >> 19 : hi >> 19;
+}
+__host__ __device__ constexpr uint32_t quad_base4(uint32_t hi) { return (hi >> 2) & 0x3FFCu; }
+__host__ __device__ constexpr uint32_t quad_gain_off(uint32_t hi) { return (hi >> 17) & 0x18u; }
+
+__host__ __device__ inline void quad_unpack(uint64_t rec, uint32_t S, uint32_t e[4]) {
+    const uint32_t lo = (uint32_t)rec, hi = (uint32_t)(rec >> 32);
+    for (int p = 0; p < 4; p++) {
+        if (!rec) {
+            e[p] = 0u;
+            continue;
+        }
+        const uint32_t a = hi & quad_flag_mask(p), m = quad_flag_mul(p, S);
+        const uint32_t off = quad_base4(hi) + (a & 0xFFFFu) * (m & 0xFFFFu) + (a >> 16) * (m >> 16);
+        e[p] = (quad_fxy_view(p, lo, hi) & 0x1FF8u) | off << 13 | (quad_gain_off(hi) >> 3) << 30;
+    }
+}
+
+__host__ __device__ inline bool quad_pack(const uint32_t e[4], uint32_t S, uint64_t* rec) {
+    *rec = 0;
+    if (!(e[0] | e[1] | e[2] | e[3])) return true;
+    if (S < 8u || (S & 3u)) return false;
+    uint32_t o[4], lo_o = 0xFFFFFFFFu;
+    for (int p = 0; p < 4; p++) {
+        if (!e[p] || (e[p] & 7u) || (e[p] >> 27 & 7u) || (e[p] >> 30) != (e[0] >> 30)) return false;
+        if ((e[p] >> 13) & 3u) return false;
+        o[p] = ((e[p] >> 13) & 0x3FFFu) >> 2;
+        lo_o = o[p] < lo_o ? o[p] : lo_o;
+    }
+    for (uint32_t back = 0; back < 2; back++) {
+        if (lo_o < back) break;
+        const uint32_t base = lo_o - back;
+        uint32_t dx[4], dy[4];
+        bool ok = true;
+        for (int p = 0; p < 4 && ok; p++) {
+            const uint32_t d = o[p] - base;
+            ok = d == 0u || d == 1u || d == S || d == S + 1u;
+            dx[p] = (d == 1u || d == S + 1u) ? 1u : 0u;
+            dy[p] = d >= S ? 1u : 0u;
+        }
+        if (!ok) continue;
+        const uint32_t f[4] = {(e[0] >> 3) & 1023u, (e[1] >> 3) & 1023u, (e[2] >> 3) & 1023u, (e[3] >> 3) & 1023u};
+        const uint32_t lo = f[0] << 2 | f[1] << 12 | f[2] << 22;
+        const uint32_t hi = dx[0] | dx[1] << 1 | dx[2] << 2 | dy[3] << 3 | base << 4 | dx[3] << 16 | dy[0] << 17 |
+                            dy[1] << 18 | dy[2] << 19 | (e[0] >> 30) << 20 | f[3] << 22;
+        *rec = (uint64_t)hi << 32 | lo;
+        return true;
+    }
+    return false;
 }
 
 __host__ __device__ constexpr uint32_t tiled_entry_tex(uint32_t off, uint32_t ab, uint32_t slot, bool nogain) {
diff --git a/opencv-octvr_amd/csrc/mapper.cpp b/opencv-octvr_amd/csrc/mapper.cpp
--- a/opencv-octvr_amd/csrc/mapper.cpp
+++ b/opencv-octvr_amd/csrc/mapper.cpp
@@ -350,7 +350,7 @@
         const std::vector<CompositeEntry> lut8 = winner_lut(*m, camera, 0, m->nc);
         const TiledLutBuild tb = build_frame_tiles(lut8, m->W, m->H, m->in_w, m->in_h, &m->n_tiles);
         footprint_add_tiles(m->foot, tb);
-        m->tiles.upload(tb);
+        m->tiles.upload(tb, false, true);
     }
     if (m->mb && n_ov) setup_overlays(*m, camera);
     if (m->scaled || m->ov.view.n_groups) ensure_result(*m);
@@ -421,8 +421,8 @@
     return launches;
 }
 
-double tiled_lut_bytes(const TiledLut& t) {
-    return (t.e24 ? 3.0 : 4.0) * t.n_items * kTilePx * t.qpl + 8.0 * t.n_wide * kTilePx +
+double tiled_lut_bytes(const TiledLut& t, int n_packed) {
+    return (t.e24 ? 3.0 : 4.0) * t.n_items * kTilePx * t.qpl - 2.0 * n_packed * kTilePx * t.qpl + 8.0 * t.n_wide * kTilePx +
            (double)t.n_items * (sizeof(TileHdr) + kTileSlots * sizeof(TileSlot)) + 4.0 * t.n_wide;
 }
 
@@ -431,7 +431,7 @@
         return multiband_traffic(*m->mb) + 4.0 * m->W * m->H + 1.5 * m->SW * m->SH +
                (double)m->ov.view.n_groups * (4.0 + 8.0 * kOvGroupPx) + m->ov.source_bytes + 4.0 * (double)m->ov.covered;
     if (m->mb) return multiband_traffic(*m->mb);
-    return tiled_lut_bytes(m->tiles.view) + 1.5 * m->W * m->H + m->tiles.source_bytes;
-}
-
-}
+    return tiled_lut_bytes(m->tiles.view, m->tiles.n_packed) + 1.5 * m->W * m->H + m->tiles.source_bytes;
+}
+
+}
diff --git a/opencv-octvr_amd/csrc/mapper.hpp b/opencv-octvr_amd/csrc/mapper.hpp
--- a/opencv-octvr_amd/csrc/mapper.hpp
+++ b/opencv-octvr_amd/csrc/mapper.hpp
@@ -83,7 +83,7 @@
 void mapper_set_timing(octvr_mapper* m, int enable);
 int mapper_drain_timing(octvr_mapper* m, const std::function<void(double start_ms, double end_ms)>& f);
 double mapper_traffic(const octvr_mapper* m);
-double tiled_lut_bytes(const TiledLut& t);
+double tiled_lut_bytes(const TiledLut& t, int n_packed = 0);
 TiledLutBuild build_frame_tiles(const std::vector<CompositeEntry>& lut, int W, int H, const std::vector<int>& in_w,
                                 const std::vector<int>& in_h, int* n_jobs = nullptr);
 int mapper_num_inputs(const octvr_mapper* m);
diff --git a/opencv-octvr_amd/csrc/octvr_hip.cpp b/opencv-octvr_amd/csrc/octvr_hip.cpp
--- a/opencv-octvr_amd/csrc/octvr_hip.cpp
+++ b/opencv-octvr_amd/csrc/octvr_hip.cpp
@@ -398,7 +398,7 @@
 int octvr_mapper_traffic_parts(const octvr_mapper* m, double* lut_bytes, double* frame_bytes) {
     return guarded([&] {
         REQUIRE(m && lut_bytes && frame_bytes, "NULL argument");
-        *lut_bytes = m->mb ? 0.0 : tiled_lut_bytes(m->tiles.view);
+        *lut_bytes = m->mb ? 0.0 : tiled_lut_bytes(m->tiles.view, m->tiles.n_packed);
         *frame_bytes = mapper_traffic(m) - *lut_bytes;
     });
 }
@@ -487,7 +487,7 @@
                  m->foot.bytes(), m->nc - m->n, m->ov.view.n_groups, m->ov.covered);
         std::string js = tmp;
         if (m->mb) js += ", " + multiband_info(*m->mb);
-        else if (!m->tiles.stats.empty()) js += ", " + m->tiles.stats;
+        else if (!m->tiles.stats.empty()) js += ", " + m->tiles.stats + ", \"items_packed\": " + std::to_string(m->tiles.n_packed);
         js += "}";
         REQUIRE(js.size() < len, "buffer too small");
         memcpy(buf, js.c_str(), js.size() + 1);
diff --git a/opencv-octvr_amd/csrc/tiling.cpp b/opencv-octvr_amd/csrc/tiling.cpp
--- a/opencv-octvr_amd/csrc/tiling.cpp
+++ b/opencv-octvr_amd/csrc/tiling.cpp
@@ -9,6 +9,13 @@
 #include "kernels.hpp"
 
 namespace octvr {
+
+static bool item_packable(const uint32_t* E, int item_px, uint32_t S) {
+    uint64_t rec;
+    for (int k = 0; k < item_px; k += 4)
+        if (!quad_pack(E + k, S, &rec)) return false;
+    return true;
+}
 
 TiledLutBuild build_tiled_lut(const std::vector<TileJob>& jobs, const EntryFn& entry, const std::vector<int>& in_w,
                               const std::vector<int>& in_h, int qpl) {
@@ -354,6 +361,13 @@
         s += "], \"band_chunks\": [";
         for (int g = 0; g < kStitchBands; g++) s += (g ? ", " : "") + std::to_string(band_chunks[g]);
         s += "]";
+        b.packable.assign((size_t)std::max(n_items, 1), 0);
+        for (int t = 0; t < n_items && !b.tex; t++) {
+            b.packable[t] = item_packable(b.entries.data() + (size_t)t * kTilePx * qpl, kTilePx * qpl,
+                                          b.hdr[t].stride & ((1u << kStrideBits) - 1u)) ? 1 : 0;
+            b.n_packable += b.packable[t];
+        }
+        s += ", \"items_packable\": " + std::to_string(b.n_packable);
         b.stats = s;
     }
     b.hdr.resize(std::max(n_items, 1));
@@ -369,9 +383,20 @@
     return b;
 }
 
-void TiledLutDev::upload(const TiledLutBuild& b, bool want_e24) {
+constexpr bool kQuadPackDefault = true;
+static bool quad_pack_wanted(int n_packable, int n_items) {
+    if (std::getenv("OCTVR_ENTRY32")) return false;
+    const char* v = std::getenv("OCTVR_ENTRY_QUAD");
+    if (v && *v) return std::strcmp(v, "0") != 0;
+    return kQuadPackDefault && 2 * n_packable > n_items;
+}
+
+void TiledLutDev::upload(const TiledLutBuild& b, bool want_e24, bool want_quad) {
     static_assert(sizeof(TileHdr) == 16 && sizeof(TileSlot) == 16, "16-byte metadata words");
     std::vector<TileHdr> m(b.hdr.size() * kMetaWords);
+    const bool quad = want_quad && !want_e24 && !b.tex && b.qpl == kItemHalves && b.n_packable > 0 &&
+                      quad_pack_wanted(b.n_packable, b.n_items);
+    n_packed = 0;
     for (size_t t = 0; t < b.hdr.size(); t++) {
         m[t * kMetaWords] = b.hdr[t];
         uint32_t map = 0;
@@ -383,6 +408,7 @@
         }
         if (t < b.item_flags.size()) map |= (uint32_t)b.item_flags[t] << 8;
         m[t * kMetaWords].stage_groups = map;
+        if (quad && t < b.packable.size() && t < (size_t)b.n_items && b.packable[t]) m[t * kMetaWords].nslots |= kItemPacked;
         std::memcpy(&m[t * kMetaWords + 1], &b.slots[t * kTileSlots], kTileSlots * sizeof(TileSlot));
     }
     meta.upload(m.data(), m.size());
@@ -403,6 +429,24 @@
             p[3 * q + 2] = c2 >> 16 | c3 << 8;
         }
         entries.upload(p.data(), p.size());
+    } else if (quad && b.n_packable > 0) {
+        std::vector<uint32_t> p(b.entries);
+        const size_t item_px = (size_t)kTilePx * b.qpl;
+        for (int t = 0; t < b.n_items; t++) {
+            if (!b.packable[t]) continue;
+            uint32_t* E = p.data() + (size_t)t * item_px;
+            const uint32_t S = b.hdr[t].stride & ((1u << kStrideBits) - 1u);
+            for (size_t k = 0; k < item_px; k += 4) {
+                uint64_t rec = 0;
+                REQUIRE(quad_pack(b.entries.data() + (size_t)t * item_px + k, S, &rec), "tiled LUT: quad record (internal error)");
+                const size_t h = k / kTilePx, q = (k % kTilePx) / 4;
+                E[q * 4 + h * 2] = (uint32_t)rec;
+                E[q * 4 + h * 2 + 1] = (uint32_t)(rec >> 32);
+            }
+            std::fill(E + kTilePx, E + item_px, 0u);
+            n_packed++;
+        }
+        entries.upload(p.data(), p.size());
     } else {
         entries.upload(b.entries.data(), b.entries.size());
     }
@@ -430,7 +474,7 @@
     if (b.item_flags.empty()) g0_bytes = 4.0 * kTilePx * ((double)b.n_items * b.qpl + b.n_wide);
     stats = b.stats;
     view = TiledLut{meta.p, entries.p, b.n_items, wide_tiles.p, wide.p, b.n_wide, wide_cams.p, bands.p, queue.p,
-                    b.qpl, grp0.p, grp1.p, (uint32_t)b.grp1.size(), b.tex, e24 ? 1 : 0};
+                    b.qpl, grp0.p, grp1.p, (uint32_t)b.grp1.size(), b.tex, e24 ? 1 : 0, n_packed};
 }
 
 void SourceFootprint::init(const std::vector<int>& in_w, const std::vector<int>& in_h) {
diff --git a/opencv-octvr_amd/octvr_amd/__init__.py b/opencv-octvr_amd/octvr_amd/__init__.py
--- a/opencv-octvr_amd/octvr_amd/__init__.py
+++ b/opencv-octvr_amd/octvr_amd/__init__.py
@@ -131,6 +131,8 @@
 if hasattr(_lib, "octvr_debug_tiled_lut_info"):
     _lib.octvr_debug_tiled_lut_info.argtypes = [_VP, C.c_int, C.POINTER(C.c_int), C.POINTER(C.c_int), C.c_int,
                                                 C.c_char_p, C.c_size_t]
+if hasattr(_lib, "octvr_debug_entry_pack"):
+    _lib.octvr_debug_entry_pack.argtypes = [_VP, C.c_int, C.c_uint32, _VP, _VP, _VP]
 if hasattr(_lib, "octvr_debug_fastmapper_audit"):
     _lib.octvr_debug_fastmapper_audit.argtypes = [_VP, C.c_int, C.POINTER(C.c_int), C.POINTER(C.c_int), C.c_int,
                                                   C.c_int, C.c_char_p, C.c_size_t]
@@ -173,6 +175,18 @@
     _check(_lib.octvr_debug_tiled_lut_info(mt._h, n, w, h, REMAP_TEXTURE if remap == "texture" else 0, buf, len(buf)))
     import json as _json
     return _json.loads(buf.value.decode())
+
+
+def debug_entry_pack(entries, stride):
+    import numpy as _np
+    e = _np.ascontiguousarray(entries, _np.uint32).reshape(-1, 4)
+    n = e.shape[0]
+    rec = _np.zeros(n, _np.uint64)
+    ok = _np.zeros(n, _np.uint8)
+    un = _np.zeros((n, 4), _np.uint32)
+    _check(_lib.octvr_debug_entry_pack(e.ctypes.data_as(_VP), n, int(stride), rec.ctypes.data_as(_VP),
+                                       ok.ctypes.data_as(_VP), un.ctypes.data_as(_VP)))
+    return ok.astype(bool), rec, un
 
 
 def _plane_args(plane_sets):
```

Result: faster. 716,200 (median of 6 runs) (+2.4%).
